# gsc74/DipGenie

Hardware: AMD Instinct MI355X
Metric: dp_state_cells_per_s (higher is better)
Workload: dtype int32

## Files before the change

### dipgenie_amd/capi.py

```python
import contextlib
import ctypes as C
import os
import struct

import numpy as np

_HERE = os.path.dirname(os.path.abspath(__file__))
LIB_PATH = os.environ.get("DG_LIB") or os.path.join(_HERE, "csrc", "libdipgenie_hip.so")

if not os.path.exists(LIB_PATH):
    raise ImportError(
        f"{LIB_PATH} is missing: build it with `make -C dipgenie_amd/csrc` (or __graft_entry__.build()). "
        "dipgenie_amd has no CPU fallback."
    )
try:
    import torch
except ImportError:
    pass
lib = C.CDLL(LIB_PATH)


class DpGraph(C.Structure):
    _fields_ = [
        ("n_vertices", C.c_int32), ("n_levels", C.c_int32), ("R", C.c_int32),
        ("level_off", C.c_void_p), ("out_off", C.c_void_p), ("out_dst", C.c_void_p), ("out_w", C.c_void_p),
        ("hom_off", C.c_void_p), ("het_off", C.c_void_p), ("hom_col", C.c_void_p), ("het_col", C.c_void_p),
    ]


class DpResult(C.Structure):
    _fields_ = [
        ("value", C.c_int32), ("s_het", C.c_int32), ("n_p1", C.c_int32), ("n_p2", C.c_int32),
        ("p1_from", C.c_void_p), ("p1_to", C.c_void_p), ("p2_from", C.c_void_p), ("p2_to", C.c_void_p),
        ("cap", C.c_int32), ("cells", C.c_uint64), ("relaxations", C.c_uint64),
    ]


class DpTiming(C.Structure):
    _fields_ = [
        ("delta_ms", C.c_float), ("forward_ms", C.c_float), ("traceback_ms", C.c_float), ("total_ms", C.c_float),
        ("n_forward_launches", C.c_int64), ("edge_pairs", C.c_uint64), ("colour_entries", C.c_uint64),
        ("state_bytes", C.c_uint64), ("bp_bytes", C.c_uint64), ("delta_bytes", C.c_uint64), ("n_segments", C.c_int32), ("n_chunks", C.c_int32),
    ]


PAIR_SCORE = np.dtype([("value", np.int32), ("s_het", np.int32), ("r1", np.int32), ("r2", np.int32)])

PARTNER = np.dtype([("value", np.int32), ("s_het", np.int32), ("r1", np.int32), ("r2", np.int32)])

LEVEL_MARGIN = np.dtype([("best_vertex", np.int32), ("best_value", np.int32), ("second_vertex", np.int32), ("second_value", np.int32)])

CALL_MARGIN = np.dtype([("vertex", np.int32), ("value", np.int32), ("alt_vertex", np.int32), ("alt_value", np.int32)])

PAIR_OBJECTIVE = np.dtype([("hom_shared", np.int32), ("hom_single", np.int32), ("het_single", np.int32), ("het_both", np.int32)])


class SketchTiming(C.Structure):
    _fields_ = [("kernel_ms", C.c_float), ("sort_ms", C.c_float), ("total_ms", C.c_float), ("n_emitted", C.c_int64)]


SYMBOLS = [
    "dg_create", "dg_destroy", "dg_last_error", "dg_set_stream", "dg_synchronize", "dg_device_info",
    "dg_dp_prealloc", "dg_dp_load_graph", "dg_dp_run", "dg_dp_get_timing", "dg_dp_solve_diploid", "dg_dp_get_level_digest",
    "dg_dp_set_option", "dg_dp_get_launch_profile", "dg_sketch_reads", "dg_sketch_haplotype", "dg_hash_kmers", "dg_free",
    "dg_sketch_get_timing", "dg_sketch_reads_dev", "dg_sketch_count_dictionary_dev", "dg_sketch_merge_runs_dev",
    "dg_sketch_partition_dev", "dg_sketch_rank_dictionary_dev", "dg_sketch_histogram_dev",
    "dg_anchor_begin", "dg_anchor_add_haplotype", "dg_anchor_finish", "dg_dp_solve_haploid", "dg_dp_get_table_digest", "dg_hip_versions", "dg_anchor_add_haplotype_sketched",
    "dg_sketch_set_option", "dg_sketch_get_stat", "dg_sketch_count_rank_dictionary_dev",
    "dg_shard_create", "dg_shard_destroy", "dg_shard_n_ranks", "dg_shard_ctx", "dg_shard_score_reads",
    "dg_dp_run_budgets", "dg_dp_get_budget_values", "dg_dp_score_paths", "dg_dp_best_partners", "dg_dp_partner_marginals",
    "dg_dp_get_option", "dg_sketch_get_option", "dg_dp_list_sweep_variants", "dg_dp_get_answer_paths", "dg_dp_call_margins",
    "dg_dp_objective_paths", "dg_dp_answer_objectives", "dg_dp_get_partner_route",
]

lib.dg_create.restype = C.c_void_p
lib.dg_create.argtypes = [C.c_int]
lib.dg_destroy.argtypes = [C.c_void_p]
lib.dg_destroy.restype = None
lib.dg_last_error.restype = C.c_char_p
lib.dg_set_stream.argtypes = [C.c_void_p, C.c_void_p]
lib.dg_synchronize.argtypes = [C.c_void_p]
lib.dg_device_info.argtypes = [C.c_void_p, C.c_char_p, C.c_int, C.POINTER(C.c_int), C.POINTER(C.c_int64)]
lib.dg_dp_prealloc.argtypes = [C.c_void_p, C.c_int64]
lib.dg_dp_load_graph.argtypes = [C.c_void_p, C.POINTER(DpGraph)]
lib.dg_dp_run.argtypes = [C.c_void_p, C.POINTER(DpResult)]
lib.dg_dp_run_budgets.argtypes = [C.c_void_p, C.c_void_p, C.c_int32, C.POINTER(DpResult)]
lib.dg_dp_get_budget_values.argtypes = [C.c_void_p, C.c_void_p, C.c_int32]
lib.dg_dp_score_paths.argtypes = [C.c_void_p, C.c_void_p, C.c_int64, C.c_void_p]
lib.dg_dp_best_partners.argtypes = [C.c_void_p, C.c_void_p, C.c_int64, C.c_void_p, C.c_void_p, C.c_void_p]
lib.dg_dp_partner_marginals.argtypes = [C.c_void_p, C.c_void_p, C.c_int64, C.c_void_p, C.c_void_p, C.c_void_p]
lib.dg_dp_get_answer_paths.argtypes = [C.c_void_p, C.c_int32, C.c_void_p]
lib.dg_dp_call_margins.argtypes = [C.c_void_p, C.c_int32, C.c_void_p, C.c_void_p, C.c_void_p]
lib.dg_dp_get_partner_route.argtypes = [C.c_void_p, C.POINTER(C.c_int32), C.POINTER(C.c_int64)]
lib.dg_dp_objective_paths.argtypes = [C.c_void_p, C.c_void_p, C.c_int64, C.c_void_p]
lib.dg_dp_answer_objectives.argtypes = [C.c_void_p, C.c_void_p, C.c_int32, C.c_void_p]
lib.dg_dp_get_timing.argtypes = [C.c_void_p, C.POINTER(DpTiming)]
lib.dg_dp_solve_diploid.argtypes = [C.c_void_p, C.POINTER(DpGraph), C.POINTER(DpResult)]
lib.dg_dp_get_level_digest.argtypes = [C.c_void_p, C.c_void_p, C.c_int64]
lib.dg_dp_set_option.argtypes = [C.c_void_p, C.c_char_p, C.c_int64]
lib.dg_dp_get_option.argtypes = [C.c_void_p, C.c_char_p, C.POINTER(C.c_int64)]
lib.dg_dp_get_launch_profile.argtypes = [C.c_void_p, C.c_char_p, C.c_int]
lib.dg_dp_list_sweep_variants.argtypes = [C.c_char_p, C.c_int]
lib.dg_dp_get_table_digest.argtypes = [C.c_void_p, C.c_void_p, C.c_int]
lib.dg_sketch_reads.argtypes = [C.c_void_p, C.c_char_p, C.c_void_p, C.c_int64, C.c_int, C.c_int,
                                C.POINTER(C.c_void_p), C.POINTER(C.c_void_p), C.POINTER(C.c_int64)]
lib.dg_sketch_haplotype.argtypes = [C.c_void_p, C.c_char_p, C.c_int64, C.c_int, C.c_int,
                                    C.POINTER(C.c_void_p), C.POINTER(C.c_void_p), C.POINTER(C.c_int64)]
lib.dg_hash_kmers.argtypes = [C.c_void_p, C.c_char_p, C.c_int64, C.c_int, C.c_void_p]
lib.dg_free.argtypes = [C.c_void_p]
lib.dg_free.restype = None
lib.dg_sketch_get_timing.argtypes = [C.c_void_p, C.POINTER(SketchTiming)]
lib.dg_sketch_reads_dev.argtypes = [C.c_void_p, C.c_void_p, C.c_void_p, C.c_int64, C.c_int64, C.c_int, C.c_int,
                                    C.c_void_p, C.c_void_p, C.c_int64, C.POINTER(C.c_int64)]
lib.dg_sketch_count_dictionary_dev.argtypes = [C.c_void_p, C.c_void_p, C.c_int64, C.c_void_p, C.c_void_p, C.c_int64, C.c_void_p]
lib.dg_sketch_merge_runs_dev.argtypes = [C.c_void_p, C.c_void_p, C.c_void_p, C.c_int64, C.c_void_p, C.c_void_p,
                                         C.c_int64, C.POINTER(C.c_int64)]
lib.dg_sketch_partition_dev.argtypes = [C.c_void_p, C.c_void_p, C.c_int64, C.c_int, C.c_void_p]
lib.dg_sketch_rank_dictionary_dev.argtypes = [C.c_void_p, C.c_void_p, C.c_int64, C.c_void_p, C.c_int64, C.c_int64, C.c_void_p]
lib.dg_sketch_histogram_dev.argtypes = [C.c_void_p, C.c_void_p, C.c_int64, C.c_int, C.c_void_p]
lib.dg_sketch_count_rank_dictionary_dev.argtypes = [C.c_void_p, C.c_void_p, C.c_int64, C.c_void_p, C.c_void_p, C.c_int64, C.c_int64, C.c_void_p, C.c_void_p]
lib.dg_sketch_set_option.argtypes = [C.c_void_p, C.c_char_p, C.c_int64]
lib.dg_sketch_get_option.argtypes = [C.c_void_p, C.c_char_p, C.POINTER(C.c_int64)]
lib.dg_sketch_get_stat.argtypes = [C.c_void_p, C.c_char_p, C.POINTER(C.c_int64)]


class HapGraph(C.Structure):
    _fields_ = [("n_vertices", C.c_int32), ("R", C.c_int32), ("out_off", C.c_void_p), ("out_dst", C.c_void_p), ("out_w", C.c_void_p), ("n_colours", C.c_void_p)]


lib.dg_dp_solve_haploid.argtypes = [C.c_void_p, C.POINTER(HapGraph), C.c_void_p, C.c_void_p, C.c_void_p]


class AnchorResult(C.Structure):
    _fields_ = [("n_occ", C.c_int64), ("n_vtx", C.c_int64), ("occ_id", C.c_void_p), ("occ_hap", C.c_void_p), ("occ_off", C.c_void_p),
                ("occ_len", C.c_void_p), ("vpool", C.c_void_p), ("n_candidates", C.c_int64), ("n_unstable_groups", C.c_int64)]


lib.dg_anchor_begin.argtypes = [C.c_void_p, C.c_int32, C.c_int32, C.c_void_p, C.c_int, C.c_int]
lib.dg_anchor_add_haplotype.argtypes = [C.c_void_p, C.c_int32, C.c_char_p, C.c_int64, C.c_void_p, C.c_void_p, C.c_int64, C.POINTER(C.c_int64)]
lib.dg_anchor_add_haplotype_sketched.argtypes = [C.c_void_p, C.c_int32, C.c_int64, C.c_void_p, C.c_void_p, C.c_int64, C.c_void_p, C.c_void_p, C.c_int64]
lib.dg_anchor_finish.argtypes = [C.c_void_p, C.c_void_p, C.c_int64, C.c_float, C.POINTER(AnchorResult)]


lib.dg_hip_versions.argtypes = [C.POINTER(C.c_int), C.POINTER(C.c_int)]


def hip_versions():
    a, b = C.c_int(), C.c_int()
    if lib.dg_hip_versions(C.byref(a), C.byref(b)) != 0:
        raise DgError(lib.dg_last_error().decode())
    fmt = lambda v: f"{v // 10000000}.{v // 100000 % 100}.{v % 100000}"
    return fmt(a.value), fmt(b.value)


class DgError(RuntimeError):
    pass


def _check(rc, what):
    if rc != 0:
        raise DgError(f"{what} failed (rc={rc}): {lib.dg_last_error().decode()}")


class DpGraphArrays:

    NAMES = ["level_off", "out_off", "out_dst", "out_w", "hom_off", "hom_col", "het_off", "het_col"]
    DTYPES = [np.int32, np.int64, np.int32, np.uint8, np.int64, np.int32, np.int64, np.int32]

    def __init__(self, R, **arrays):
        self.R = int(R)
        for n, dt in zip(self.NAMES, self.DTYPES):
            setattr(self, n, np.ascontiguousarray(arrays[n], dtype=dt))

    @classmethod
    def load(cls, path):
        with open(path, "rb") as f:
            if f.read(8) != b"DGDP0001":
                raise ValueError("not a .dpg file")
            (R,) = struct.unpack("<i", f.read(4))
            arrs = {}
            for n, dt in zip(cls.NAMES, cls.DTYPES):
                (cnt,) = struct.unpack("<Q", f.read(8))
                arrs[n] = np.frombuffer(f.read(cnt * np.dtype(dt).itemsize), dtype=dt).copy()
        return cls(R, **arrs)

    def save(self, path):
        with open(path, "wb") as f:
            f.write(b"DGDP0001")
            f.write(struct.pack("<i", self.R))
            for n in self.NAMES:
                a = getattr(self, n)
                f.write(struct.pack("<Q", a.size))
                f.write(a.tobytes())

    @property
    def n_vertices(self):
        return self.out_off.size - 1

    @property
    def n_levels(self):
        return self.level_off.size - 1

    def as_struct(self, struct_cls=DpGraph):
        g = struct_cls()
        g.n_vertices, g.n_levels, g.R = self.n_vertices, self.n_levels, self.R
        for n in self.NAMES:
            a = getattr(self, n)
            setattr(g, n, a.ctypes.data if a.size else np.zeros(1, a.dtype).ctypes.data)
        return g


class DpOutcome:
    def __init__(self, res, p1, p2):
        self.value, self.s_het = res.value, res.s_het
        self.cells, self.relaxations = res.cells, res.relaxations
        self.p1, self.p2 = p1, p2

    def key(self):
        return (self.value, self.s_het, tuple(self.p1), tuple(self.p2))


def make_result(cap):
    bufs = [np.zeros(cap, np.int32) for _ in range(4)]
    res = DpResult()
    res.p1_from, res.p1_to, res.p2_from, res.p2_to = (b.ctypes.data for b in bufs)
    res.cap = cap
    return res, bufs


def outcome_from(res, bufs):
    p1 = [(int(bufs[0][i]), int(bufs[1][i])) for i in range(res.n_p1)]
    p2 = [(int(bufs[2][i]), int(bufs[3][i])) for i in range(res.n_p2)]
    return DpOutcome(res, p1, p2)


@contextlib.contextmanager
def _options(get, set_, kv):
    saved = []
    try:
        for key, value in kv.items():
            old = get(key)
            set_(key, value)
            saved.append((key, old))
        yield
    finally:
        for key, old in reversed(saved):
            set_(key, old)


class Context:

    def __init__(self, device=0):
        self.h = lib.dg_create(device)
        if not self.h:
            raise DgError(f"dg_create({device}) failed: {lib.dg_last_error().decode()}")

    def close(self):
        if self.h:
            lib.dg_destroy(self.h)
            self.h = None

    def __del__(self):
        try:
            self.close()
        except Exception:
            pass

    def set_stream(self, stream_ptr):
        _check(lib.dg_set_stream(self.h, C.c_void_p(stream_ptr)), "dg_set_stream")

    def device_info(self):
        name = C.create_string_buffer(256)
        ncu, hbm = C.c_int(), C.c_int64()
        _check(lib.dg_device_info(self.h, name, 256, C.byref(ncu), C.byref(hbm)), "dg_device_info")
        return name.value.decode(), ncu.value, hbm.value

    def dp_set_option(self, key, value):
        _check(lib.dg_dp_set_option(self.h, key.encode(), int(value)), "dg_dp_set_option")

    def dp_get_option(self, key):
        v = C.c_int64(0)
        _check(lib.dg_dp_get_option(self.h, key.encode(), C.byref(v)), "dg_dp_get_option")
        return v.value

    def dp_options(self, **kv):
        return _options(self.dp_get_option, self.dp_set_option, kv)

    def dp_prealloc(self, nbytes=0):
        _check(lib.dg_dp_prealloc(self.h, int(nbytes)), "dg_dp_prealloc")

    def dp_load_graph(self, g):
        self._g = g
        st = g.as_struct()
        _check(lib.dg_dp_load_graph(self.h, C.byref(st)), "dg_dp_load_graph")

    def dp_run(self):
        res, bufs = make_result(self._g.R + 8)
        _check(lib.dg_dp_run(self.h, C.byref(res)), "dg_dp_run")
        return outcome_from(res, bufs)

    def dp_run_budgets(self, budgets):
        budgets = [int(b) for b in budgets]
        arr = (DpResult * max(len(budgets), 1))()
        keep = []
        for q, b in enumerate(budgets):
            res, bufs = make_result(max(b, 0) + 8)
            arr[q] = res
            keep.append(bufs)
        want = np.asarray(budgets, np.int32)
        _check(lib.dg_dp_run_budgets(self.h, want.ctypes.data if want.size else None, len(budgets), arr), "dg_dp_run_budgets")
        return [outcome_from(arr[q], keep[q]) for q in range(len(budgets))]

    def dp_budget_values(self):
        out = np.zeros(self._g.R + 1, np.int32)
        _check(lib.dg_dp_get_budget_values(self.h, out.ctypes.data, out.size), "dg_dp_get_budget_values")
        return out

    def dp_score_paths(self, paths):
        p = np.ascontiguousarray(paths, np.int32)
        g = getattr(self, "_g", None)
        if p.ndim != 3 or p.shape[1] != 2 or (g is not None and p.shape[2] != g.n_levels):
            raise ValueError(f"paths must have shape [n, 2, n_levels], got {p.shape}")
        out = np.zeros(p.shape[0], PAIR_SCORE)
        _check(lib.dg_dp_score_paths(self.h, p.ctypes.data if p.size else None, p.shape[0], out.ctypes.data if out.size else None), "dg_dp_score_paths")
        return out

    def dp_best_partners(self, given, budgets, want_paths=True):
        p = np.ascontiguousarray(given, np.int32)
        b = np.ascontiguousarray(budgets, np.int32)
        g = getattr(self, "_g", None)
        if p.ndim != 2 or (g is not None and p.shape[1] != g.n_levels):
            raise ValueError(f"given must have shape [n, n_levels], got {p.shape}")
        if b.shape != (p.shape[0],):
            raise ValueError(f"budgets must have shape [{p.shape[0]}], got {b.shape}")
        out = np.zeros(p.shape[0], PARTNER)
        partners = np.zeros(p.shape, np.int32) if want_paths else None
        _check(lib.dg_dp_best_partners(self.h, p.ctypes.data if p.size else None, p.shape[0], b.ctypes.data if b.size else None,
                                       partners.ctypes.data if want_paths and partners.size else None, out.ctypes.data if out.size else None), "dg_dp_best_partners")
        return out, partners

    def dp_partner_marginals(self, given, budgets, want_vertices=False):
        p = np.ascontiguousarray(given, np.int32)
        b = np.ascontiguousarray(budgets, np.int32)
        g = getattr(self, "_g", None)
        if p.ndim != 2 or (g is not None and p.shape[1] != g.n_levels):
            raise ValueError(f"given must have shape [n, n_levels], got {p.shape}")
        if b.shape != (p.shape[0],):
            raise ValueError(f"budgets must have shape [{p.shape[0]}], got {b.shape}")
        levels = np.zeros(p.shape, LEVEL_MARGIN)
        values = np.zeros((p.shape[0], g.n_vertices if g is not None else 0), np.int32) if want_vertices else None
        _check(lib.dg_dp_partner_marginals(self.h, p.ctypes.data if p.size else None, p.shape[0], b.ctypes.data if b.size else None,
                                           levels.ctypes.data if levels.size else None, values.ctypes.data if want_vertices and values.size else None),
               "dg_dp_partner_marginals")
        return levels, values

    def dp_answer_paths(self, budget):
        g = getattr(self, "_g", None)
        paths = np.zeros((2, g.n_levels if g is not None else 1), np.int32)
        _check(lib.dg_dp_get_answer_paths(self.h, int(budget), paths.ctypes.data), "dg_dp_get_answer_paths")
        return paths

    def dp_call_margins(self, budget, vertex_class=None, want_paths=False):
        g = getattr(self, "_g", None)
        n_levels = g.n_levels if g is not None else 1
        cls = None
        if vertex_class is not None:
            cls = np.ascontiguousarray(vertex_class, np.int32)
            if g is not None and cls.shape != (g.n_vertices,):
                raise ValueError(f"vertex_class must have shape [{g.n_vertices}], got {cls.shape}")
        levels = np.zeros((2, n_levels), CALL_MARGIN)
        paths = np.zeros((2, n_levels), np.int32) if want_paths else None
        _check(lib.dg_dp_call_margins(self.h, int(budget), cls.ctypes.data if cls is not None else None, levels.ctypes.data,
                                      paths.ctypes.data if want_paths else None), "dg_dp_call_margins")
        return levels, paths

    def dp_partner_route(self):
        route, cells = C.c_int32(0), C.c_int64(0)
        _check(lib.dg_dp_get_partner_route(self.h, C.byref(route), C.byref(cells)), "dg_dp_get_partner_route")
        return route.value, cells.value

    def dp_objective_paths(self, paths):
        p = np.ascontiguousarray(paths, np.int32)
        g = getattr(self, "_g", None)
        if p.ndim != 3 or p.shape[1] != 2 or (g is not None and p.shape[2] != g.n_levels):
            raise ValueError(f"paths must have shape [n, 2, n_levels], got {p.shape}")
        out = np.zeros(p.shape[0], PAIR_OBJECTIVE)
        _check(lib.dg_dp_objective_paths(self.h, p.ctypes.data if p.size else None, p.shape[0], out.ctypes.data if out.size else None), "dg_dp_objective_paths")
        return out

    def dp_answer_objectives(self, budgets):
        b = np.ascontiguousarray(budgets, np.int32).reshape(-1)
        out = np.zeros(b.size, PAIR_OBJECTIVE)
        _check(lib.dg_dp_answer_objectives(self.h, b.ctypes.data if b.size else None, b.size, out.ctypes.data if out.size else None), "dg_dp_answer_objectives")
        return out

    def dp_solve(self, g):
        self.dp_load_graph(g)
        return self.dp_run()

    def dp_solve_haploid(self, R, out_off, out_dst, out_w, n_colours):
        out_off = np.ascontiguousarray(out_off, np.int64); out_dst = np.ascontiguousarray(out_dst, np.int32)
        out_w = np.ascontiguousarray(out_w, np.uint8); n_colours = np.ascontiguousarray(n_colours, np.int32)
        n = out_off.size - 1
        g = HapGraph(n, R, out_off.ctypes.data, out_dst.ctypes.data if out_dst.size else 0, out_w.ctypes.data if out_w.size else 0, n_colours.ctypes.data)
        arrs = [np.zeros((n, R + 1), np.int32) for _ in range(3)]
        _check(lib.dg_dp_solve_haploid(self.h, C.byref(g), *(a.ctypes.data for a in arrs)), "dg_dp_solve_haploid")
        return arrs

    def dp_timing(self):
        t = DpTiming()
        _check(lib.dg_dp_get_timing(self.h, C.byref(t)), "dg_dp_get_timing")
        return t

    def dp_launch_profile(self):
        buf = C.create_string_buffer(8192)
        _check(lib.dg_dp_get_launch_profile(self.h, buf, 8192), "dg_dp_get_launch_profile")
        return {k: int(v) for k, v in (item.rsplit(":", 1) for item in buf.value.decode().split())}

    @staticmethod
    def dp_sweep_variants():
        buf = C.create_string_buffer(8192)
        _check(lib.dg_dp_list_sweep_variants(buf, 8192), "dg_dp_list_sweep_variants")
        return buf.value.decode().split()

    TABLES = ["descs", "in_off", "in_edge", "in_dst", "dtrans", "dblk_first", "grp_begin", "dead_cols", "heavy_rows", "rowrec", "rowx", "slots"]

    def dp_table_digest(self):
        out = np.zeros(12, np.uint64)
        _check(lib.dg_dp_get_table_digest(self.h, out.ctypes.data, 12), "dg_dp_get_table_digest")
        return dict(zip(self.TABLES, (int(x) for x in out)))

    def dp_level_digest(self, n_levels):
        out = np.zeros(n_levels, np.uint64)
        _check(lib.dg_dp_get_level_digest(self.h, out.ctypes.data, n_levels), "dg_dp_get_level_digest")
        return out

    def sketch_reads(self, reads, k, w):
        bases = b"".join(reads)
        off = np.zeros(len(reads) + 1, np.int64)
        np.cumsum([len(r) for r in reads], out=off[1:])
        return self.sketch_reads_flat(bases, off, k, w)

    def sketch_reads_flat(self, bases, off, k, w):
        hp, cp, n = C.c_void_p(), C.c_void_p(), C.c_int64()
        off = np.ascontiguousarray(off, np.int64)
        _check(lib.dg_sketch_reads(self.h, bases, off.ctypes.data, off.size - 1, k, w, C.byref(hp), C.byref(cp), C.byref(n)),
               "dg_sketch_reads")
        h = np.ctypeslib.as_array(C.cast(hp, C.POINTER(C.c_uint64)), (n.value,)).copy() if n.value else np.zeros(0, np.uint64)
        c = np.ctypeslib.as_array(C.cast(cp, C.POINTER(C.c_int32)), (n.value,)).copy() if n.value else np.zeros(0, np.int32)
        lib.dg_free(hp)
        lib.dg_free(cp)
        return h, c

    def sketch_haplotype(self, seq, k, w):
        hp, pp, n = C.c_void_p(), C.c_void_p(), C.c_int64()
        _check(lib.dg_sketch_haplotype(self.h, seq, len(seq), k, w, C.byref(hp), C.byref(pp), C.byref(n)), "dg_sketch_haplotype")
        h = np.ctypeslib.as_array(C.cast(hp, C.POINTER(C.c_uint64)), (n.value,)).copy() if n.value else np.zeros(0, np.uint64)
        p = np.ctypeslib.as_array(C.cast(pp, C.POINTER(C.c_int64)), (n.value,)).copy() if n.value else np.zeros(0, np.int64)
        lib.dg_free(hp)
        lib.dg_free(pp)
        return h, p

    def hash_kmers(self, kmers, k):
        n = len(kmers) // k if k > 0 else 0
        out = np.zeros(n, np.uint64)
        _check(lib.dg_hash_kmers(self.h, kmers, n, k, out.ctypes.data), "dg_hash_kmers")
        return out

    def anchor_begin(self, n_haps, n_vertices, top_order_map, k, w):
        top = np.ascontiguousarray(top_order_map, np.int32)
        _check(lib.dg_anchor_begin(self.h, n_haps, n_vertices, top.ctypes.data if top.size else None, k, w), "dg_anchor_begin")

    @staticmethod
    def _steps(step_vtx, step_start):
        sv = np.ascontiguousarray(step_vtx, np.int32)
        ss = np.ascontiguousarray(step_start, np.int64)
        if ss.size != sv.size + 1:
            raise ValueError("step_start needs one entry more than step_vtx")
        return sv if sv.size else np.zeros(1, np.int32), ss, sv.size

    def anchor_add_haplotype(self, h, seq, step_vtx, step_start):
        sv, ss, n_steps = self._steps(step_vtx, step_start)
        n = C.c_int64()
        _check(lib.dg_anchor_add_haplotype(self.h, h, seq, len(seq), sv.ctypes.data, ss.ctypes.data, n_steps, C.byref(n)), "dg_anchor_add_haplotype")
        return n.value

    def anchor_add_haplotype_sketched(self, h, length, hash, pos, step_vtx, step_start):
        sv, ss, n_steps = self._steps(step_vtx, step_start)
        hs = np.ascontiguousarray(hash, np.uint64)
        ps = np.ascontiguousarray(pos, np.int64)
        if hs.size != ps.size:
            raise ValueError("hash and pos differ in length")
        _check(lib.dg_anchor_add_haplotype_sketched(self.h, h, length, hs.ctypes.data if hs.size else None, ps.ctypes.data if ps.size else None, hs.size,
                                                    sv.ctypes.data, ss.ctypes.data, n_steps), "dg_anchor_add_haplotype_sketched")

    def anchor_finish(self, sp_hash, min_shared):
        sp = np.ascontiguousarray(sp_hash, np.uint64)
        res = AnchorResult()
        try:
            _check(lib.dg_anchor_finish(self.h, sp.ctypes.data if sp.size else None, sp.size, float(min_shared), C.byref(res)), "dg_anchor_finish")
            def arr(p, ct, dt, n):
                return np.ctypeslib.as_array(C.cast(p, C.POINTER(ct)), (n,)).astype(dt, copy=True) if n and p else np.zeros(0, dt)
            return dict(occ_id=arr(res.occ_id, C.c_int32, np.int32, res.n_occ), occ_hap=arr(res.occ_hap, C.c_int32, np.int32, res.n_occ),
                        occ_off=arr(res.occ_off, C.c_uint32, np.uint32, res.n_occ), occ_len=arr(res.occ_len, C.c_uint32, np.uint32, res.n_occ),
                        vpool=arr(res.vpool, C.c_int32, np.int32, res.n_vtx), n_candidates=res.n_candidates, n_unstable_groups=res.n_unstable_groups)
        finally:
            for p in (res.occ_id, res.occ_hap, res.occ_off, res.occ_len, res.vpool):
                if p:
                    lib.dg_free(p)

    def sketch_set_option(self, name, value):
        _check(lib.dg_sketch_set_option(self.h, name.encode(), int(value)), "dg_sketch_set_option")

    def sketch_get_option(self, name):
        v = C.c_int64(0)
        _check(lib.dg_sketch_get_option(self.h, name.encode(), C.byref(v)), "dg_sketch_get_option")
        return v.value

    def sketch_options(self, **kv):
        return _options(self.sketch_get_option, self.sketch_set_option, kv)

    def sketch_stat(self, name):
        v = C.c_int64(0)
        _check(lib.dg_sketch_get_stat(self.h, name.encode(), C.byref(v)), "dg_sketch_get_stat")
        return v.value

    def sketch_timing(self):
        t = SketchTiming()
        _check(lib.dg_sketch_get_timing(self.h, C.byref(t)), "dg_sketch_get_timing")
        return t
```

### dipgenie_amd/csrc/dg_dp.hpp

```cpp
#pragma once
#include <condition_variable>
#include <atomic>
#include <map>
#include <mutex>
#include <thread>
#include <tuple>

#include "dg_internal.hpp"

namespace dgi {

constexpr int32_t NEG_INF = INT32_MIN / 4;
constexpr uint32_t BP_NONE = 0xFFFFFFFFu;
constexpr int MAX_K = 1 << 15;
constexpr int BP_MAX_RANK = 255;
constexpr int COOP_MIN = 8;
constexpr int HEAVY_INLINE = 8;
constexpr int ROWX_MAX = 64;
constexpr int DELTA_PER_BLOCK = 256 * 16;
constexpr int DELTA_PAD = 8;
constexpr int32_t CHAIN_CORRUPT = INT32_MIN;
constexpr int64_t DELTA_MAX = 65535, COLOUR_LIST_MAX = 16383;
inline bool colour_lists_fit_delta(int64_t max_hom, int64_t max_het) {
    return max_hom <= COLOUR_LIST_MAX && max_het <= COLOUR_LIST_MAX && 2 * max_hom + 4 * max_het <= DELTA_MAX;
}

struct LevelDesc {
    int32_t a0, k;
    int32_t b0, k2;
    uint32_t in_base;
    int32_t T;
    int64_t delta_off;
    int64_t bp_off;
    int32_t grp_first, ngroups;
    int32_t dead_first, ndead;
    int64_t slot_first;
    int32_t fast_ok, nblocks;
    int32_t heavy_first, n_heavy;
    int32_t bp_wide, bp_nt;
    int64_t rowx_off;
    int32_t rowx_stride;
    int16_t heavy_in[HEAVY_INLINE];
    int32_t dmax;
};

struct TraceOut { int32_t value, s_het, n_e, overflow, corrupt, path_score; };
struct ChainState { int32_t i, j, r, value; };
struct BudgetSlot { int32_t chain, budget, planes, pad_; };
constexpr int BUDGET_SYNC_STRIDE = 128;
constexpr int BUDGET_HELPER_BLOCKS = 80;
struct ColourCsr { const int64_t *hom_off, *het_off; const int32_t *hom_col, *het_col; };

struct SweepArgs {
    const LevelDesc *descs;
    const uint32_t *in_off, *in_edge, *grp_begin;
    const int32_t *in_dst, *dead_cols;
    const uint16_t *delta, *delta_zero;
    char *ring;
    size_t slot_bytes, pad_bytes;
    uint16_t *bp;
    unsigned long long *digest;
    int RP;
    int *progress;
};

struct FastArgs {
    const uint4 *rowrec;
    const uint2 *slots;
    const uint32_t *in_edge, *rowx;
    const int32_t *dead_cols;
    const uint16_t *delta, *delta_zero;
    char *ring;
    uint16_t *bp;
    unsigned long long *digest;
    int RP, pad_bytes;
    uint32_t buf_bytes;
    uint32_t slot_bytes;
    int *progress;
#ifdef DG_SWEEP_PROBE
    unsigned long long *probe;
#endif
};

inline std::atomic<int> &dp_states_on_device(int device) { static std::atomic<int> n[64]; return n[device & 63]; }

struct SweepVariant {
    int rc;
    bool general, coop;
    int index() const;
    std::string name() const;
    bool exists() const;
    static int count();
    static SweepVariant at(int index);
};
struct SweepHist {
    std::vector<int64_t> n = std::vector<int64_t>((size_t)SweepVariant::count(), 0);
    void add(const SweepHist &o, int64_t sign = 1) { for (size_t q = 0; q < n.size(); ++q) n[q] += sign * o.n[q]; }
};

struct DpOptions {
    int64_t side_stream = -1;
    int64_t plane_limit = 1;
    int64_t want_digest = 0;
    int64_t use_fast = 1;
    int64_t adaptive_rc = 1;
    int64_t use_coop = 1;
    int64_t max_blocks = 1024;
    int64_t segment_cells = 0;
    int64_t host_threads = 16;
    int64_t test_poison_level = 0, test_poison_byte = 0xFF;
    int64_t test_force_rc = 0;
    int64_t host_tables = 0;
    int64_t bp_nt_min_cells = 262144;
    int64_t graph_batch = -1;
    int64_t warm_ahead = 128;
    int64_t sync_every = 0;
    int64_t l2_prefetch = 6;
    int64_t use_lean_chain = 1;
    int64_t delta_overlap = 1;
    int64_t pf_far = 128;
    int64_t use_rowx = 1;
    int64_t delta_cap_entries = (int64_t)4 << 30;
    int64_t rc_cap = 65536, rc_t0_ns = 3000, rc_tg_ps = 20000, rc_tw_ps = 50;
    int64_t chunk_units_cfg = (int64_t)4 << 30;
    int64_t score_slab_bytes = (int64_t)256 << 20;
    int64_t partner_slab_bytes = (int64_t)4 << 30;
    int64_t partner_wide = 0;
    int64_t objective_lds_bytes = 131072;
};

struct DpState {
    explicit DpState(int dev) : device(dev) { ++dp_states_on_device(device); }
    ~DpState() { --dp_states_on_device(device); }
    const int device;
    DpOptions opt;
    bool side_stream_ok() const { return opt.side_stream < 0 ? dp_states_on_device(device).load() <= 1 : opt.side_stream != 0; }
    DpState(const DpState &) = delete;
    DpState &operator=(const DpState &) = delete;
    int32_t nV = 0, L = 0, R = 0, RP = 0, cap = 0;
    bool loaded = false;
    bool lean_chain = false;
    std::vector<hipEvent_t> delta_piece_ev;
    std::vector<int32_t> delta_piece_level;
    int delta_piece_next = 0;
    hipStream_t pf_stream = nullptr;
    hipEvent_t pf_ev = nullptr;
    int pf_seq = 0;
    bool pf_active = false;
    int pf_tested = 0;
    std::vector<int> seg_begin;
    std::vector<int64_t> ckpt_off;
    bool graph_failed = false;
    typedef std::tuple<int, int, const void *, int> GraphKey;
    struct Batch { hipGraphExec_t exec = nullptr; SweepHist hist; };
    std::map<GraphKey, Batch> graphs;
    bool all_fast = false;
    size_t state_alloc_bytes = 0;
    std::vector<LevelDesc> descs;
    uint64_t cells = 0, relaxations = 0, edge_pairs = 0, colour_entries = 0;
    int64_t total_units = 0, max_level_units = 0;
    int64_t max_level_cells = 0, delta_entries = 0, n_delta_blocks = 0, pad_front = 0;
    std::vector<int64_t> level_units;
    std::vector<int32_t> dwin_t, level_win;
    int cur_win = -1;
    std::vector<int32_t> dtrans_host;
    std::vector<int64_t> dblk_first_host;
    int64_t delta_buf_entries = 0;
    std::vector<int32_t> level_dmax;
    int64_t n_grp = 0, n_dead = 0, n_heavy_rows = 0, n_slot_records = 0, n_rowx_words = 0, n_dtrans = 0, n_edges = 0;
    DevBuf d_descs, d_in_off, d_in_edge, d_in_dst, d_hom_off, d_het_off, d_hom_col, d_het_col, d_eflag, d_eself;
    DevBuf d_delta, d_bp, d_ring, d_digest, d_dblk_first, d_dtrans, d_grp, d_dead, d_heavy, d_rowrec, d_rowx, d_slots, d_ckpt, d_pfctl;
#ifdef DG_SWEEP_PROBE
    DevBuf d_probe;
#endif
    std::vector<uint64_t> digest_host;
    SweepHist launch_hist;
    dg_dp_timing timing;
    hipEvent_t ev[4] = {nullptr, nullptr, nullptr, nullptr};
    struct Pool {
        std::mutex mu;
        std::condition_variable cv;
        std::vector<void *> chunks;
        size_t chunk_units = (size_t)DpOptions().chunk_units_cfg;
        size_t target = 0;
        size_t cap_chunks = 0;
        bool running = false, failed = false, paused = false;
        std::thread th;
    } pool;
    std::vector<int> chunk_begin;
    int seg_chunks = 1;
    DevBuf d_sink, d_ch_path, d_ch_state, d_ch_sync, d_ch_trace, d_ch_edges, d_ch_tab;
    std::vector<int32_t> sink_host;
    std::vector<BudgetSlot> tab_host;
    int n_groups = 0;
    mutable int walk_seq = 0;
    DevBuf d_sc_paths, d_sc_out, d_sc_err;
    DevBuf d_pt_pairs, d_pt_bud, d_pt_val, d_pt_out, d_pt_err, d_pt_bp, d_pt_scores;
    DevBuf d_pt_state;
    int32_t pt_route = 0;
    int64_t pt_route_cells = 0;
    DevBuf d_mg_levels, d_mg_vertex;
    bool run_ok = false;
    DevBuf d_ans_paths, d_ans_cnt;
    DevBuf d_cm_class, d_cm_out;
    bool ob_dict = false;
    int64_t ob_ch = 0, ob_ct = 0;
    DevBuf d_ob_hom_rank, d_ob_het_rank, d_ob_paths, d_ob_out, d_ob_err, d_ob_bits;
};

inline ColourCsr colour_csr(const DpState &S) {
    return ColourCsr{S.d_hom_off.as<int64_t>(), S.d_het_off.as<int64_t>(), S.d_hom_col.as<int32_t>(), S.d_het_col.as<int32_t>()};
}

void pool_request(DpState &S, int device, size_t target);
void pool_trim(DpState &S, size_t keep);
inline void pool_clear(DpState &S) { pool_trim(S, 0); }
void *pool_wait(DpState &S, size_t c);
struct PoolPause {
    DpState &S;
    explicit PoolPause(DpState &s);
    ~PoolPause();
};
void graphs_clear(DpState &S);
double wall_s();

int dp_load(dg_ctx *c, const dg_dp_graph *g);
int dp_build_tables_device(dg_ctx *c, const dg_dp_graph *g, DpState &S, std::vector<int32_t> &dtrans, std::vector<int64_t> &dblk_first, int &max_k);
int dp_table_digest(dg_ctx *c, uint64_t *out, int n);

void delta_launch_edge_flags(const DpState &S, hipStream_t s);
const uint16_t *delta_launch_window(DpState &S, int w, hipStream_t s);
const uint16_t *delta_launch_overlapped(DpState &S, hipStream_t s);
void delta_overlap_free(DpState &S);

struct SweepLaunch {
    SweepArgs A;
    FastArgs F;
    bool small_state = true;
    int rc_sel = 0;
    bool digest = false;
    int rp_active = 0;
    SweepHist hist;
};
void sweep_prepare(const DpState &S, SweepLaunch &X);
void sweep_init_state(const DpState &S, hipStream_t s);
int sweep_launch_level(const DpState &S, SweepLaunch &X, int l, hipStream_t s);
void sweep_warm_tables(const DpState &S, const SweepLaunch &X, int q0, int q1, hipStream_t s);
int sweep_prefetch_begin(DpState &S, const SweepLaunch &X, int lb, int le, bool delta_resident, hipStream_t s);
void sweep_prefetch_end(DpState &S, int le, hipStream_t s);
void sweep_prefetch_free(DpState &S);

void trace_launch_warm_rows(const DpState &S, int lb, int le, hipStream_t s);
void trace_launch_chains(const DpState &S, int n, int l_hi, int l_lo, const uint16_t *bp_biased, const int32_t *final_val, hipStream_t s);
void trace_launch_finish_chain(const DpState &S, const uint2 *path, int32_t *edges, const ChainState *st, TraceOut *out, hipStream_t s);
void trace_debug_report(const DpState &S, int n);

void budgets_launch_sink_copy(const DpState &S, const int32_t *sink_state, hipStream_t s);
int budgets_reserve(DpState &S, int n);
int budgets_prepare(DpState &S, const int32_t *budgets, int n, hipStream_t s);
void budgets_launch_finish(const DpState &S, int n, hipStream_t s);
int budgets_find_chain(const char *fn, const DpState *S, int32_t budget, int &chain);
void budgets_launch_expand(const DpState &S, int chain, int swap, int32_t *out, int32_t *cnt, hipStream_t s);
int dp_get_answer_paths(dg_ctx *c, int32_t budget, int32_t *paths);

int dp_score_paths(dg_ctx *c, const int32_t *paths, int64_t n_pairs, dg_dp_pair_score *out);
int score_pair_blocks(const DpState &S);
void score_launch_pairs(const DpState &S, const int32_t *pairs, int64_t n, int32_t *out, unsigned long long *err, hipStream_t s);

int dp_objective_paths(dg_ctx *c, const int32_t *paths, int64_t n_pairs, dg_dp_pair_objective *out);
int dp_answer_objectives(dg_ctx *c, const int32_t *budgets, int32_t n_budgets, dg_dp_pair_objective *out);
int64_t objective_lds_limit(const dg_ctx *c);

int dp_best_partners(dg_ctx *c, const int32_t *given, int64_t n, const int32_t *budgets, int32_t *partners, dg_dp_partner *out);

int dp_partner_marginals(dg_ctx *c, const int32_t *given, int64_t n, const int32_t *budgets, dg_dp_level_margin *levels, int32_t *vertex_values);
int dp_call_margins(dg_ctx *c, int32_t budget, const int32_t *vertex_class, dg_dp_call_margin *levels, int32_t *paths);

}
```

### dipgenie_amd/csrc/dg_dp_run.hip

```cpp
#include <algorithm>
#include <cstdlib>
#include <cstring>
#include <ctime>

#include "dg_dp.hpp"

namespace dgi {

constexpr int DELTA_NO_PIECES = 1 << 30;

double wall_s() { struct timespec ts; clock_gettime(CLOCK_MONOTONIC, &ts); return ts.tv_sec + 1e-9 * ts.tv_nsec; }

void graphs_clear(DpState &S) {
    for (auto &kv : S.graphs) if (kv.second.exec) (void)hipGraphExecDestroy(kv.second.exec);
    S.graphs.clear();
}

void dp_state_free(DpState *s) {
    if (!s) return;
    graphs_clear(*s);
    sweep_prefetch_free(*s);
    delta_overlap_free(*s);
    { std::unique_lock<std::mutex> lk(s->pool.mu); s->pool.target = 0; }
    s->pool.cv.notify_all();
    if (s->pool.th.joinable()) s->pool.th.join();
    const double tf0 = wall_s();
    for (void *q : s->pool.chunks) (void)hipFree(q);
    if (getenv("DG_DEBUG")) fprintf(stderr, "[dipgenie_hip] destroy: %zu lattice chunks freed in %.3f s\n", s->pool.chunks.size(), wall_s() - tf0);
    for (auto &e : s->ev) if (e) (void)hipEventDestroy(e);
    delete s;
}

void pool_request(DpState &S, int device, size_t target) {
    std::unique_lock<std::mutex> lk(S.pool.mu);
    S.pool.target = std::max(target, S.pool.chunks.size());
    if (S.pool.running || S.pool.chunks.size() >= S.pool.target) return;
    if (S.pool.th.joinable()) { lk.unlock(); S.pool.th.join(); lk.lock(); }
    S.pool.running = true;
    S.pool.failed = false;
    DpState *Sp = &S;
    S.pool.th = std::thread([Sp, device]() {
        (void)hipSetDevice(device);
        for (;;) {
            size_t bytes;
            {
                std::unique_lock<std::mutex> lk2(Sp->pool.mu);
                Sp->pool.cv.wait(lk2, [&] { return !Sp->pool.paused || Sp->pool.chunks.size() >= Sp->pool.target; });
                if (Sp->pool.chunks.size() >= Sp->pool.target) { Sp->pool.running = false; Sp->pool.cv.notify_all(); return; }
                bytes = Sp->pool.chunk_units * 2;
            }
            void *q = nullptr;
            const hipError_t e = hipMalloc(&q, bytes);
            std::unique_lock<std::mutex> lk2(Sp->pool.mu);
            if (e != hipSuccess) { (void)hipGetLastError(); Sp->pool.failed = true; Sp->pool.running = false; Sp->pool.cv.notify_all(); return; }
            Sp->pool.chunks.push_back(q);
            Sp->pool.cv.notify_all();
            lk2.unlock();
            std::this_thread::sleep_for(std::chrono::milliseconds(1));
        }
    });
}
PoolPause::PoolPause(DpState &s) : S(s) { std::unique_lock<std::mutex> lk(S.pool.mu); S.pool.paused = true; }
PoolPause::~PoolPause() { { std::unique_lock<std::mutex> lk(S.pool.mu); S.pool.paused = false; } S.pool.cv.notify_all(); }
void pool_trim(DpState &S, size_t keep) {
    { std::unique_lock<std::mutex> lk(S.pool.mu); S.pool.target = std::min(std::min(S.pool.target, keep), S.pool.chunks.size()); }
    S.pool.cv.notify_all();
    if (S.pool.th.joinable()) S.pool.th.join();
    std::unique_lock<std::mutex> lk(S.pool.mu);
    while (S.pool.chunks.size() > keep) { (void)hipFree(S.pool.chunks.back()); S.pool.chunks.pop_back(); }
    S.pool.running = false;
}
void *pool_wait(DpState &S, size_t c) {
    std::unique_lock<std::mutex> lk(S.pool.mu);
    S.pool.cv.wait(lk, [&] { return S.pool.chunks.size() > c || S.pool.failed || !S.pool.running; });
    return S.pool.chunks.size() > c ? S.pool.chunks[c] : nullptr;
}

namespace {

struct Run {
    dg_ctx *c;
    DpState &S;
    hipStream_t s;
    SweepLaunch X;
    int64_t n_launch = 0;
    int next_warm = 0;
    double host_enqueue_s = 0;
    int n_chains = 1;
    std::vector<uint16_t *> pool_base;

    Run(dg_ctx *c_, DpState &S_) : c(c_), S(S_), s(c_->stream) { sweep_prepare(S, X); }
    int n_win() const { return (int)S.dwin_t.size() - 1; }
    int32_t *state_ptr(int level) const { return (int32_t *)(S.d_ring.as<char>() + (size_t)(level & 1) * S.state_alloc_bytes) + S.pad_front; }
    size_t level_cells(int level) const {
        const int64_t k = level == 0 ? 1 : S.descs[level].k2;
        return (size_t)(k * k * S.RP);
    }
    void load_window(int w) { X.A.delta = X.F.delta = delta_launch_window(S, w, s); }

    int issue_levels(int l0, int l1, int lb, int le) {
        for (int l = l0; l < l1; ++l) {
            if (S.level_win[l] >= 0 && S.level_win[l] != S.cur_win) load_window(S.level_win[l]);
            if (S.opt.warm_ahead > 0 && l >= next_warm && (l == lb || !(S.pf_active && S.opt.pf_far > 0))) {
                const int q0 = l == lb ? l : (int)std::min<int64_t>(l + S.opt.warm_ahead, le), q1 = (int)std::min<int64_t>(l + 2 * S.opt.warm_ahead, le);
                if (q1 > q0) sweep_warm_tables(S, X, q0, q1, s);
            }
            if (l >= next_warm) next_warm = l + (int)std::max<int64_t>(S.opt.warm_ahead, 1);
            if (int rc = sweep_launch_level(S, X, l, s)) return rc;
            ++n_launch;
            if (S.opt.sync_every > 0 && n_launch % S.opt.sync_every == 0) DG_HIP(hipStreamSynchronize(s));
        }
        return DG_OK;
    }

    int sweep_range(int lb, int le, uint16_t *bp_biased) {
        X.A.bp = bp_biased; X.F.bp = bp_biased;
        next_warm = lb;
        if (int rc = sweep_prefetch_begin(S, X, lb, le, n_win() == 1, s)) return rc;
        const int64_t gb = S.opt.graph_batch >= 0 ? S.opt.graph_batch : 1000;
        const int pf_key = ((S.pf_active && S.opt.pf_far > 0) ? 1 : 0) | (X.rp_active << 1);
        for (int l0 = lb; l0 < le;) {
            const bool use_graph = gb > 0 && n_win() == 1 && S.opt.sync_every == 0 && !S.graph_failed;
            const int l1 = use_graph ? (int)std::min<int64_t>((int64_t)l0 + gb, le) : le;
            while (S.delta_piece_next < (int)S.delta_piece_level.size() && S.delta_piece_level[S.delta_piece_next] < l1) {
                DG_HIP(hipStreamWaitEvent(s, S.delta_piece_ev[S.delta_piece_next], 0));
                ++S.delta_piece_next;
            }
            const DpState::GraphKey key(l0, l1, (const void *)bp_biased, pf_key);
            DpState::Batch *slot = nullptr;
            bool capturing = false;
            if (use_graph) {
                slot = &S.graphs[key];
                if (slot->exec) {
                    DG_HIP(hipGraphLaunch(slot->exec, s));
                    X.hist.add(slot->hist);
                    n_launch += l1 - l0; l0 = l1;
                    continue;
                }
                if (hipStreamBeginCapture(s, hipStreamCaptureModeThreadLocal) == hipSuccess) capturing = true;
                else { (void)hipGetLastError(); S.graph_failed = true; continue; }
            }
            const int64_t n_launch_before = n_launch;
            const SweepHist hist_before = X.hist;
            if (int rc = issue_levels(l0, l1, lb, le)) {
                if (capturing) {
                    hipGraph_t cg = nullptr;
                    (void)hipStreamEndCapture(s, &cg);
                    if (cg) (void)hipGraphDestroy(cg);
                    (void)hipGetLastError();
                    S.graphs.erase(key);
                }
                return rc;
            }
            if (capturing) {
                hipGraph_t cg = nullptr;
                const bool ok = hipStreamEndCapture(s, &cg) == hipSuccess && cg && hipGraphInstantiate(&slot->exec, cg, nullptr, nullptr, 0) == hipSuccess;
                if (cg) (void)hipGraphDestroy(cg);
                if (!ok) {
                    (void)hipGetLastError();
                    slot->exec = nullptr; S.graph_failed = true; n_launch = n_launch_before; X.hist = hist_before;
                    continue;
                }
                slot->hist = X.hist;
                slot->hist.add(hist_before, -1);
                DG_HIP(hipGraphLaunch(slot->exec, s));
            }
            l0 = l1;
        }
        sweep_prefetch_end(S, le, s);
        return DG_OK;
    }

    int wait_for_chunks() {
        if (S.d_bp.p) return DG_OK;
        const double tw0 = wall_s();
        const size_t need = (size_t)std::min(S.seg_chunks, (int)S.chunk_begin.size() - 1);
        if (!pool_wait(S, need - 1)) { set_error("back-pointer lattice: hipMalloc of a %.1f GB chunk failed", S.pool.chunk_units * 2 / 1e9); return DG_ERR_OOM; }
        std::unique_lock<std::mutex> lk(S.pool.mu);
        for (size_t q = 0; q < need; ++q) pool_base.push_back((uint16_t *)S.pool.chunks[q]);
        if (getenv("DG_DEBUG")) fprintf(stderr, "[dipgenie_hip] run: waited %.3f s for lattice chunks\n", wall_s() - tw0);
        return DG_OK;
    }

    std::tuple<int, int, uint16_t *> chunk(int ch, int c0) const {
        const int lb = S.d_bp.p ? 1 : S.chunk_begin[ch], le = S.d_bp.p ? S.L : S.chunk_begin[ch + 1];
        return {lb, le, (S.d_bp.p ? S.d_bp.as<uint16_t>() : pool_base[ch - c0]) - S.descs[lb].bp_off};
    }

    int sweep_and_walk(int c0, int c1, bool from_sink, bool mark_forward_end) {
        for (int ch = c0; ch < c1; ++ch) {
            const auto [lb, le, bp] = chunk(ch, c0);
            const double th0 = wall_s();
            if (int rc = sweep_range(lb, le, bp)) return rc;
            host_enqueue_s += wall_s() - th0;
        }
        if (mark_forward_end) { DG_HIP(hipEventRecord(S.ev[2], s)); budgets_launch_sink_copy(S, state_ptr(S.L - 1), s); }
        if (S.opt.test_poison_level > 0 && S.opt.test_poison_level < S.L)
            for (int ch = c0; ch < c1; ++ch) {
                const auto [lb, le, bp] = chunk(ch, c0);
                const int lp = (int)S.opt.test_poison_level;
                if (lp >= lb && lp < le) DG_HIP(hipMemsetAsync(bp + S.descs[lp].bp_off, (int)S.opt.test_poison_byte, 2 * (size_t)S.level_units[lp], s));
            }
        for (int ch = c1 - 1; ch >= c0; --ch) {
            const auto [lb, le, bp] = chunk(ch, c0);
            trace_launch_warm_rows(S, lb, le, s);
            const int32_t *final_val = from_sink && ch == c1 - 1 ? state_ptr(S.L - 1) : (const int32_t *)nullptr;
            trace_launch_chains(S, n_chains, le - 1, lb, bp, final_val, s);
        }
        return DG_OK;
    }

    int forward_and_trace() {
        const int n_seg = (int)S.seg_begin.size() - 1, n_chunks_all = (int)S.chunk_begin.size() - 1;
        DG_HIP(hipEventRecord(S.ev[0], s));
        S.cur_win = -1;
        S.delta_piece_next = DELTA_NO_PIECES;
        if (n_win() == 1 && S.n_delta_blocks > 0) X.A.delta = X.F.delta = delta_launch_overlapped(S, s);
        DG_HIP(hipEventRecord(S.ev[1], s));
        if (S.opt.want_digest) DG_HIP(hipMemsetAsync(S.d_digest.p, 0, 8 * (size_t)S.L, s));
#ifdef DG_SWEEP_PROBE
        {
            std::vector<unsigned long long> init((size_t)S.L * 8, 0ULL);
            for (int l = 0; l < S.L; ++l) init[(size_t)l * 8] = ~0ULL;
            DG_HIP(hipMemcpy(S.d_probe.p, init.data(), 8 * init.size(), hipMemcpyHostToDevice));
        }
#endif
        sweep_init_state(S, s);
        if (n_seg == 1) {
            if (int rc = sweep_and_walk(0, S.d_bp.p ? 1 : n_chunks_all, true, true)) return rc;
        } else {
            int64_t planes_swept = 0;
            for (int sg = 0; sg < n_seg; ++sg) {
                if (sg > 0)
                    DG_HIP(hipMemcpyAsync(S.d_ckpt.as<int32_t>() + S.ckpt_off[sg], state_ptr(S.seg_begin[sg] - 1),
                                          4 * level_cells(S.seg_begin[sg] - 1), hipMemcpyDeviceToDevice, s));
                if (int rc = sweep_range(S.seg_begin[sg], S.seg_begin[sg + 1], nullptr)) return rc;
            }
            DG_HIP(hipEventRecord(S.ev[2], s));
            budgets_launch_sink_copy(S, state_ptr(S.L - 1), s);
            X.digest = false;
            for (int sg = n_seg - 1; sg >= 0; --sg) {
                const int lb = S.seg_begin[sg];
                if (sg > 0)
                    DG_HIP(hipMemcpyAsync(state_ptr(lb - 1), S.d_ckpt.as<int32_t>() + S.ckpt_off[sg], 4 * level_cells(lb - 1), hipMemcpyDeviceToDevice, s));
                else
                    sweep_init_state(S, s);
                const int c0 = sg * S.seg_chunks, c1 = std::min(n_chunks_all, c0 + S.seg_chunks);
                if (int rc = sweep_and_walk(c0, c1, sg == n_seg - 1, false)) return rc;
                if (S.opt.plane_limit && sg > 0) {
                    std::vector<ChainState> cs((size_t)n_chains);
                    DG_HIP(hipMemcpyAsync(cs.data(), S.d_ch_state.p, sizeof(ChainState) * cs.size(), hipMemcpyDeviceToHost, s));
                    DG_HIP(hipStreamSynchronize(s));
                    int planes = 1;
                    for (const ChainState &q : cs) {
                        if (q.value == NEG_INF) continue;
                        planes = std::max(planes, (q.value != CHAIN_CORRUPT && q.r >= 0 && q.r < S.RP) ? q.r + 1 : S.RP);
                    }
                    X.rp_active = planes;
                    planes_swept += (int64_t)planes * (S.seg_begin[sg] - S.seg_begin[sg - 1]);
                }
            }
            if (getenv("DG_DEBUG") && S.opt.plane_limit) fprintf(stderr, "[dipgenie_hip] run: second pass swept %.1f %% of the (level, plane) pairs before the last segment\n",
                                                              100.0 * (double)planes_swept / std::max(1.0, (double)S.RP * (S.seg_begin[n_seg - 1] - 1)));
        }
        budgets_launch_finish(S, n_chains, s);
        DG_HIP(hipEventRecord(S.ev[3], s));
        DG_HIP(hipGetLastError());
        return DG_OK;
    }
};

}

static int emit_result(const DpState &S, const TraceOut &to, const int32_t *edges, dg_dp_result *res, int budget) {
    char who[32] = "";
    if (budget >= 0) snprintf(who, sizeof who, " (budget %d)", budget);
    if (to.value == CHAIN_CORRUPT || to.corrupt) { set_error("back-pointer lattice is corrupt: the chain walk left its level (a level was not swept?)%s", who); return DG_ERR_STATE; }
    if (to.value != NEG_INF && to.path_score != to.value) {
        set_error("traceback path scores %d but the DP value is %d: sweep, lattice and walk disagree%s", to.path_score, to.value, who); return DG_ERR_STATE;
    }
    if (to.overflow || to.n_e > S.cap) { set_error("traceback edge list overflow (%d > %d)%s", to.n_e, S.cap, who); return DG_ERR_STATE; }
    res->value = to.value; res->s_het = to.s_het;
    res->cells = S.cells; res->relaxations = S.relaxations;
    std::vector<int> order(to.n_e);
    for (int q = 0; q < to.n_e; ++q) order[q] = q;
    std::stable_sort(order.begin(), order.end(), [&](int a, int b) { return edges[a] < edges[b]; });
    int n1 = 0, n2 = 0;
    for (int q : order) {
        const int from = edges[S.cap + q], tov = edges[2 * S.cap + q];
        if (edges[3 * S.cap + q] == 0) { if (n1 < res->cap && res->p1_from && res->p1_to) { res->p1_from[n1] = from; res->p1_to[n1] = tov; } ++n1; }
        else { if (n2 < res->cap && res->p2_from && res->p2_to) { res->p2_from[n2] = from; res->p2_to[n2] = tov; } ++n2; }
    }
    res->n_p1 = n1; res->n_p2 = n2;
    return DG_OK;
}

static int dp_run(dg_ctx *c, const int32_t *budgets, int n_budgets, dg_dp_result *res, bool name_budget) {
    DpState &S = *c->dp;
    Run run(c, S);
    hipStream_t s = c->stream;
    if (int rc = run.wait_for_chunks()) return rc;
    std::vector<TraceOut> to((size_t)n_budgets);
    std::vector<int32_t> edges(4 * (size_t)S.cap * (size_t)n_budgets);
    S.run_ok = false;
    if (int rc = budgets_prepare(S, budgets, n_budgets, s)) return rc;
    run.n_chains = n_budgets;
    S.sink_host.clear();
    const int rc_run = run.forward_and_trace();
    S.launch_hist = run.X.hist;
    if (rc_run) return rc_run;
    DG_HIP(hipMemcpyAsync(to.data(), S.d_ch_trace.p, sizeof(TraceOut) * to.size(), hipMemcpyDeviceToHost, s));
    DG_HIP(hipMemcpyAsync(edges.data(), S.d_ch_edges.p, 4 * edges.size(), hipMemcpyDeviceToHost, s));
    std::vector<int32_t> sink((size_t)S.RP);
    DG_HIP(hipMemcpyAsync(sink.data(), S.d_sink.p, 4 * sink.size(), hipMemcpyDeviceToHost, s));
    if (S.opt.want_digest) {
        S.digest_host.assign(S.L, 0);
        DG_HIP(hipMemcpyAsync(S.digest_host.data(), S.d_digest.p, 8 * (size_t)S.L, hipMemcpyDeviceToHost, s));
    }
    DG_HIP(hipStreamSynchronize(s));
    S.sink_host.swap(sink);
#ifdef DG_SWEEP_PROBE
    if (const char *po = getenv("DG_PROBE_OUT")) {
        std::vector<unsigned long long> pr((size_t)S.L * 8);
        DG_HIP(hipMemcpy(pr.data(), S.d_probe.p, 8 * pr.size(), hipMemcpyDeviceToHost));
        if (FILE *f = fopen(po, "wb")) { fwrite(pr.data(), 8, pr.size(), f); fclose(f); }
    }
#endif
    if (getenv("DG_DEBUG") && S.lean_chain) trace_debug_report(S, n_budgets);
    if (getenv("DG_DEBUG") && S.pf_stream) {
        int w[4] = {0, 0, 0, 0};
        if (hipStreamSynchronize(S.pf_stream) == hipSuccess && hipMemcpy(w, S.d_pfctl.p, sizeof w, hipMemcpyDeviceToHost) == hipSuccess)
            fprintf(stderr, "[dipgenie_hip] run: L2 table prefetcher covered %d levels (since load)\n", w[2]);
    }
    if (getenv("DG_DEBUG"))
        fprintf(stderr, "[dipgenie_hip] run: host issued %lld sweep launches in %.1f ms (%.2f us each)\n", (long long)run.n_launch, 1e3 * run.host_enqueue_s,
                1e6 * run.host_enqueue_s / (double)std::max<int64_t>(run.n_launch, 1));
    DG_HIP(hipEventElapsedTime(&S.timing.delta_ms, S.ev[0], S.ev[1]));
    DG_HIP(hipEventElapsedTime(&S.timing.forward_ms, S.ev[1], S.ev[2]));
    DG_HIP(hipEventElapsedTime(&S.timing.traceback_ms, S.ev[2], S.ev[3]));
    DG_HIP(hipEventElapsedTime(&S.timing.total_ms, S.ev[0], S.ev[3]));
    S.timing.n_forward_launches = run.n_launch;
    S.timing.n_segments = (int32_t)S.seg_begin.size() - 1;
    S.timing.n_chunks = (int32_t)S.chunk_begin.size() - 1;
    for (int q = 0; q < n_budgets; ++q)
        if (int rc = emit_result(S, to[q], edges.data() + 4 * (size_t)S.cap * (size_t)q, res + q, name_budget ? budgets[q] : -1)) return rc;
    S.run_ok = true;
    return DG_OK;
}

static int dp_run_budgets(dg_ctx *c, const int32_t *budgets, int32_t n, dg_dp_result *results) {
    DpState *Sp = c->dp;
    if (!Sp || !Sp->loaded) { set_error("dg_dp_run_budgets: no graph loaded"); return DG_ERR_STATE; }
    if (!budgets || !results || n <= 0) { set_error("dg_dp_run_budgets: budgets, results and n_budgets > 0 are required"); return DG_ERR_ARG; }
    std::vector<char> seen((size_t)Sp->RP, 0);
    for (int q = 0; q < n; ++q) {
        const int b = budgets[q];
        if (b < 0 || b > Sp->R) { set_error("dg_dp_run_budgets: budget %d (entry %d) outside 0..%d, the R of the loaded graph", b, q, Sp->R); return DG_ERR_ARG; }
        if (seen[b]) { set_error("dg_dp_run_budgets: budget %d listed twice", b); return DG_ERR_ARG; }
        seen[b] = 1;
        if (results[q].cap < b + 2) { set_error("dg_dp_run_budgets: results[%d].cap = %d, budget %d needs %d", q, results[q].cap, b, b + 2); return DG_ERR_ARG; }
    }
    return dp_run(c, budgets, n, results, true);
}

static int dp_run_single(dg_ctx *c, dg_dp_result *res) {
    if (!c->dp || !c->dp->loaded) { set_error("dg_dp_run: no graph loaded"); return DG_ERR_STATE; }
    if (!res) { set_error("dg_dp_run: null result"); return DG_ERR_ARG; }
    const int32_t budget = c->dp->R;
    return dp_run(c, &budget, 1, res, false);
}

}

extern "C" int dg_dp_load_graph(dg_ctx *c, const dg_dp_graph *g) {
    if (int rc = dgi::bind(c)) return rc;
    return dgi::dp_load(c, g);
}
extern "C" int dg_dp_run(dg_ctx *c, dg_dp_result *r) {
    if (int rc = dgi::bind(c)) return rc;
    return dgi::dp_run_single(c, r);
}
extern "C" int dg_dp_run_budgets(dg_ctx *c, const int32_t *budgets, int32_t n_budgets, dg_dp_result *results) {
    if (int rc = dgi::bind(c)) return rc;
    return dgi::dp_run_budgets(c, budgets, n_budgets, results);
}
extern "C" int dg_dp_get_budget_values(dg_ctx *c, int32_t *out, int32_t n) {
    if (!c || !c->dp || !out) { dgi::set_error("dg_dp_get_budget_values: no state"); return DG_ERR_STATE; }
    const std::vector<int32_t> &v = c->dp->sink_host;
    if (v.empty()) { dgi::set_error("dg_dp_get_budget_values: no completed dg_dp_run / dg_dp_run_budgets on the loaded graph"); return DG_ERR_STATE; }
    if (n < (int32_t)v.size()) { dgi::set_error("dg_dp_get_budget_values: out has %d entries, R + 1 = %zu needed", n, v.size()); return DG_ERR_ARG; }
    memcpy(out, v.data(), 4 * v.size());
    return DG_OK;
}
extern "C" int dg_dp_solve_diploid(dg_ctx *c, const dg_dp_graph *g, dg_dp_result *r) {
    if (int rc = dg_dp_load_graph(c, g)) return rc;
    return dg_dp_run(c, r);
}
extern "C" int dg_dp_prealloc(dg_ctx *c, int64_t bytes) {
    if (int rc = dgi::bind(c)) return rc;
    if (!c->dp) c->dp = new dgi::DpState(c->device);
    dgi::DpState &S = *c->dp;
    if (S.pool.chunk_units != (size_t)S.opt.chunk_units_cfg) { dgi::pool_clear(S); S.pool.chunk_units = (size_t)S.opt.chunk_units_cfg; }
    const size_t chunk_bytes = S.pool.chunk_units * 2;
    if (S.pool.cap_chunks == 0) {
        size_t free_b = 0, total_b = 0;
        DG_HIP(hipMemGetInfo(&free_b, &total_b));
        S.pool.cap_chunks = std::max<size_t>(1, (size_t)(0.6 * (double)free_b) / chunk_bytes);
    }
    const size_t want_chunks = bytes > 0 ? std::min(((size_t)bytes + chunk_bytes - 1) / chunk_bytes, S.pool.cap_chunks) : S.pool.cap_chunks;
    dgi::pool_request(S, c->device, want_chunks);
    return DG_OK;
}
extern "C" int dg_dp_get_timing(dg_ctx *c, dg_dp_timing *t) {
    if (!c || !c->dp || !t) { dgi::set_error("dg_dp_get_timing: no state"); return DG_ERR_STATE; }
    *t = c->dp->timing;
    return DG_OK;
}
extern "C" int dg_dp_get_level_digest(dg_ctx *c, uint64_t *out, int64_t n) {
    if (!c || !c->dp || !out) { dgi::set_error("dg_dp_get_level_digest: no state"); return DG_ERR_STATE; }
    if ((int64_t)c->dp->digest_host.size() != n) { dgi::set_error("digest not collected (set option digest=1) or size mismatch"); return DG_ERR_STATE; }
    memcpy(out, c->dp->digest_host.data(), 8 * (size_t)n);
    return DG_OK;
}
extern "C" int dg_dp_get_table_digest(dg_ctx *c, uint64_t *out, int n) {
    if (int rc = dgi::bind(c)) return rc;
    return dgi::dp_table_digest(c, out, n);
}
extern "C" int dg_dp_get_launch_profile(dg_ctx *c, char *buf, int cap) {
    if (!c || !c->dp || !buf || cap < 2) { dgi::set_error("dg_dp_get_launch_profile: no state"); return DG_ERR_STATE; }
    std::string out;
    for (int q = 0; q < dgi::SweepVariant::count(); ++q)
        if (const int64_t n = c->dp->launch_hist.n[(size_t)q]) out += (out.empty() ? "" : " ") + dgi::SweepVariant::at(q).name() + ':' + std::to_string(n);
    if ((int)out.size() + 1 > cap) { dgi::set_error("dg_dp_get_launch_profile: buffer too small (%zu needed)", out.size() + 1); return DG_ERR_ARG; }
    memcpy(buf, out.c_str(), out.size() + 1);
    return DG_OK;
}
extern "C" int dg_dp_list_sweep_variants(char *buf, int cap) {
    std::string out;
    for (int q = 0; q < dgi::SweepVariant::count(); ++q)
        if (dgi::SweepVariant::at(q).exists()) out += (out.empty() ? "" : " ") + dgi::SweepVariant::at(q).name();
    if (!buf || (int)out.size() + 1 > cap) { dgi::set_error("dg_dp_list_sweep_variants: buffer too small (%zu needed)", out.size() + 1); return DG_ERR_ARG; }
    memcpy(buf, out.c_str(), out.size() + 1);
    return DG_OK;
}
typedef dgi::DpOptions DpO;
static const struct DpOptionKey { const char *key; int64_t DpO::*field; int64_t lo; bool nonpos_is_default; } dp_option_keys[] = {
    {"digest", &DpO::want_digest, 0, false}, {"fast", &DpO::use_fast, 0, false}, {"adaptive_rc", &DpO::adaptive_rc, 0, false}, {"coop", &DpO::use_coop, 0, false},
    {"sync_every", &DpO::sync_every, 0, false}, {"rc_t0_ns", &DpO::rc_t0_ns, 0, false}, {"rc_tg_ps", &DpO::rc_tg_ps, 0, false}, {"rc_tw_ps", &DpO::rc_tw_ps, 0, false},
    {"rc_cap", &DpO::rc_cap, 0, true}, {"max_blocks", &DpO::max_blocks, 0, true}, {"bp_nt_min_cells", &DpO::bp_nt_min_cells, 0, false}, {"warm_ahead", &DpO::warm_ahead, 0, false},
    {"graph_batch", &DpO::graph_batch, -1, false}, {"l2_prefetch", &DpO::l2_prefetch, 0, false}, {"delta_overlap", &DpO::delta_overlap, 0, false}, {"pf_far", &DpO::pf_far, 0, false},
    {"side_stream", &DpO::side_stream, -1, false}, {"plane_limit", &DpO::plane_limit, 0, false}, {"test_poison_level", &DpO::test_poison_level, 0, false},
    {"test_poison_byte", &DpO::test_poison_byte, 0, false}, {"test_force_rc", &DpO::test_force_rc, 0, false}, {"score_slab_bytes", &DpO::score_slab_bytes, 0, true}, {"partner_slab_bytes", &DpO::partner_slab_bytes, 0, true},
    {"partner_wide", &DpO::partner_wide, 0, false},
    {"objective_lds_bytes", &DpO::objective_lds_bytes, 0, true},
    {"rowx", &DpO::use_rowx, 0, false}, {"lean_chain", &DpO::use_lean_chain, 0, false}, {"segment_cells", &DpO::segment_cells, 0, false},
    {"host_threads", &DpO::host_threads, 1, false}, {"host_tables", &DpO::host_tables, 0, false}, {"delta_cap_entries", &DpO::delta_cap_entries, 0, true},
    {"lattice_chunk_cells", &DpO::chunk_units_cfg, 1, false},
};
static int dp_option(dg_ctx *c, const char *what, const char *key, const int64_t *set, int64_t *get) {
    if (!c || !key || (!set && !get)) { dgi::set_error("%s: null", what); return DG_ERR_ARG; }
    if (!c->dp) c->dp = new dgi::DpState(c->device);
    dgi::DpState &S = *c->dp;
    if (set) dgi::graphs_clear(S);
    for (const DpOptionKey &o : dp_option_keys) {
        if (strcmp(key, o.key)) continue;
        if (!set) { *get = S.opt.*o.field; return DG_OK; }
        int64_t v = *set;
        if (o.field == &DpO::chunk_units_cfg) {
            if (v < o.lo) { dgi::set_error("lattice_chunk_cells must be positive"); return DG_ERR_ARG; }
            dgi::pool_clear(S);
            v = (int64_t)(S.pool.chunk_units = ((size_t)v + 1) & ~(size_t)1);
        }
        if (o.field == &DpO::objective_lds_bytes) v = std::min(v, dgi::objective_lds_limit(c));
        if (o.field == &DpO::partner_wide) v = std::min<int64_t>(v, 2);
        S.opt.*o.field = o.nonpos_is_default && v <= 0 ? DpO().*o.field : v < o.lo ? o.lo : v;
        return DG_OK;
    }
    dgi::set_error("unknown option %s", key);
    return DG_ERR_ARG;
}
extern "C" int dg_dp_set_option(dg_ctx *c, const char *key, int64_t v) { return dp_option(c, "dg_dp_set_option", key, &v, nullptr); }
extern "C" int dg_dp_get_option(dg_ctx *c, const char *key, int64_t *value) { return dp_option(c, "dg_dp_get_option", key, nullptr, value); }
```

### dipgenie_amd/csrc/dg_dp_sweep.hip

```cpp
#include <algorithm>
#include <cmath>
#include <type_traits>

#include "dg_dp.hpp"

namespace dgi {

#define DG_SLOT(LEVEL) ((LEVEL) & 1)

constexpr unsigned long long DIGEST_PRED_MUL = 0x9E3779B97F4A7C15ULL;

__device__ __forceinline__ void store_bp_nt(uint16_t *p, uint32_t v) { asm volatile("global_store_short %0, %1, off nt" ::"v"(p), "v"(v) : "memory"); }
__device__ __forceinline__ uint32_t ord_rank(int eu, int ev) { return ((uint32_t)(BP_MAX_RANK - eu) << 8) | (uint32_t)(BP_MAX_RANK - ev); }

__device__ __forceinline__ unsigned long long digest_term(int value, unsigned long long o, uint32_t pred_i, uint32_t pred_j) {
    return (unsigned long long)(uint32_t)(value + 1) * (o + 1) +
           DIGEST_PRED_MUL * ((((unsigned long long)pred_i << 15) | pred_j) + 1ULL) * (o + 1);
}

__device__ __forceinline__ int lane_down1(int x) { return __builtin_amdgcn_update_dpp(x, x, 0x130 , 0xF, 0xF, false); }
__device__ __forceinline__ int lane_up1(int x) { return __builtin_amdgcn_update_dpp(x, x, 0x138 , 0xF, 0xF, false); }

struct LevelHead {
    const uint4 *rowrec_l;
    const uint2 *slots_l;
    const uint32_t *rowx_l;
    const int32_t *cur;
    const uint16_t *dm;
    int rowx_stride, RP, k, pad_bytes, dT;
    uint32_t buf_bytes;
};

__device__ __forceinline__ __amdgpu_buffer_rsrc_t state_rsrc(const int32_t *padded_base, uint32_t bytes) {
    return __builtin_amdgcn_make_buffer_rsrc((void *)padded_base, 0, bytes, 0x00020000);
}

__device__ __forceinline__ void publish_level(int *progress, int lvl) {
    if ((blockIdx.x | blockIdx.y | blockIdx.z) == 0 && threadIdx.x == 0) __hip_atomic_store(progress, lvl, __ATOMIC_RELAXED, __HIP_MEMORY_SCOPE_AGENT);
}

__device__ __forceinline__ uint32_t ord_word(int i, int j, int wu, int wv) {
    return ((uint32_t)(0x7FFF - i) << 17) | ((uint32_t)(0x7FFF - j) << 2) | ((uint32_t)wu << 1) | (uint32_t)wv;
}
__device__ __forceinline__ uint32_t bp_from_ord(uint32_t o) {
    const uint32_t i = 0x7FFFu - (o >> 17), j = 0x7FFFu - ((o >> 2) & 0x7FFFu);
    return i | (j << 15) | (((o >> 1) & 1u) << 30) | ((o & 1u) << 31);
}
template <int RC, bool DIGEST>
__device__ __forceinline__ void sweep_level_pairs(const SweepArgs &A, int lvl, int wave_id, int n_waves) {
    const LevelDesc d = A.descs[lvl];
    const int RP = A.RP;
    const int32_t *__restrict__ cur = (const int32_t *)(A.ring + (size_t)DG_SLOT(lvl - 1) * A.slot_bytes + A.pad_bytes);
    int32_t *__restrict__ nxt = (int32_t *)(A.ring + (size_t)DG_SLOT(lvl) * A.slot_bytes + A.pad_bytes);
    const int lane = threadIdx.x & 63;
    const int nchunk = (RP + RC - 1) / RC;
    const int64_t ntask = (int64_t)d.k2 * d.ngroups * nchunk;
    const bool has_delta = d.delta_off >= 0;
    const uint16_t *dm = has_delta ? A.delta + d.delta_off : A.delta_zero;
    const int dT = has_delta ? d.T : 0, dmask = has_delta ? -1 : 0;
    const uint32_t *gb = A.grp_begin + d.grp_first;
    unsigned long long dsum = 0;
    for (int64_t task = wave_id; task < ntask; task += n_waves) {
        const int g = (int)(task % d.ngroups);
        const int64_t rest = task / d.ngroups;
        const int rc = (int)(rest % nchunk), i2 = (int)(rest / nchunk);
        const int r0 = rc * RC;
        const uint32_t gbeg = gb[g], gend = gb[g + 1];
        const uint32_t eu0 = A.in_off[d.b0 + i2], eu1 = A.in_off[d.b0 + i2 + 1];
        int bval[RC];
        uint32_t bord[RC];
#pragma unroll
        for (int q = 0; q < RC; ++q) { bval[q] = NEG_INF; bord[q] = 0; }
        int j2 = -1 - lane;
        for (uint32_t cb = gbeg; cb < gend; cb += 64) {
            const uint32_t ev = cb + lane;
            const bool act = ev < gend;
            int j = 0, wv = 0, evr = 0;
            if (act) {
                const uint32_t pv = A.in_edge[ev];
                j = (int)(pv & 0x7FFFFFFFu); wv = (int)(pv >> 31);
                const int cv = A.in_dst[ev];
                j2 = cv - d.b0;
                if (!d.bp_wide) evr = (int)(ev - A.in_off[cv]);
            }
            const int dcol = (int)(ev - d.in_base) & dmask;
            for (uint32_t eu = eu0; eu < eu1; ++eu) {
                const uint32_t pu = A.in_edge[eu];
                const int i = (int)(pu & 0x7FFFFFFFu), wu = (int)(pu >> 31);
                if (act) {
                    const int w = wu + wv;
                    const int dl = (int)dm[(int64_t)(eu - d.in_base) * dT + dcol];
                    const uint32_t ord = d.bp_wide ? ord_word(i, j, wu, wv) : ord_rank((int)(eu - eu0), evr);
                    const int32_t *base = cur + ((int64_t)i * RP + (r0 - w)) * d.k + j;
                    int vals[RC];
#pragma unroll
                    for (int q = 0; q < RC; ++q) vals[q] = base[q * d.k];
#pragma unroll
                    for (int q = 0; q < RC; ++q) {
                        const int cand = vals[q] + dl;
                        const bool ok = (r0 + q < RP) & (r0 + q - w >= 0) & (vals[q] != NEG_INF);
                        const bool take = ok & ((cand > bval[q]) | ((cand == bval[q]) & (ord > bord[q])));
                        bval[q] = take ? cand : bval[q];
                        bord[q] = take ? ord : bord[q];
                    }
                }
            }
        }
        const int span = (int)min(gend - gbeg, 64u);
        for (int s = 1; s < span; s <<= 1) {
            const int oj2 = __shfl_down(j2, s);
            const bool same = (lane + s < 64) & (oj2 == j2);
#pragma unroll
            for (int q = 0; q < RC; ++q) {
                const int ov = __shfl_down(bval[q], s);
                const uint32_t oo = (uint32_t)__shfl_down((int)bord[q], s);
                const bool take = same & ((ov > bval[q]) | ((ov == bval[q]) & (oo > bord[q])));
                bval[q] = take ? ov : bval[q];
                bord[q] = take ? oo : bord[q];
            }
        }
        const int pj2 = __shfl_up(j2, 1);
        const bool head = (j2 >= 0) & ((lane == 0) | (pj2 != j2));
        if (head) {
#pragma unroll
            for (int q = 0; q < RC; ++q) {
                const int r2 = r0 + q;
                if (r2 < RP) {
                    const int64_t idx = ((int64_t)i2 * RP + r2) * d.k2 + j2;
                    nxt[idx] = bval[q];
                    if (A.bp) {
                        if (d.bp_wide) __builtin_nontemporal_store((uint32_t)(bval[q] == NEG_INF ? BP_NONE : bp_from_ord(bord[q])), (uint32_t *)(A.bp + d.bp_off + 2 * idx));
                        else __builtin_nontemporal_store((uint16_t)~bord[q], &A.bp[d.bp_off + idx]);
                    }
                    if (DIGEST && bval[q] != NEG_INF) {
                        const unsigned long long o = ((unsigned long long)r2 * d.k2 + i2) * d.k2 + j2;
                        uint32_t pi, pj;
                        if (d.bp_wide) { const uint32_t h = bp_from_ord(bord[q]); pi = h & 0x7FFFu; pj = (h >> 15) & 0x7FFFu; }
                        else {
                            const uint32_t ru = BP_MAX_RANK - (bord[q] >> 8), rv = BP_MAX_RANK - (bord[q] & 0xFFu);
                            pi = A.in_edge[eu0 + ru] & 0x7FFFFFFFu;
                            pj = A.in_edge[A.in_off[d.b0 + j2] + rv] & 0x7FFFFFFFu;
                        }
                        dsum += digest_term(bval[q], o, pi, pj);
                    }
                }
            }
        }
        if (g == 0 && d.ndead > 0) {
            for (int t = lane; t < d.ndead * RC; t += 64) {
                const int q = t % RC, c = A.dead_cols[d.dead_first + t / RC];
                if (r0 + q < RP) {
                    const int64_t idx = ((int64_t)i2 * RP + r0 + q) * d.k2 + c;
                    nxt[idx] = NEG_INF;
                    if (A.bp) {
                        if (d.bp_wide) __builtin_nontemporal_store((uint32_t)(BP_NONE), (uint32_t *)(A.bp + d.bp_off + 2 * idx));
                        else __builtin_nontemporal_store((uint16_t)0xFFFFu, &A.bp[d.bp_off + idx]);
                    }
                }
            }
        }
    }
    if (DIGEST && dsum) atomicAdd(&A.digest[lvl], dsum);
}

template <int RC, bool DIGEST>
__global__ __launch_bounds__(256) void dp_sweep_kernel(SweepArgs A, int lvl) {
    sweep_level_pairs<RC, DIGEST>(A, lvl, (int)(blockIdx.x * 4 + (threadIdx.x >> 6)), (int)(gridDim.x * 4));
}

__global__ void dp_init_kernel(int32_t *cur, int RP) {
    const int r = (int)(blockIdx.x * blockDim.x + threadIdx.x);
    if (r < RP) cur[r] = 0;
}


template <int RC>
__device__ __forceinline__ void relax_select(const int (&vals)[RC], int dl, uint32_t ord, int r0, int w, int RP,
                                             int (&bval)[RC], uint32_t (&bord)[RC]) {
#pragma unroll
    for (int q = 0; q < RC; ++q) {
        const int cand = vals[q] + dl;
        const bool ok = (r0 + q < RP) & (r0 + q - w >= 0) & (vals[q] != NEG_INF);
        const bool take = ok & ((cand > bval[q]) | ((cand == bval[q]) & (ord > bord[q])));
        bval[q] = take ? cand : bval[q];
        bord[q] = take ? ord : bord[q];
    }
}

__device__ __forceinline__ void merge_best(int ov, uint32_t oo, bool same, int &bv, uint32_t &bo) {
    const bool take = same & ((ov > bv) | ((ov == bv) & (oo > bo)));
    bv = take ? ov : bv;
    bo = take ? oo : bo;
}

#ifdef DG_SWEEP_PROBE
#define DG_PROBE_BEGIN unsigned long long pq[6] = {0, 0, 0, 0, 0, 0}; \
    const bool probe_on = A.probe != nullptr && blockIdx.x == 0 && blockIdx.y == 0 && (threadIdx.x >> 6) == 0 && (int)blockIdx.z < d.k2;
#define DG_PROBE(q) do { if (probe_on) { asm volatile("s_waitcnt vmcnt(0) lgkmcnt(0)" ::: "memory"); pq[q] = __builtin_amdgcn_s_memrealtime(); } } while (0)
#define DG_PROBE_END do { if (probe_on && (threadIdx.x & 63) == 0) { \
        atomicMin(&A.probe[(size_t)lvl * 8 + 0], pq[0]); atomicMax(&A.probe[(size_t)lvl * 8 + 1], pq[5]); \
        if ((int)blockIdx.z == d.k2 / 2) for (int q = 0; q < 6; ++q) A.probe[(size_t)lvl * 8 + 2 + q] = pq[q]; } } while (0)
#else
#define DG_PROBE_BEGIN
#define DG_PROBE(q) do { } while (0)
#define DG_PROBE_END do { } while (0)
#endif

template <int RC, bool DIGEST, bool GENERAL, int COOP>
__device__ __forceinline__ void sweep_task(const LevelHead &H, const FastArgs &A, const LevelDesc &d, __amdgpu_buffer_rsrc_t cur_rsrc,
                                           int32_t *__restrict__ nxt, int i2, int g, int r0, int lvl, int part = 0, uint2 *ex = nullptr) {
    const int lane = threadIdx.x & 63;
    const int RP = H.RP;
    DG_PROBE_BEGIN
    DG_PROBE(0);
    const uint4 rr = H.rowrec_l[i2];
    uint2 sl = H.slots_l[g * 64 + lane];
    const bool rowx = !GENERAL && H.rowx_stride > 0;
    uint32_t mypu = 0;
    if (rowx && lane < H.rowx_stride) mypu = H.rowx_l[i2 * H.rowx_stride + lane];
    int steps = __builtin_amdgcn_readfirstlane((int)(sl.y >> 28));
    const int j2 = (sl.x != 0xFFFFFFFFu) ? (int)((sl.x >> 16) & 0x7FFFu) : -1 - lane;
    int nblk = 1;
    if (GENERAL) {
        if (steps == 14) return;
        if (steps == 15) {
            const int col = __builtin_amdgcn_readfirstlane(j2);
            nblk = ((int)H.rowrec_l[col].y + 63) >> 6;
            steps = 6;
        }
    }
    const uint16_t *dm = H.dm;
    const int dT = H.dT;
    const bool has_delta = dT != 0;
    const int du = (int)rr.y;
    if (COOP == 1 && du > COOP_MIN) return;
    DG_PROBE(1);
    const int t_lo = COOP == 2 ? (du * part) >> 2 : 0, t_hi = COOP == 2 ? (du * (part + 1)) >> 2 : du;
    int bval[RC];
    uint32_t bord[RC];
#pragma unroll
    for (int q = 0; q < RC; ++q) { bval[q] = NEG_INF; bord[q] = 0; }
    const int64_t erow0 = (int64_t)rr.x * dT;
    const int rowbytes = H.k * 4;
    bool act = false;
    for (int blk = 0; blk < (GENERAL ? nblk : 1); ++blk) {
        if (GENERAL && blk > 0) sl = H.slots_l[(g + blk) * 64 + lane];
        const bool actb = sl.x != 0xFFFFFFFFu;
        act |= actb;
        const int j = (int)(sl.x & 0x7FFFu), wv = (int)((sl.x >> 15) & 1u);
        const int dcol = has_delta ? (int)(sl.y & 0x000FFFFFu) : 0;
        const int evr = (int)((sl.y >> 20) & 0xFFu);
        if (du <= 2) {
            if (actb && du > 0) {
                const int ia = (int)(rr.z & 0x7FFFu), wa = (int)(rr.z >> 31) + wv;
                const int ib = (int)(rr.w & 0x7FFFu), wb = (int)(rr.w >> 31) + wv;
                const int offa = ((ia * RP + (r0 - wa)) * H.k + j) * 4 + H.pad_bytes;
                const int offb = ((ib * RP + (r0 - wb)) * H.k + j) * 4 + H.pad_bytes;
                int va[RC], vb[RC];
                const int dla = (int)dm[erow0 + dcol];
                int dlb = 0;
#pragma unroll
                for (int q = 0; q < RC; ++q)
                    va[q] = __builtin_amdgcn_raw_buffer_load_b32(cur_rsrc, offa + q * rowbytes, 0, 0);
                if (du == 2) {
                    dlb = (int)dm[erow0 + dT + dcol];
#pragma unroll
                    for (int q = 0; q < RC; ++q)
                        vb[q] = __builtin_amdgcn_raw_buffer_load_b32(cur_rsrc, offb + q * rowbytes, 0, 0);
                }
                relax_select<RC>(va, dla, ord_rank(0, evr), r0, wa, RP, bval, bord);
                if (du == 2) relax_select<RC>(vb, dlb, ord_rank(1, evr), r0, wb, RP, bval, bord);
            }
        } else {
            constexpr int U = GENERAL ? (RC >= 4 ? 2 : 4) : (RC >= 8 ? 2 : (RC >= 4 ? 4 : 8));
            for (int c0 = GENERAL ? t_lo : 0; c0 < t_hi; c0 += GENERAL ? 64 : (1 << 30)) {
                const int tb = GENERAL ? c0 : t_lo, te = GENERAL ? min(c0 + 64, t_hi) : t_hi;
                if (!rowx) { mypu = 0; if (c0 + lane < te) mypu = A.in_edge[rr.x + c0 + lane]; }
                for (int t = tb; t < te; t += U) {
                    uint32_t wmask = 0;
                    if (actb) {
                        int vals[U][RC], dl[U];
#pragma unroll
                        for (int u = 0; u < U; ++u) {
                            if (t + u < te) {
                                const uint32_t p = (uint32_t)__builtin_amdgcn_readlane((int)mypu, t + u - c0);
                                wmask |= (p >> 31) << u;
                                const int iu = (int)(p & 0x7FFFFFFFu), w = (int)(p >> 31) + wv;
                                const int off = ((iu * RP + (r0 - w)) * H.k + j) * 4 + H.pad_bytes;
                                dl[u] = (int)dm[erow0 + (int64_t)(t + u) * dT + dcol];
#pragma unroll
                                for (int q = 0; q < RC; ++q)
                                    vals[u][q] = __builtin_amdgcn_raw_buffer_load_b32(cur_rsrc, off + q * rowbytes, 0, 0);
                            }
                        }
#pragma unroll
                        for (int u = 0; u < U; ++u) {
                            if (t + u < te) {
                                const int wu = (int)((wmask >> u) & 1u);
                                relax_select<RC>(vals[u], dl[u], ord_rank(t + u, evr), r0, wu + wv, RP, bval, bord);
                            }
                        }
                    }
                }
            }
        }
    }
    DG_PROBE(2);
    if (COOP == 2) {
        if (part > 0) {
#pragma unroll
            for (int q = 0; q < RC; ++q) ex[((part - 1) * RC + q) * 64 + lane] = make_uint2((uint32_t)bval[q], bord[q]);
        }
        __syncthreads();
        if (part > 0) return;
#pragma unroll
        for (int p = 0; p < 3; ++p) {
#pragma unroll
            for (int q = 0; q < RC; ++q) {
                const uint2 o = ex[(p * RC + q) * 64 + lane];
                merge_best((int)o.x, o.y, true, bval[q], bord[q]);
            }
        }
    }
    if (steps > 0) {
        const int oj2 = lane_down1(j2);
        const bool same = (lane + 1 < 64) & (oj2 == j2);
#pragma unroll
        for (int q = 0; q < RC; ++q) merge_best(lane_down1(bval[q]), (uint32_t)lane_down1((int)bord[q]), same, bval[q], bord[q]);
    }
    for (int st = 1, sh = 2; st < steps; ++st, sh <<= 1) {
        const int oj2 = __shfl_down(j2, sh);
        const bool same = (lane + sh < 64) & (oj2 == j2);
#pragma unroll
        for (int q = 0; q < RC; ++q) merge_best(__shfl_down(bval[q], sh), (uint32_t)__shfl_down((int)bord[q], sh), same, bval[q], bord[q]);
    }
    const int pj2 = lane_up1(j2);
    const bool head = act & ((lane == 0) | (pj2 != j2));
    unsigned long long dsum = 0;
    DG_PROBE(3);
    if (head) {
#pragma unroll
        for (int q = 0; q < RC; ++q) {
            const int r2 = r0 + q;
            if (r2 < RP) {
                const int idx = (i2 * RP + r2) * d.k2 + j2;
                nxt[idx] = bval[q];
                if (A.bp) { if (d.bp_nt) store_bp_nt(&A.bp[d.bp_off + idx], ~bord[q]); else A.bp[d.bp_off + idx] = (uint16_t)~bord[q]; }
                if (DIGEST && bval[q] != NEG_INF) {
                    const unsigned long long o = ((unsigned long long)r2 * d.k2 + i2) * d.k2 + j2;
                    const uint32_t ru = BP_MAX_RANK - (bord[q] >> 8), rv = BP_MAX_RANK - (bord[q] & 0xFFu);
                    const uint32_t pi = A.in_edge[rr.x + ru] & 0x7FFFFFFFu;
                    const uint32_t pj = A.in_edge[H.rowrec_l[j2].x + rv] & 0x7FFFFFFFu;
                    dsum += digest_term(bval[q], o, pi, pj);
                }
            }
        }
    }
    if (g == 0 && d.ndead > 0) {
        for (int t = lane; t < d.ndead * RC; t += 64) {
            const int q = t % RC, c = A.dead_cols[d.dead_first + t / RC];
            if (r0 + q < RP) {
                const int64_t idx = ((int64_t)i2 * RP + r0 + q) * d.k2 + c;
                nxt[idx] = NEG_INF;
                if (A.bp) { if (d.bp_nt) store_bp_nt(&A.bp[d.bp_off + idx], 0xFFFFu); else A.bp[d.bp_off + idx] = (uint16_t)0xFFFFu; }
            }
        }
    }
    if (DIGEST && dsum) atomicAdd(&A.digest[lvl], dsum);
#ifdef DG_SWEEP_PROBE
    if (probe_on) pq[4] = __builtin_amdgcn_s_memrealtime();
    DG_PROBE(5);
    DG_PROBE_END;
#endif
}

#ifndef DG_PLAIN_WG
#define DG_PLAIN_WG 256
#endif
#define DG_PLAIN_GW ((DG_PLAIN_WG / 64) < 4 ? (DG_PLAIN_WG / 64) : 4)
#define DG_PLAIN_CH ((DG_PLAIN_WG / 64) / DG_PLAIN_GW)
template <int RC, bool DIGEST, bool GENERAL>
__global__ __launch_bounds__(DG_PLAIN_WG) void dp_sweep_fast_kernel(const uint4 *rowrec_l, const uint2 *slots_l, const uint32_t *rowx_l, const int32_t *cur, const uint16_t *dm,
                                                            int rowx_stride, int nblocks, int rp_k, int pad_bytes, int dT, uint32_t buf_bytes,
                                                            FastArgs A, LevelDesc d, int lvl) {
    const LevelHead H{rowrec_l, slots_l, rowx_l, cur, dm, rowx_stride, rp_k & 0x1FFF, rp_k >> 13, pad_bytes, dT, buf_bytes};
    publish_level(A.progress, lvl);
    const int wv = (int)(threadIdx.x >> 6);
    const int g = (int)blockIdx.x * DG_PLAIN_GW + (wv % DG_PLAIN_GW);
    const int r0 = ((int)blockIdx.y * DG_PLAIN_CH + wv / DG_PLAIN_GW) * RC;
    if (g >= nblocks || r0 >= (rp_k & 0x1FFF)) return;
    int32_t *nxt = (int32_t *)(A.ring + (size_t)DG_SLOT(lvl) * A.slot_bytes + A.pad_bytes);
    sweep_task<RC, DIGEST, GENERAL, 0>(H, A, d, state_rsrc(cur, buf_bytes), nxt, (int)blockIdx.z, g, r0, lvl);
}

template <int RC, bool DIGEST, bool GENERAL>
__global__ __launch_bounds__(256) void dp_sweep_coop_kernel(const uint4 *rowrec_l, const uint2 *slots_l, const uint32_t *rowx_l, const int32_t *cur,
                                                            int rowx_stride, int nblocks, int n_heavy, int rp_k, unsigned long long heavy_lo,
                                                            unsigned long long heavy_hi,
                                                            FastArgs A, LevelDesc d, int lvl, const uint16_t *dm, int dT, const int32_t *__restrict__ heavy_rows) {
    const LevelHead H{rowrec_l, slots_l, rowx_l, cur, dm, rowx_stride, rp_k & 0x1FFF, rp_k >> 13, A.pad_bytes, dT, A.buf_bytes};
    publish_level(A.progress, lvl);
    int32_t *nxt = (int32_t *)(A.ring + (size_t)DG_SLOT(lvl) * A.slot_bytes + A.pad_bytes);
    const int r0 = (int)blockIdx.y * RC;
    const int zc = 4 * n_heavy;
    if ((int)blockIdx.z < zc) {
        __shared__ uint2 ex[3 * RC * 64];
        const int hz = (int)blockIdx.z;
        const int g = (int)blockIdx.x * 4 + (hz & 3);
        if (g >= nblocks) return;
        const int h = hz >> 2;
        int i2;
        if (h < 4) i2 = (int)((heavy_lo >> (16 * h)) & 0xFFFFu);
        else if (h < HEAVY_INLINE) i2 = (int)((heavy_hi >> (16 * (h - 4))) & 0xFFFFu);
        else i2 = heavy_rows[d.heavy_first + h];
        sweep_task<RC, DIGEST, GENERAL, 2>(H, A, d, state_rsrc(cur, A.buf_bytes), nxt, i2, g, r0, lvl, (int)(threadIdx.x >> 6), ex);
        return;
    }
    const int g = (int)blockIdx.x * 4 + (int)(threadIdx.x >> 6);
    if (g >= nblocks) return;
    sweep_task<RC, DIGEST, GENERAL, 1>(H, A, d, state_rsrc(cur, A.buf_bytes), nxt, (int)blockIdx.z - zc, g, r0, lvl);
}

constexpr int WARM_RANGES = 5;
struct WarmRanges { const char *p[WARM_RANGES]; long long n16[WARM_RANGES]; };
__global__ __launch_bounds__(256) void dp_warm_tables_kernel(WarmRanges W) {
    const long long tid = (long long)blockIdx.x * blockDim.x + threadIdx.x, nth = (long long)gridDim.x * blockDim.x;
#pragma unroll
    for (int q = 0; q < WARM_RANGES; ++q) {
        const uint4 *p = (const uint4 *)W.p[q];
        for (long long i = tid; i < W.n16[q]; i += nth) { uint4 v = p[i]; asm volatile("" ::"v"(v.x), "v"(v.y), "v"(v.z), "v"(v.w)); }
    }
}

constexpr int PF_WORKGROUPS = 16, PF_FAR_WORKGROUPS = 16;
constexpr unsigned long long PF_IDLE_TICKS = 30000;
struct PfCtl { int seq, stop, levels_done, probe, probe_ok, pad_[27]; int level; int pad2_[31]; };

__global__ void dp_pf_ctl_kernel(PfCtl *c, int seq, int level, int stop) {
    __hip_atomic_store(&c->level, level, __ATOMIC_RELAXED, __HIP_MEMORY_SCOPE_AGENT);
    __hip_atomic_store(&c->stop, stop, __ATOMIC_RELAXED, __HIP_MEMORY_SCOPE_AGENT);
    __hip_atomic_store(&c->seq, seq, __ATOMIC_RELEASE, __HIP_MEMORY_SCOPE_AGENT);
}

__global__ void dp_pf_probe_wait_kernel(PfCtl *c, int token) {
    const unsigned long long t0 = __builtin_amdgcn_s_memrealtime();
    int ok = 0;
    while (__builtin_amdgcn_s_memrealtime() - t0 < 200000ULL) {
        if (__hip_atomic_load(&c->probe, __ATOMIC_RELAXED, __HIP_MEMORY_SCOPE_AGENT) == token) { ok = 1; break; }
        __builtin_amdgcn_s_sleep(16);
    }
    c->probe_ok = ok;
}
__global__ void dp_pf_probe_set_kernel(PfCtl *c, int token) { __hip_atomic_store(&c->probe, token, __ATOMIC_RELAXED, __HIP_MEMORY_SCOPE_AGENT); }

__global__ __launch_bounds__(64) void dp_l2_prefetch_kernel(const LevelDesc *__restrict__ descs, FastArgs F, PfCtl *ctl, int seq, int lb, int le, int ahead_near, int delta_resident, int far) {
    __shared__ int dump[64];
#define DG_DROP_LOAD(PTR) __builtin_amdgcn_global_load_lds((const __attribute__((address_space(1))) void *)(PTR), (__attribute__((address_space(3))) void *)dump, 4, 0, 0)
    const bool far_role = (int)blockIdx.x >= PF_WORKGROUPS;
    const int lane = (int)threadIdx.x;
    const int slot = far_role ? (int)blockIdx.x - PF_WORKGROUPS : (int)(blockIdx.x >> 3), nslot = far_role ? (int)gridDim.x - PF_WORKGROUPS : PF_WORKGROUPS >> 3;
    const int ahead = far_role ? far : ahead_near, behind = far_role ? far - 64 : 0;
    int last = INT32_MIN, done = 0;
    unsigned long long t_last = __builtin_amdgcn_s_memrealtime();
    int *level_word = &ctl->level;
    auto lines = [&](const char *base, long long bytes) {
        if (bytes <= 0) return;
        const uintptr_t a = (uintptr_t)base & ~(uintptr_t)127;
        const int n = (int)(((uintptr_t)base + (uintptr_t)bytes - a + 127) >> 7);
        for (int t = slot * 64 + lane; t < n; t += nslot * 64) DG_DROP_LOAD((const char *)a + ((size_t)t << 7));
    };
    int polls = 0;
    for (int lp = lb; lp < le;) {
        if ((polls++ & 31) == 0 &&
            (__hip_atomic_load(&ctl->seq, __ATOMIC_ACQUIRE, __HIP_MEMORY_SCOPE_AGENT) != seq || __hip_atomic_load(&ctl->stop, __ATOMIC_RELAXED, __HIP_MEMORY_SCOPE_AGENT))) break;
        const int lv = __builtin_amdgcn_readfirstlane(__hip_atomic_load(level_word, __ATOMIC_RELAXED, __HIP_MEMORY_SCOPE_AGENT));
        const unsigned long long now = __builtin_amdgcn_s_memrealtime();
        if (lv != last) { last = lv; t_last = now; } else if (now - t_last > PF_IDLE_TICKS) break;
        if (lp <= lv + behind) lp = lv + behind + 1;
        if (lp >= le) break;
        if (lp - lv > ahead) { __builtin_amdgcn_s_sleep(48); continue; }
        const LevelDesc &d = descs[lp];
        const int k2 = __builtin_amdgcn_readfirstlane(d.k2), T = __builtin_amdgcn_readfirstlane(d.T);
        lines((const char *)(F.rowrec + d.b0), 16LL * k2);
        lines((const char *)(F.slots + d.slot_first), 512LL * d.nblocks);
        lines((const char *)(F.in_edge + d.in_base), 4LL * T);
        if (d.rowx_stride > 0) lines((const char *)(F.rowx + d.rowx_off), 4LL * k2 * d.rowx_stride);
        if (delta_resident && d.delta_off >= 0 && (long long)T * T <= (128 << 10)) lines((const char *)(F.delta + d.delta_off), 2LL * T * T);
        ++lp; ++done;
    }
    if (lane == 0 && blockIdx.x == 0) atomicAdd(&ctl->levels_done, done);
#undef DG_DROP_LOAD
}

enum : unsigned { RC_COOP = 1, RC_PART = 2, RC_ALL = 4, RC_ANY = 7 };
constexpr struct SweepRc { int rc; unsigned is; } SWEEP_RCS[] = {
    {1, RC_COOP | RC_PART}, {2, RC_COOP | RC_PART}, {3, RC_COOP | RC_PART}, {4, RC_COOP | RC_PART}, {5, RC_PART}, {6, RC_PART},
    {8, RC_PART | RC_ALL}, {10, RC_PART}, {11, RC_PART}, {16, RC_PART}, {19, RC_ALL}, {33, RC_ALL}};
constexpr int N_SWEEP_RCS = (int)(sizeof SWEEP_RCS / sizeof SWEEP_RCS[0]);
constexpr bool sweep_rcs_ascend(int q = 1) { return q >= N_SWEEP_RCS || (SWEEP_RCS[q - 1].rc < SWEEP_RCS[q].rc && sweep_rcs_ascend(q + 1)); }
static_assert(SWEEP_RCS[0].rc >= 1 && sweep_rcs_ascend() && (SWEEP_RCS[N_SWEEP_RCS - 1].is & RC_ALL), "ascending (choose_rc's ties go to the larger RC), and the largest chunk is an all-planes one");

int SweepVariant::count() { return 1 + 4 * N_SWEEP_RCS; }
SweepVariant SweepVariant::at(int index) { return index == 0 ? SweepVariant{0, false, false} : SweepVariant{SWEEP_RCS[(index - 1) / 4].rc, ((index - 1) & 2) != 0, ((index - 1) & 1) != 0}; }
int SweepVariant::index() const {
    for (int q = 0; q < N_SWEEP_RCS; ++q) if (SWEEP_RCS[q].rc == rc) return 1 + 4 * q + (general ? 2 : 0) + (coop ? 1 : 0);
    return 0;
}
bool SweepVariant::exists() const {
    if (rc == 0) return !general && !coop;
    for (const SweepRc &e : SWEEP_RCS) if (e.rc == rc) return !coop || (e.is & RC_COOP);
    return false;
}
std::string SweepVariant::name() const {
    return rc == 0 ? "dp_sweep_kernel" : std::string("dp_sweep_") + (coop ? "coop" : "fast") + "_kernel<" + std::to_string(rc) + (general ? ",general>" : ",lean>");
}

template <unsigned WANT, int Q = 0, class F>
static bool launch_variant(int rc, bool digest, bool general, F &f) {
    if constexpr (Q < N_SWEEP_RCS) {
        if constexpr ((SWEEP_RCS[Q].is & WANT) != 0) if (rc == SWEEP_RCS[Q].rc) {
            constexpr std::integral_constant<int, SWEEP_RCS[Q].rc> RC{};
            if (digest) { if (general) f(RC, std::true_type{}, std::true_type{}); else f(RC, std::true_type{}, std::false_type{}); }
            else { if (general) f(RC, std::false_type{}, std::true_type{}); else f(RC, std::false_type{}, std::false_type{}); }
            return true;
        }
        return launch_variant<WANT, Q + 1>(rc, digest, general, f);
    }
    return false;
}

void sweep_prepare(const DpState &S, SweepLaunch &X) {
    for (const SweepRc &e : SWEEP_RCS) if ((e.is & RC_ALL) && (X.rc_sel = e.rc) >= S.RP) break;
    X.digest = S.opt.want_digest != 0; X.rp_active = S.RP;
    X.small_state = S.state_alloc_bytes < ((size_t)1 << 31);
    SweepArgs &A = X.A;
    A.descs = S.d_descs.as<LevelDesc>(); A.in_off = S.d_in_off.as<uint32_t>(); A.in_edge = S.d_in_edge.as<uint32_t>();
    A.grp_begin = S.d_grp.as<uint32_t>(); A.in_dst = S.d_in_dst.as<int32_t>(); A.dead_cols = S.d_dead.as<int32_t>();
    A.delta = A.delta_zero = S.d_delta.as<uint16_t>();
    A.ring = S.d_ring.as<char>(); A.slot_bytes = S.state_alloc_bytes; A.pad_bytes = 4 * (size_t)S.pad_front;
    A.bp = nullptr; A.digest = S.d_digest.as<unsigned long long>(); A.RP = S.RP;
    FastArgs &F = X.F;
    F.rowrec = S.d_rowrec.as<uint4>(); F.slots = S.d_slots.as<uint2>(); F.in_edge = A.in_edge; F.rowx = S.d_rowx.as<uint32_t>(); F.dead_cols = A.dead_cols;
    F.delta = F.delta_zero = A.delta; F.bp = nullptr; F.digest = A.digest; F.RP = S.RP;
    F.ring = S.d_ring.as<char>(); F.slot_bytes = (uint32_t)S.state_alloc_bytes;
#ifdef DG_SWEEP_PROBE
    F.probe = S.d_probe.as<unsigned long long>();
#endif
    F.progress = A.progress = &S.d_pfctl.as<PfCtl>()->level;
    F.pad_bytes = (int)(4 * S.pad_front);
    F.buf_bytes = (uint32_t)std::min<size_t>(S.state_alloc_bytes, 0x7FFFFFFFu);
}

void sweep_init_state(const DpState &S, hipStream_t s) {
    hipLaunchKernelGGL(dp_init_kernel, dim3((unsigned)((S.RP + 255) / 256)), dim3(256), 0, s, S.d_ring.as<int32_t>() + S.pad_front, S.RP);
}

static void choose_rc(const DpState &S, const SweepLaunch &X, const LevelDesc &d, int l, int &rc, bool &coop) {
    const int rc_sel = rc = X.rc_sel;
    coop = false;
    if (S.opt.adaptive_rc == 0) return;
    const bool coop_ok = S.opt.use_coop && d.n_heavy > 0 && d.k2 + 4 * d.n_heavy <= 65535;
    const double dmax = (double)std::max(1, S.level_dmax[l]);
    double best = 1e300;
    for (int pass = (coop_ok && S.opt.use_coop == 2) ? 1 : 0; pass < (coop_ok ? 2 : 1); ++pass) {
        for (const SweepRc &e : SWEEP_RCS) {
            if (e.rc != rc_sel && !((e.is & RC_PART) && e.rc < rc_sel)) continue;
            if (pass == 1 && !(e.is & RC_COOP)) continue;
            if (S.opt.test_force_rc && e.rc != S.opt.test_force_rc) continue;
            const double rows = pass ? (double)d.k2 + 4.0 * d.n_heavy : (double)d.k2;
            const double chain = pass ? std::max((double)COOP_MIN, std::ceil(dmax / 4.0)) + 1.0 : dmax;
            const double W = rows * d.nblocks * ((X.rp_active + e.rc - 1) / e.rc);
            const double T = std::max(1.0, W / (double)S.opt.rc_cap) * ((double)S.opt.rc_t0_ns + chain * e.rc * (double)S.opt.rc_tg_ps * 1e-3) + W * (double)S.opt.rc_tw_ps * 1e-3;
            if (T <= best) { best = T; rc = e.rc; coop = pass == 1; }
        }
    }
}

int sweep_launch_level(const DpState &S, SweepLaunch &X, int l, hipStream_t s) {
    LevelDesc d = S.descs[l];
    d.bp_nt = (int64_t)d.k2 * d.k2 * S.RP >= S.opt.bp_nt_min_cells ? 1 : 0;
    SweepVariant v{0, false, false};
    bool launched;
    if (d.fast_ok && X.small_state && S.RP <= 65535 && S.opt.use_fast) {
        choose_rc(S, X, d, l, v.rc, v.coop);
        v.general = d.fast_ok == 2;
        const int nch = (X.rp_active + v.rc - 1) / v.rc;
        const dim3 grid((unsigned)((d.nblocks + 3) / 4), (unsigned)nch, (unsigned)(d.k2 + (v.coop ? 4 * d.n_heavy : 0)));
        const dim3 pgrid((unsigned)((d.nblocks + DG_PLAIN_GW - 1) / DG_PLAIN_GW), (unsigned)((nch + DG_PLAIN_CH - 1) / DG_PLAIN_CH), grid.z);
        const int32_t *hv = S.d_heavy.as<int32_t>();
        const FastArgs &F = X.F;
        const uint4 *rowrec_l = F.rowrec + d.b0;
        const uint2 *slots_l = F.slots + d.slot_first;
        const uint32_t *rowx_l = F.rowx + d.rowx_off;
        const int32_t *cur = (const int32_t *)(F.ring + (size_t)DG_SLOT(l - 1) * F.slot_bytes);
        const int dT = d.delta_off >= 0 ? d.T : 0;
        const uint16_t *dm = dT ? F.delta + d.delta_off - (int64_t)d.in_base * dT : F.delta_zero;
        const int rp_k = S.RP | (d.k << 13);
        unsigned long long hlo = 0, hhi = 0;
        for (int q = 0; q < 4; ++q) { hlo |= (unsigned long long)(uint16_t)d.heavy_in[q] << (16 * q); hhi |= (unsigned long long)(uint16_t)d.heavy_in[4 + q] << (16 * q); }
        auto fast = [&](auto RC, auto DG, auto GEN) { hipLaunchKernelGGL((dp_sweep_fast_kernel<RC.value, DG.value, GEN.value>), pgrid, dim3(DG_PLAIN_WG), 0, s, rowrec_l, slots_l, rowx_l, cur, dm, d.rowx_stride, d.nblocks, rp_k, F.pad_bytes, dT, F.buf_bytes, F, d, l); };
        auto cooperative = [&](auto RC, auto DG, auto GEN) { hipLaunchKernelGGL((dp_sweep_coop_kernel<RC.value, DG.value, GEN.value>), grid, dim3(256), 0, s, rowrec_l, slots_l, rowx_l, cur, d.rowx_stride, d.nblocks, d.n_heavy, rp_k, hlo, hhi, F, d, l, dm, dT, hv); };
        launched = v.coop ? launch_variant<RC_COOP>(v.rc, X.digest, v.general, cooperative) : launch_variant<RC_ANY>(v.rc, X.digest, v.general, fast);
    } else {
        const int nchunk = (S.RP + X.rc_sel - 1) / X.rc_sel;
        const int64_t ntask = (int64_t)d.k2 * d.ngroups * nchunk;
        const unsigned grid = (unsigned)std::min<int64_t>((ntask + 3) / 4, S.opt.max_blocks);
        const SweepArgs &A = X.A;
        auto generic = [&](auto RC, auto DG, auto) { hipLaunchKernelGGL((dp_sweep_kernel<RC.value, DG.value>), dim3(grid), dim3(256), 0, s, A, l); };
        launched = launch_variant<RC_ALL>(X.rc_sel, X.digest, false, generic);
    }
    if (!launched) { set_error("sweep of level %d: no %s kernel is instantiated for chunks of %d recombination counts", l, v.coop ? "cooperative" : v.rc ? "fast" : "generic", v.rc ? v.rc : X.rc_sel); return DG_ERR_STATE; }
    X.hist.n[(size_t)v.index()]++;
    return DG_OK;
}

void sweep_warm_tables(const DpState &S, const SweepLaunch &X, int q0, int q1, hipStream_t s) {
    const LevelDesc &da = S.descs[q0], &db = S.descs[q1 - 1];
    const FastArgs &F = X.F;
    WarmRanges W{};
    auto put = [&](int q, const void *base, int64_t b0, int64_t b1) {
        const uintptr_t a = ((uintptr_t)base + (uintptr_t)b0) & ~(uintptr_t)15, e = ((uintptr_t)base + (uintptr_t)b1) & ~(uintptr_t)15;
        W.p[q] = (const char *)a; W.n16[q] = e > a ? (long long)((e - a) >> 4) : 0;
    };
    put(0, F.rowrec, 16 * (int64_t)da.b0, 16 * ((int64_t)db.b0 + db.k2));
    put(1, F.slots, 8 * da.slot_first, 8 * (db.slot_first + (int64_t)db.nblocks * 64));
    put(2, F.in_edge, 4 * (int64_t)da.in_base, 4 * ((int64_t)db.in_base + db.T));
    int64_t d0 = -1, d1 = -1, x0 = -1, x1 = -1;
    for (int q = q0; q < q1; ++q) {
        const LevelDesc &dq = S.descs[q];
        if (dq.rowx_stride > 0) {
            if (x0 < 0) x0 = dq.rowx_off;
            x1 = dq.rowx_off + (int64_t)dq.k2 * dq.rowx_stride;
        }
        if (dq.delta_off < 0 || S.level_win[q] != S.cur_win) continue;
        const int64_t e = dq.delta_off + (int64_t)dq.T * dq.T;
        d0 = d0 < 0 ? dq.delta_off : std::min(d0, dq.delta_off);
        d1 = std::max(d1, e);
    }
    if (d0 >= 0) put(3, F.delta, 2 * d0, 2 * d1);
    if (x0 >= 0) put(4, F.rowx, 4 * x0, 4 * x1);
    long long tot = 0;
    for (int q = 0; q < WARM_RANGES; ++q) tot += W.n16[q];
    if (tot <= 0) return;
    const unsigned grid = (unsigned)std::min<long long>((tot + 255) / 256, 2048);
    hipLaunchKernelGGL(dp_warm_tables_kernel, dim3(grid), dim3(256), 0, s, W);
}

int sweep_prefetch_begin(DpState &S, const SweepLaunch &X, int lb, int le, bool delta_resident, hipStream_t s) {
    S.pf_active = false;
    if (S.opt.l2_prefetch <= 0 || !X.small_state || !S.opt.use_fast || le - lb < 64) return DG_OK;
    if (!S.pf_stream && hipStreamCreateWithFlags(&S.pf_stream, hipStreamNonBlocking) != hipSuccess) { (void)hipGetLastError(); S.pf_stream = nullptr; S.opt.l2_prefetch = 0; return DG_OK; }
    if (!S.pf_ev && hipEventCreateWithFlags(&S.pf_ev, hipEventDisableTiming) != hipSuccess) { (void)hipGetLastError(); S.pf_ev = nullptr; S.opt.l2_prefetch = 0; return DG_OK; }
    if (!S.side_stream_ok()) return DG_OK;
    if (!S.pf_tested) {
        S.pf_tested = 1;
        DG_HIP(hipStreamSynchronize(s));
        hipLaunchKernelGGL(dp_pf_probe_wait_kernel, dim3(1), dim3(1), 0, S.pf_stream, S.d_pfctl.as<PfCtl>(), 0x5EED);
        hipLaunchKernelGGL(dp_pf_probe_set_kernel, dim3(1), dim3(1), 0, s, S.d_pfctl.as<PfCtl>(), 0x5EED);
        PfCtl h;
        if (hipStreamSynchronize(S.pf_stream) != hipSuccess || hipStreamSynchronize(s) != hipSuccess ||
            hipMemcpy(&h, S.d_pfctl.p, sizeof h, hipMemcpyDeviceToHost) != hipSuccess || !h.probe_ok) {
            (void)hipGetLastError();
            if (getenv("DG_DEBUG")) fprintf(stderr, "[dipgenie_hip] L2 prefetcher off: its stream does not run beside the sweep's\n");
            S.opt.l2_prefetch = 0;
            return DG_OK;
        }
    }
    const int seq = ++S.pf_seq;
    hipLaunchKernelGGL(dp_pf_ctl_kernel, dim3(1), dim3(1), 0, s, S.d_pfctl.as<PfCtl>(), seq, lb - 1, 0);
    DG_HIP(hipEventRecord(S.pf_ev, s));
    DG_HIP(hipStreamWaitEvent(S.pf_stream, S.pf_ev, 0));
    const int far = (int)S.opt.pf_far;
    hipLaunchKernelGGL(dp_l2_prefetch_kernel, dim3(PF_WORKGROUPS + (far > 0 ? PF_FAR_WORKGROUPS : 0)), dim3(64), 0, S.pf_stream, S.d_descs.as<LevelDesc>(), X.F,
                       S.d_pfctl.as<PfCtl>(), seq, lb, le, (int)S.opt.l2_prefetch, delta_resident ? 1 : 0, far);
    S.pf_active = true;
    return DG_OK;
}
void sweep_prefetch_end(DpState &S, int le, hipStream_t s) {
    if (S.pf_stream && S.opt.l2_prefetch > 0) hipLaunchKernelGGL(dp_pf_ctl_kernel, dim3(1), dim3(1), 0, s, S.d_pfctl.as<PfCtl>(), S.pf_seq, le, 1);
}
void sweep_prefetch_free(DpState &S) {
    if (S.pf_stream) { (void)hipStreamSynchronize(S.pf_stream); (void)hipStreamDestroy(S.pf_stream); S.pf_stream = nullptr; }
    if (S.pf_ev) { (void)hipEventDestroy(S.pf_ev); S.pf_ev = nullptr; }
}

}
```

### dipgenie_amd/csrc/dg_dp_tables.hip

```cpp
#include <algorithm>
#include <cstdlib>
#include <cstring>

#include "dg_dp.hpp"

namespace dgi {

namespace {

constexpr int64_t ROWX_MAX_LEVEL_CELLS = (int64_t)1 << 21;
constexpr int64_t ROWX_BUDGET_WORDS = (int64_t)1 << 30;

struct Part {
    std::vector<int32_t> dtrans, dead_cols, heavy;
    std::vector<uint32_t> grp_begin, slots, rowx;
    std::vector<int64_t> dblk_first;
    int64_t cells = 0, units = 0, max_level_cells = 0, max_level_units = 0, delta_entries = 0, nblk = 0;
    uint64_t edge_pairs = 0, colour_entries = 0;
};

struct Builder {
    const dg_dp_graph *g;
    DpState &S;
    int nV, L, NT;
    int64_t E = 0;
    int max_k = 0;
    std::vector<int> lcut;
    std::vector<std::string> terr;
    std::vector<int> trc;
    std::vector<int32_t> level_of;
    std::vector<uint32_t> in_off, in_edge;
    std::vector<int32_t> in_dst;
    std::vector<uint8_t> has_col;
    std::vector<uint32_t> rowrec;
    std::vector<int32_t> dtrans, dead_cols, heavy_rows;
    std::vector<uint32_t> grp_begin, slots, rowx;
    std::vector<int64_t> dblk_first;

    Builder(const dg_dp_graph *g_, DpState &S_) : g(g_), S(S_), nV(g_->n_vertices), L(g_->n_levels) {
        NT = (int)std::max<int64_t>(1, std::min<int64_t>({(int64_t)S.opt.host_threads, (int64_t)std::thread::hardware_concurrency(), (int64_t)L / 64 + 1}));
        lcut.assign(NT + 1, L);
        lcut[0] = 0;
        for (int t = 1; t < NT; ++t) {
            const int32_t want = (int32_t)((int64_t)nV * t / NT);
            lcut[t] = (int)(std::upper_bound(g->level_off, g->level_off + L + 1, want) - g->level_off) - 1;
            lcut[t] = std::min(std::max(lcut[t], lcut[t - 1]), L);
        }
        terr.resize(NT);
        trc.assign(NT, DG_OK);
    }
    template <class F> void run_threads(F &&fn) {
        std::vector<std::thread> th;
        for (int t = 1; t < NT; ++t) th.emplace_back([&fn, t] { fn(t); });
        fn(0);
        for (auto &x : th) x.join();
    }
    template <class... A> void tfail(int t, int rc, const char *fmt, A... a) {
        if (trc[t] != DG_OK) return;
        char buf[256];
        snprintf(buf, sizeof buf, fmt, a...);
        terr[t] = buf; trc[t] = rc;
    }
    int first_error() {
        for (int t = 0; t < NT; ++t) if (trc[t] != DG_OK) { set_error("%s", terr[t].c_str()); return trc[t]; }
        return DG_OK;
    }
    int range_v0(int t) const { return g->level_off[lcut[t]]; }
    int range_v1(int t) const { return lcut[t + 1] < L ? g->level_off[lcut[t + 1]] : nV; }

    int validate_and_index();
    int build_in_csr();
    int check_colours();
    int build_level_tables();
};

int Builder::validate_and_index() {
    for (int l = 0; l < L; ++l)
        if (g->level_off[l + 1] <= g->level_off[l]) { set_error("level %d is empty", l); return DG_ERR_ARG; }
    level_of.resize(nV);
    std::vector<int> tmax_k(NT, 0);
    run_threads([&](int t) {
        for (int l = lcut[t]; l < lcut[t + 1]; ++l) {
            tmax_k[t] = std::max(tmax_k[t], g->level_off[l + 1] - g->level_off[l]);
            for (int v = g->level_off[l]; v < g->level_off[l + 1]; ++v) level_of[v] = l;
        }
    });
    for (int t = 0; t < NT; ++t) max_k = std::max(max_k, tmax_k[t]);
    if (max_k > MAX_K) { set_error("level width %d exceeds the supported %d", max_k, MAX_K); return DG_ERR_UNSUPPORTED; }
    if (g->out_off[0] != 0) { set_error("out_off must start at 0"); return DG_ERR_ARG; }
    for (int t = 1; t <= NT; ++t) {
        const int v = lcut[t] < L ? g->level_off[lcut[t]] : nV;
        if (g->out_off[v] < 0) { set_error("out_off negative at %d", v); return DG_ERR_ARG; }
    }
    E = g->out_off[nV];
    if (E < 0 || E >= (int64_t)1 << 31) { set_error("unsupported number of edges (%lld)", (long long)E); return DG_ERR_UNSUPPORTED; }
    return DG_OK;
}

int Builder::build_in_csr() {
    in_off.assign((size_t)nV + 1, 0);
    in_edge.resize((size_t)E);
    in_dst.resize((size_t)E);
    run_threads([&](int t) {
        for (int u = range_v0(t); u < range_v1(t); ++u) {
            if (g->out_off[u + 1] < g->out_off[u] || g->out_off[u + 1] > E) { tfail(t, DG_ERR_ARG, "out_off not monotone at %d", u); return; }
            for (int64_t e = g->out_off[u]; e < g->out_off[u + 1]; ++e) {
                const int v = g->out_dst[e];
                if (v < 0 || v >= nV || level_of[v] != level_of[u] + 1) { tfail(t, DG_ERR_ARG, "edge %d->%d does not go to the next level", u, v); return; }
                if (g->out_w[e] > 1) { tfail(t, DG_ERR_ARG, "edge weight %d > 1", (int)g->out_w[e]); return; }
                in_off[v + 1]++;
            }
        }
    });
    if (int rc = first_error()) return rc;
    for (int v = 0; v < nV; ++v) in_off[v + 1] += in_off[v];
    run_threads([&](int t) {
        const int da = g->level_off[std::min(lcut[t] + 1, L)], db = g->level_off[std::min(lcut[t + 1] + 1, L)];
        std::vector<uint32_t> fill(in_off.begin() + da, in_off.begin() + db);
        for (int u = range_v0(t); u < range_v1(t); ++u) {
            const uint32_t pos = (uint32_t)(u - g->level_off[level_of[u]]);
            for (int64_t e = g->out_off[u]; e < g->out_off[u + 1]; ++e) {
                const int v = g->out_dst[e];
                const uint32_t slot = fill[v - da]++;
                in_edge[slot] = pos | ((uint32_t)g->out_w[e] << 31);
                in_dst[slot] = v;
            }
        }
        for (int v = da; v < db; ++v)
            for (uint32_t e = in_off[v] + 1; e < in_off[v + 1]; ++e)
                if ((in_edge[e] & 0x7FFFFFFFu) == (in_edge[e - 1] & 0x7FFFFFFFu) && in_edge[e] != in_edge[e - 1]) {
                    tfail(t, DG_ERR_UNSUPPORTED, "parallel edges with different weights into vertex %d: tie order would be schedule dependent", v);
                    return;
                }
    });
    return first_error();
}

int Builder::check_colours() {
    if (g->hom_off[0] != 0 || g->het_off[0] != 0) { set_error("colour offsets must start at 0"); return DG_ERR_ARG; }
    std::vector<int64_t> tmax_list(2 * (size_t)NT, 0);
    has_col.assign(L, 0);
    run_threads([&](int t) {
        for (int v = range_v0(t); v < range_v1(t); ++v) {
            for (int pass = 0; pass < 2; ++pass) {
                const int64_t *off = pass ? g->het_off : g->hom_off;
                const int32_t *colv = pass ? g->het_col : g->hom_col;
                if (off[v + 1] < off[v]) { tfail(t, DG_ERR_ARG, "colour offsets not monotone at %d", v); return; }
                tmax_list[2 * t + pass] = std::max(tmax_list[2 * t + pass], off[v + 1] - off[v]);
                if (off[v + 1] > off[v]) has_col[level_of[v]] = 1;
                for (int64_t q = off[v] + 1; q < off[v + 1]; ++q)
                    if (colv[q] <= colv[q - 1]) { tfail(t, DG_ERR_ARG, "colour list of vertex %d is not sorted-unique", v); return; }
            }
        }
    });
    if (int rc = first_error()) return rc;
    int64_t max_hom = 0, max_het = 0;
    for (int t = 0; t < NT; ++t) { max_hom = std::max(max_hom, tmax_list[2 * t]); max_het = std::max(max_het, tmax_list[2 * t + 1]); }
    if (!colour_lists_fit_delta(max_hom, max_het)) {
        set_error("colour lists too long for uint16 score deltas (longest hom list %lld, longest het list %lld: 2 hom + 4 het must not exceed 65535)", (long long)max_hom, (long long)max_het);
        return DG_ERR_UNSUPPORTED;
    }
    return DG_OK;
}

int Builder::build_level_tables() {
    S.descs.assign(L, LevelDesc{});
    S.cells = S.relaxations = S.edge_pairs = S.colour_entries = 0;
    S.total_units = 0; S.max_level_units = 0; S.max_level_cells = S.RP; S.delta_entries = DELTA_PAD;
    S.level_units.assign(L, 0);
    S.level_dmax.assign(L, 0);
    rowrec.assign((size_t)nV * 4, 0);
    std::vector<Part> part(NT);
    run_threads([&](int t) {
        Part &P = part[t];
        for (int v = range_v0(t); v < range_v1(t); ++v) {
            const uint32_t e0 = in_off[v], dv = in_off[v + 1] - e0;
            rowrec[4 * (size_t)v] = e0; rowrec[4 * (size_t)v + 1] = dv;
            const int a0v = g->level_off[std::max(0, level_of[v] - 1)];
            for (uint32_t q = 0; q < 2; ++q) {
                uint32_t word = 0;
                if (dv > q) {
                    word = in_edge[e0 + q];
                    const int src = a0v + (int)(word & 0x7FFFu);
                    if (in_off[src + 1] - in_off[src] == 1) word |= 1u << 16;
                }
                rowrec[4 * (size_t)v + 2 + q] = word;
            }
        }
        auto &gb = P.grp_begin; auto &dead = P.dead_cols; auto &slots_p = P.slots;
        for (int l = std::max(1, lcut[t]); l < lcut[t + 1]; ++l) {
            LevelDesc &d = S.descs[l];
            d.a0 = g->level_off[l - 1]; d.k = g->level_off[l] - d.a0;
            d.b0 = g->level_off[l]; d.k2 = g->level_off[l + 1] - d.b0;
            d.in_base = in_off[d.b0];
            d.T = (int32_t)(in_off[d.b0 + d.k2] - d.in_base);
            auto indeg = [&](int c) { return in_off[d.b0 + c + 1] - in_off[d.b0 + c]; };
            d.grp_first = (int32_t)gb.size();
            d.dead_first = (int32_t)dead.size();
            d.heavy_first = (int32_t)P.heavy.size();
            uint32_t max_indeg = 0;
            for (int c = 0; c < d.k2; ++c) {
                max_indeg = std::max(max_indeg, indeg(c));
                if (indeg(c) > (uint32_t)COOP_MIN) P.heavy.push_back(c);
            }
            d.n_heavy = (int32_t)P.heavy.size() - d.heavy_first;
            for (int q = 0; q < HEAVY_INLINE; ++q) d.heavy_in[q] = q < d.n_heavy ? (int16_t)P.heavy[(size_t)d.heavy_first + q] : (int16_t)-1;
            S.level_dmax[l] = (int32_t)max_indeg;
            d.dmax = (int32_t)max_indeg;
            {
                uint32_t cur_size = 0;
                for (int c = 0; c < d.k2; ++c) {
                    const uint32_t e0 = in_off[d.b0 + c], dv = indeg(c);
                    if (dv == 0) { dead.push_back(c); continue; }
                    if (cur_size == 0 || cur_size + dv > 64 || dv > 64) { gb.push_back(e0); cur_size = 0; }
                    cur_size += dv;
                    if (dv > 64) cur_size = 65;
                }
            }
            d.ngroups = (int32_t)gb.size() - d.grp_first;
            gb.push_back(d.in_base + (uint32_t)d.T);
            d.slot_first = (int64_t)(slots_p.size() / 2);
            d.fast_ok = (d.T < (1 << 20)) ? 1 : 0;
            d.bp_wide = max_indeg > (uint32_t)BP_MAX_RANK ? 1 : 0;
            if (d.bp_wide) d.fast_ok = 0;
            int32_t n_blocks = 0;
            for (int gi = 0; gi < d.ngroups; ++gi) {
                const uint32_t gb0 = gb[d.grp_first + gi], ge0 = gb[d.grp_first + gi + 1];
                const bool giant = ge0 - gb0 > 64;
                if (giant && d.fast_ok) d.fast_ok = 2;
                uint32_t maxdv = 1;
                if (!giant)
                    for (uint32_t e = gb0; e < ge0;) {
                        const uint32_t dv = indeg(in_dst[e] - d.b0);
                        maxdv = std::max(maxdv, dv);
                        e += dv;
                    }
                uint32_t steps = 0;
                while ((1u << steps) < std::min(maxdv, 64u)) ++steps;
                const uint32_t nb = giant ? (ge0 - gb0 + 63) / 64 : 1;
                const size_t s0 = slots_p.size();
                slots_p.resize(s0 + (size_t)nb * 128);
                uint32_t *sp = slots_p.data() + s0;
                for (uint32_t bq = 0; bq < nb; ++bq) {
                    const uint32_t tag = giant ? (bq == 0 ? 15u : 14u) : steps;
                    for (uint32_t q = 0; q < 64; ++q, sp += 2) {
                        const uint32_t e = gb0 + bq * 64 + q;
                        if (e < ge0) {
                            const uint32_t pv = in_edge[e];
                            sp[0] = (pv & 0x7FFFu) | ((pv >> 31) << 15) | ((uint32_t)(in_dst[e] - d.b0) << 16);
                            sp[1] = (e - d.in_base) | ((e - in_off[in_dst[e]]) << 20) | (tag << 28);
                        } else {
                            sp[0] = 0xFFFFFFFFu;
                            sp[1] = tag << 28;
                        }
                    }
                }
                n_blocks += (int32_t)nb;
            }
            if (n_blocks == 0) {
                for (int q = 0; q < 64; ++q) { slots_p.push_back(0xFFFFFFFFu); slots_p.push_back(0); }
                n_blocks = 1;
            }
            d.nblocks = n_blocks;
            d.ndead = (int32_t)dead.size() - d.dead_first;
            if (d.ngroups == 0) { d.ngroups = 1; gb.push_back(d.in_base + (uint32_t)d.T); }
            const int64_t ncell = (int64_t)d.k2 * d.k2 * S.RP;
            d.rowx_off = (int64_t)P.rowx.size();
            d.rowx_stride = 0;
            if (S.opt.use_rowx && d.fast_ok == 1 && max_indeg > 2 && max_indeg <= (uint32_t)ROWX_MAX && ncell <= ROWX_MAX_LEVEL_CELLS) {
                d.rowx_stride = (int32_t)max_indeg;
                P.rowx.resize(P.rowx.size() + (size_t)d.k2 * max_indeg, 0u);
                uint32_t *rx = P.rowx.data() + d.rowx_off;
                for (int c = 0; c < d.k2; ++c)
                    for (uint32_t q = 0; q < indeg(c); ++q) rx[(size_t)c * max_indeg + q] = in_edge[in_off[d.b0 + c] + q];
            }
            const int64_t units = ((d.bp_wide ? 2 * ncell : ncell) + 1) & ~(int64_t)1;
            S.level_units[l] = units;
            d.bp_off = P.units;
            P.units += units;
            P.cells += ncell;
            P.max_level_cells = std::max(P.max_level_cells, ncell);
            P.max_level_units = std::max(P.max_level_units, units);
            P.edge_pairs += (uint64_t)d.T * (uint64_t)d.T;
            if (has_col[l - 1] || has_col[l]) {
                d.delta_off = P.delta_entries;
                P.delta_entries += (int64_t)d.T * d.T;
                P.dtrans.push_back(l);
                P.dblk_first.push_back(P.nblk);
                P.nblk += ((int64_t)d.T * d.T + DELTA_PER_BLOCK - 1) / DELTA_PER_BLOCK;
                int64_t f = 0;
                for (uint32_t e = d.in_base; e < d.in_base + (uint32_t)d.T; ++e) {
                    const int sv = d.a0 + (int)(in_edge[e] & 0x7FFFFFFFu), tv = in_dst[e];
                    f += (g->hom_off[sv + 1] - g->hom_off[sv]) + (g->het_off[sv + 1] - g->het_off[sv]) +
                         (g->hom_off[tv + 1] - g->hom_off[tv]) + (g->het_off[tv + 1] - g->het_off[tv]);
                }
                P.colour_entries += (uint64_t)(2 * (int64_t)d.T * f);
            } else {
                d.delta_off = -1;
            }
        }
    });
    std::vector<int64_t> b_grp(NT + 1, 0), b_dead(NT + 1, 0), b_slot(NT + 1, 0), b_cells(NT + 1, 0), b_units(NT + 1, 0), b_delta(NT + 1, DELTA_PAD),
        b_blk(NT + 1, 0), b_dt(NT + 1, 0), b_heavy(NT + 1, 0), b_rowx(NT + 1, 0);
    for (int t = 0; t < NT; ++t) {
        const Part &P = part[t];
        b_grp[t + 1] = b_grp[t] + (int64_t)P.grp_begin.size();
        b_dead[t + 1] = b_dead[t] + (int64_t)P.dead_cols.size();
        b_slot[t + 1] = b_slot[t] + (int64_t)P.slots.size() / 2;
        b_cells[t + 1] = b_cells[t] + P.cells;
        b_units[t + 1] = b_units[t] + P.units;
        b_delta[t + 1] = b_delta[t] + P.delta_entries;
        b_blk[t + 1] = b_blk[t] + P.nblk;
        b_dt[t + 1] = b_dt[t] + (int64_t)P.dtrans.size();
        b_heavy[t + 1] = b_heavy[t] + (int64_t)P.heavy.size();
        b_rowx[t + 1] = b_rowx[t] + (int64_t)P.rowx.size();
        S.max_level_cells = std::max(S.max_level_cells, P.max_level_cells);
        S.max_level_units = std::max(S.max_level_units, P.max_level_units);
        S.edge_pairs += P.edge_pairs;
        S.colour_entries += P.colour_entries;
    }
    S.total_units = b_units[NT];
    {
        int kmax = 1;
        bool wide = false;
        for (int l = 1; l < L; ++l) { kmax = std::max(kmax, S.descs[l].k2); wide |= S.descs[l].bp_wide != 0; }
        S.lean_chain = S.opt.use_lean_chain && !wide && S.max_level_cells < ((int64_t)1 << 30) && (int64_t)S.RP * kmax < ((int64_t)1 << 24) && nV < (1 << 27);
    }
    S.cells = (uint64_t)b_cells[NT];
    S.delta_entries = b_delta[NT];
    S.n_delta_blocks = b_blk[NT];
    S.relaxations = S.edge_pairs * (uint64_t)S.RP;
    if (b_grp[NT] >= (int64_t)1 << 31 || b_dead[NT] >= (int64_t)1 << 31) { set_error("group tables too large"); return DG_ERR_UNSUPPORTED; }
    if (S.n_delta_blocks >= (int64_t)1 << 31) { set_error("delta grid too large"); return DG_ERR_UNSUPPORTED; }
    const int64_t rowx_words = std::min(b_rowx[NT], ROWX_BUDGET_WORDS);
    dtrans.resize((size_t)b_dt[NT]); dead_cols.resize((size_t)b_dead[NT]); heavy_rows.resize((size_t)b_heavy[NT] + 1);
    grp_begin.resize((size_t)b_grp[NT]);
    slots.resize((size_t)b_slot[NT] * 2);
    rowx.assign((size_t)rowx_words + 4, 0u);
    dblk_first.resize((size_t)b_dt[NT]);
    run_threads([&](int t) {
        Part &P = part[t];
        for (int l = std::max(1, lcut[t]); l < lcut[t + 1]; ++l) {
            LevelDesc &d = S.descs[l];
            d.grp_first += (int32_t)b_grp[t];
            d.dead_first += (int32_t)b_dead[t];
            d.heavy_first += (int32_t)b_heavy[t];
            d.slot_first += b_slot[t];
            d.bp_off += b_units[t];
            if (d.delta_off >= 0) d.delta_off += b_delta[t];
            d.rowx_off += b_rowx[t];
            if (d.rowx_stride > 0 && d.rowx_off + (int64_t)d.k2 * d.rowx_stride > rowx_words) d.rowx_stride = 0;
        }
        std::copy(P.grp_begin.begin(), P.grp_begin.end(), grp_begin.begin() + b_grp[t]);
        std::copy(P.dead_cols.begin(), P.dead_cols.end(), dead_cols.begin() + b_dead[t]);
        std::copy(P.heavy.begin(), P.heavy.end(), heavy_rows.begin() + b_heavy[t]);
        std::copy(P.slots.begin(), P.slots.end(), slots.begin() + 2 * b_slot[t]);
        std::copy(P.dtrans.begin(), P.dtrans.end(), dtrans.begin() + b_dt[t]);
        if (b_rowx[t] < rowx_words)
            std::copy(P.rowx.begin(), P.rowx.begin() + std::min<int64_t>((int64_t)P.rowx.size(), rowx_words - b_rowx[t]), rowx.begin() + b_rowx[t]);
        for (size_t q = 0; q < P.dblk_first.size(); ++q) dblk_first[(size_t)b_dt[t] + q] = P.dblk_first[q] + b_blk[t];
        std::vector<uint32_t>().swap(P.slots); std::vector<uint32_t>().swap(P.rowx);
    });
    return DG_OK;
}

void plan_delta_windows(DpState &S, const std::vector<int32_t> &dtrans, const std::vector<int64_t> &dblk_first) {
    S.dtrans_host = dtrans;
    S.dblk_first_host = dblk_first;
    S.dblk_first_host.push_back(S.n_delta_blocks);
    S.dwin_t.assign(1, 0);
    S.level_win.assign(S.L, -1);
    int64_t acc = 0, max_win = 0;
    for (size_t t = 0; t < dtrans.size(); ++t) {
        const int64_t n = (int64_t)S.descs[dtrans[t]].T * S.descs[dtrans[t]].T;
        if (acc > 0 && acc + n > S.opt.delta_cap_entries) { S.dwin_t.push_back((int32_t)t); max_win = std::max(max_win, acc); acc = 0; }
        acc += n;
        S.level_win[dtrans[t]] = (int32_t)S.dwin_t.size() - 1;
    }
    max_win = std::max(max_win, acc);
    S.dwin_t.push_back((int32_t)dtrans.size());
    S.delta_buf_entries = DELTA_PAD + max_win;
}

int plan_lattice(dg_ctx *c, DpState &S, size_t st_bytes, size_t dl_bytes, size_t table_bytes, size_t &bp_bytes, size_t &ck_bytes, bool dbg) {
    const int L = S.L;
    size_t free_b = 0, total_b = 0;
    DG_HIP(hipMemGetInfo(&free_b, &total_b));
    size_t pool_bytes;
    { std::unique_lock<std::mutex> lk(S.pool.mu); pool_bytes = S.pool.chunks.size() * S.pool.chunk_units * 2; }
    const size_t have = free_b + pool_bytes + S.d_bp.bytes + S.d_delta.bytes + S.d_ring.bytes + S.d_ckpt.bytes;
    const size_t fixed = st_bytes + dl_bytes + table_bytes + ((size_t)2 << 30);
    if (fixed > have) {
        set_error("graph needs %.1f GB of HBM for state/delta/tables but only %.1f GB is free", fixed / 1e9, have / 1e9);
        return DG_ERR_OOM;
    }
    size_t chunk_units = (size_t)S.opt.chunk_units_cfg;
    if (S.opt.segment_cells > 0) chunk_units = std::min(chunk_units, ((size_t)S.opt.segment_cells + 1) & ~(size_t)1);
    if ((size_t)S.max_level_units > chunk_units) chunk_units = (size_t)S.max_level_units;
    S.chunk_begin.assign(1, 1);
    {
        size_t acc = 0;
        for (int l = 1; l < L; ++l) {
            const size_t nu = (size_t)S.level_units[l];
            if (acc > 0 && acc + nu > chunk_units) { S.chunk_begin.push_back(l); acc = 0; }
            acc += nu;
        }
        S.chunk_begin.push_back(L);
    }
    const size_t n_chunks = S.chunk_begin.size() - 1;
    const bool tiny = n_chunks == 1 && S.total_units < S.opt.chunk_units_cfg / 8 && S.opt.segment_cells == 0;
    const size_t chunk_bytes = chunk_units * 2;
    const size_t resident_bytes = tiny ? (size_t)S.total_units * 2 : n_chunks * chunk_bytes;
    const bool segmented = (resident_bytes + fixed > have || S.opt.segment_cells > 0) && n_chunks > 1;
    if (!segmented && resident_bytes + fixed > have) {
        set_error("back-pointer lattice of %.1f GB (one level alone needs %.1f GB) does not fit the %.1f GB of free HBM", resident_bytes / 1e9,
                  S.max_level_units * 2 / 1e9, (have - fixed) / 1e9);
        return DG_ERR_OOM;
    }
    size_t group = n_chunks;
    S.seg_begin.assign(1, 1);
    S.ckpt_off.assign(1, 0);
    int64_t ckpt_cells = 0;
    if (segmented) {
        group = S.opt.segment_cells > 0 ? 1 : std::max<size_t>(1, std::min(n_chunks - 1, (have - fixed) / chunk_bytes));
        if (S.opt.segment_cells == 0) group = std::min(group, std::max<size_t>(8, pool_bytes / chunk_bytes + 2));
        for (;; --group) {
            S.seg_begin.assign(1, 1);
            S.ckpt_off.assign(1, 0);
            ckpt_cells = 0;
            for (size_t cb = group; cb < n_chunks; cb += group) {
                const int l = S.chunk_begin[cb];
                S.seg_begin.push_back(l);
                S.ckpt_off.push_back(ckpt_cells);
                ckpt_cells += (int64_t)S.descs[l].k * S.descs[l].k * S.RP;
            }
            if (group * chunk_bytes + (size_t)ckpt_cells * 4 + fixed <= have || group == 1) break;
        }
        if (group * chunk_bytes + (size_t)ckpt_cells * 4 + fixed > have) {
            set_error("segmented lattice needs %.1f GB (+%.1f GB checkpoints) but only %.1f GB of HBM is free", group * chunk_bytes / 1e9,
                      ckpt_cells * 4 / 1e9, (have - fixed) / 1e9);
            return DG_ERR_OOM;
        }
        if (dbg)
            fprintf(stderr, "[dipgenie_hip] lattice %.1f GB does not fit: %zu segments of <= %zu chunks of %.1f GB, checkpoints %.2f GB\n",
                    S.total_units * 2 / 1e9, S.seg_begin.size(), group, chunk_bytes / 1e9, ckpt_cells * 4 / 1e9);
    }
    S.seg_begin.push_back(L);
    S.seg_chunks = (int)group;
    bp_bytes = tiny ? resident_bytes : group * chunk_bytes;
    ck_bytes = (size_t)ckpt_cells * 4;
    S.d_bp.release();
    if (tiny) {
        pool_clear(S);
        if (int rc = S.d_bp.ensure((size_t)S.total_units * 2)) return rc;
    } else {
        if (chunk_units != S.pool.chunk_units) { pool_clear(S); S.pool.chunk_units = chunk_units; pool_bytes = 0; }
        const size_t mapped = pool_bytes / chunk_bytes;
        if (mapped > group && free_b < fixed + ck_bytes) pool_trim(S, group);
        pool_request(S, c->device, group);
        if (dbg) fprintf(stderr, "[dipgenie_hip] lattice: %zu chunks of %.1f GB (%zu resident at a time), %zu mapped so far\n", n_chunks, chunk_bytes / 1e9, group, mapped);
    }
    return DG_OK;
}

int upload(DevBuf &b, const void *src, size_t bytes, hipStream_t s) {
    if (int rc = b.ensure(bytes)) return rc;
    if (bytes) DG_HIP(hipMemcpyAsync(b.p, src, bytes, hipMemcpyHostToDevice, s));
    return DG_OK;
}

}

int dp_load(dg_ctx *c, const dg_dp_graph *g) {
    const bool dbg = getenv("DG_DEBUG") != nullptr;
    double tl0 = wall_s();
    auto lap = [&](const char *what) { if (dbg) { double t = wall_s(); fprintf(stderr, "[dipgenie_hip] load: %-22s %.3f s\n", what, t - tl0); tl0 = t; } };
    if (!g || !g->level_off || !g->out_off || !g->out_dst || !g->out_w || !g->hom_off || !g->het_off) {
        set_error("dg_dp_load_graph: null array"); return DG_ERR_ARG;
    }
    const int nV = g->n_vertices, L = g->n_levels, R = g->R;
    if (nV < 2 || L < 2 || R < 0 || R > 4096) { set_error("dg_dp_load_graph: bad sizes (V=%d L=%d R=%d)", nV, L, R); return DG_ERR_ARG; }
    if (g->level_off[0] != 0 || g->level_off[L] != nV) { set_error("level_off must span [0, n_vertices]"); return DG_ERR_ARG; }
    if (g->level_off[1] != 1) { set_error("level 0 must hold exactly the source vertex"); return DG_ERR_ARG; }
    if (!c->dp) c->dp = new DpState(c->device);
    DpState &S = *c->dp;
    graphs_clear(S);
    S.loaded = false;
    S.ob_dict = false;
    S.nV = nV; S.L = L; S.R = R; S.RP = R + 1;
    hipStream_t s = c->stream;
    PoolPause pause(S);
    std::vector<int32_t> dtrans;
    std::vector<int64_t> dblk_first;
    int max_k = 1;
    if (!S.opt.host_tables) {
        if (int rc = dp_build_tables_device(c, g, S, dtrans, dblk_first, max_k)) return rc;
    } else {
        Builder B(g, S);
        if (int rc = B.validate_and_index()) return rc;
        if (int rc = B.build_in_csr()) return rc;
        lap("validate + in-CSR");
        if (int rc = B.check_colours()) return rc;
        lap("colour checks");
        if (int rc = B.build_level_tables()) return rc;
        lap("descs + groups + slots");
        if (int rc = upload(S.d_descs, S.descs.data(), sizeof(LevelDesc) * L, s)) return rc;
        if (int rc = upload(S.d_in_off, B.in_off.data(), 4 * B.in_off.size(), s)) return rc;
        if (int rc = upload(S.d_in_edge, B.in_edge.data(), 4 * B.in_edge.size(), s)) return rc;
        if (int rc = upload(S.d_in_dst, B.in_dst.data(), 4 * B.in_dst.size(), s)) return rc;
        if (int rc = upload(S.d_hom_off, g->hom_off, 8 * ((size_t)nV + 1), s)) return rc;
        if (int rc = upload(S.d_het_off, g->het_off, 8 * ((size_t)nV + 1), s)) return rc;
        if (int rc = upload(S.d_hom_col, g->hom_col, 4 * (size_t)g->hom_off[nV], s)) return rc;
        if (int rc = upload(S.d_het_col, g->het_col, 4 * (size_t)g->het_off[nV], s)) return rc;
        if (int rc = upload(S.d_dtrans, B.dtrans.data(), 4 * B.dtrans.size(), s)) return rc;
        if (int rc = upload(S.d_dblk_first, B.dblk_first.data(), 8 * B.dblk_first.size(), s)) return rc;
        if (int rc = upload(S.d_grp, B.grp_begin.data(), 4 * B.grp_begin.size(), s)) return rc;
        if (int rc = upload(S.d_dead, B.dead_cols.data(), 4 * B.dead_cols.size(), s)) return rc;
        if (int rc = upload(S.d_heavy, B.heavy_rows.data(), 4 * B.heavy_rows.size(), s)) return rc;
        if (int rc = upload(S.d_rowrec, B.rowrec.data(), 4 * B.rowrec.size(), s)) return rc;
        if (int rc = upload(S.d_rowx, B.rowx.data(), 4 * B.rowx.size(), s)) return rc;
        if (int rc = upload(S.d_slots, B.slots.data(), 4 * B.slots.size(), s)) return rc;
        DG_HIP(hipStreamSynchronize(s));
        S.n_grp = (int64_t)B.grp_begin.size(); S.n_dead = (int64_t)B.dead_cols.size(); S.n_heavy_rows = (int64_t)B.heavy_rows.size() - 1;
        S.n_slot_records = (int64_t)B.slots.size() / 2; S.n_rowx_words = (int64_t)B.rowx.size() - 4;
        dtrans.swap(B.dtrans); dblk_first.swap(B.dblk_first);
        max_k = B.max_k;
        lap("table uploads");
    }
    S.n_dtrans = (int64_t)dtrans.size();
    S.n_edges = g->out_off[nV];
    plan_delta_windows(S, dtrans, dblk_first);
    const size_t n_edges = (size_t)g->out_off[nV];
    const size_t st_bytes = (size_t)S.max_level_cells * 4 * 2, dl_bytes = (size_t)S.delta_buf_entries * 2;
    size_t bp_bytes = 0, ck_bytes = 0;
    if (int rc = plan_lattice(c, S, st_bytes, dl_bytes, 3 * n_edges + 16 * (size_t)L + (1 << 20), bp_bytes, ck_bytes, dbg)) return rc;
    lap("plan lattice");
    if (int rc = S.d_eflag.ensure(n_edges + 16)) return rc;
    if (int rc = S.d_eself.ensure(2 * n_edges + 16)) return rc;
    delta_launch_edge_flags(S, s);
    if (int rc = S.d_delta.ensure(dl_bytes)) return rc;
    DG_HIP(hipMemsetAsync(S.d_delta.p, 0, 2 * DELTA_PAD, s));
    if (int rc = S.d_ckpt.ensure(ck_bytes)) return rc;
    if (int rc = S.d_pfctl.ensure(256)) return rc;
    DG_HIP(hipMemsetAsync(S.d_pfctl.p, 0, 256, s));
    S.pad_front = 2 * (int64_t)max_k;
    const size_t pad_bytes = 4 * (size_t)(S.pad_front + 33 * (int64_t)max_k);
    S.state_alloc_bytes = (((size_t)S.max_level_cells * 4 + pad_bytes) + 255) & ~(size_t)255;
    if (int rc = S.d_ring.ensure(S.state_alloc_bytes * 2)) return rc;
    DG_HIP(hipMemsetAsync(S.d_ring.p, 0, S.state_alloc_bytes * 2, s));
    if (int rc = S.d_digest.ensure(8 * (size_t)L)) return rc;
#ifdef DG_SWEEP_PROBE
    if (int rc = S.d_probe.ensure(64 * (size_t)L)) return rc;
#endif
    if (int rc = S.d_sink.ensure(4 * (size_t)S.RP)) return rc;
    S.sink_host.clear();
    S.cap = 2 * (R + 8);
    if (int rc = budgets_reserve(S, 1)) return rc;
    lap("allocs");
    for (auto &e : S.ev) if (!e) DG_HIP(hipEventCreate(&e));
    memset(&S.timing, 0, sizeof S.timing);
    S.timing.edge_pairs = S.edge_pairs;
    S.timing.colour_entries = S.colour_entries;
    S.timing.state_bytes = st_bytes; S.timing.bp_bytes = bp_bytes; S.timing.delta_bytes = dl_bytes;
    S.loaded = true;
    return DG_OK;
}

int dp_table_digest(dg_ctx *c, uint64_t *out, int n) {
    DpState *Sp = c->dp;
    if (!Sp || !Sp->loaded) { set_error("dg_dp_get_table_digest: no graph loaded"); return DG_ERR_STATE; }
    if (!out || n < 12) { set_error("dg_dp_get_table_digest: need 12 words"); return DG_ERR_ARG; }
    DpState &S = *Sp;
    DG_HIP(hipStreamSynchronize(c->stream));
    std::vector<unsigned char> h;
    auto fnv = [&](const DevBuf &b, size_t bytes, uint64_t &dst) -> int {
        h.resize(bytes);
        if (bytes) DG_HIP(hipMemcpy(h.data(), b.p, bytes, hipMemcpyDeviceToHost));
        uint64_t x = 1469598103934665603ULL;
        for (size_t i = 0; i < bytes; ++i) { x ^= h[i]; x *= 1099511628211ULL; }
        dst = x;
        return DG_OK;
    };
    if (int rc = fnv(S.d_descs, sizeof(LevelDesc) * (size_t)S.L, out[0])) return rc;
    if (int rc = fnv(S.d_in_off, 4 * ((size_t)S.nV + 1), out[1])) return rc;
    if (int rc = fnv(S.d_in_edge, 4 * (size_t)S.n_edges, out[2])) return rc;
    if (int rc = fnv(S.d_in_dst, 4 * (size_t)S.n_edges, out[3])) return rc;
    if (int rc = fnv(S.d_dtrans, 4 * (size_t)S.n_dtrans, out[4])) return rc;
    if (int rc = fnv(S.d_dblk_first, 8 * (size_t)S.n_dtrans, out[5])) return rc;
    if (int rc = fnv(S.d_grp, 4 * (size_t)S.n_grp, out[6])) return rc;
    if (int rc = fnv(S.d_dead, 4 * (size_t)S.n_dead, out[7])) return rc;
    if (int rc = fnv(S.d_heavy, 4 * (size_t)S.n_heavy_rows, out[8])) return rc;
    if (int rc = fnv(S.d_rowrec, 16 * (size_t)S.nV, out[9])) return rc;
    if (int rc = fnv(S.d_rowx, 4 * (size_t)S.n_rowx_words, out[10])) return rc;
    if (int rc = fnv(S.d_slots, 8 * (size_t)S.n_slot_records, out[11])) return rc;
    return DG_OK;
}

}
```

### include/dipgenie_hip.h

```cpp
#ifndef DIPGENIE_HIP_H
#define DIPGENIE_HIP_H
#include <stdint.h>
#ifdef __cplusplus
extern "C" {
#endif

#define DG_OK              0
#define DG_ERR_ARG        -1
#define DG_ERR_NO_DEVICE  -2
#define DG_ERR_HIP        -3
#define DG_ERR_OOM        -4
#define DG_ERR_UNSUPPORTED -5
#define DG_ERR_STATE      -6

typedef struct dg_ctx dg_ctx;

dg_ctx     *dg_create(int device);
void        dg_destroy(dg_ctx *);
const char *dg_last_error(void);
int         dg_set_stream(dg_ctx *, void *hip_stream);
int         dg_synchronize(dg_ctx *);
int         dg_device_info(dg_ctx *, char *name, int name_cap, int *n_cu, int64_t *hbm_bytes);
int         dg_hip_versions(int *compiled, int *runtime);

typedef struct dg_dp_graph {
    int32_t n_vertices, n_levels, R;
    const int32_t *level_off;
    const int64_t *out_off;
    const int32_t *out_dst;
    const uint8_t *out_w;
    const int64_t *hom_off, *het_off;
    const int32_t *hom_col, *het_col;
} dg_dp_graph;

typedef struct dg_dp_result {
    int32_t value, s_het, n_p1, n_p2;
    int32_t *p1_from, *p1_to, *p2_from, *p2_to;
    int32_t cap;
    uint64_t cells, relaxations;
} dg_dp_result;

typedef struct dg_dp_timing {
    float delta_ms;
    float forward_ms;
    float traceback_ms;
    float total_ms;
    int64_t n_forward_launches;
    uint64_t edge_pairs;
    uint64_t colour_entries;
    uint64_t state_bytes, bp_bytes, delta_bytes;
    int32_t n_segments;
    int32_t n_chunks;
} dg_dp_timing;

int dg_dp_prealloc(dg_ctx *, int64_t bytes);
int dg_dp_load_graph(dg_ctx *, const dg_dp_graph *);
int dg_dp_run(dg_ctx *, dg_dp_result *);
int dg_dp_get_timing(dg_ctx *, dg_dp_timing *);
int dg_dp_solve_diploid(dg_ctx *, const dg_dp_graph *, dg_dp_result *);
int dg_dp_run_budgets(dg_ctx *, const int32_t *budgets, int32_t n_budgets, dg_dp_result *results);
int dg_dp_get_budget_values(dg_ctx *, int32_t *out, int32_t n);
typedef struct dg_dp_pair_score {
    int32_t value;
    int32_t s_het;
    int32_t r1, r2;
} dg_dp_pair_score;
int dg_dp_score_paths(dg_ctx *, const int32_t *paths, int64_t n_pairs, dg_dp_pair_score *out);
typedef struct dg_dp_partner {
    int32_t value;
    int32_t s_het;
    int32_t r1, r2;
} dg_dp_partner;
int dg_dp_best_partners(dg_ctx *, const int32_t *given, int64_t n, const int32_t *budgets, int32_t *partners, dg_dp_partner *out);
typedef struct dg_dp_level_margin {
    int32_t best_vertex, best_value;
    int32_t second_vertex, second_value;
} dg_dp_level_margin;
int dg_dp_partner_marginals(dg_ctx *, const int32_t *given, int64_t n, const int32_t *budgets, dg_dp_level_margin *levels, int32_t *vertex_values);
int dg_dp_get_answer_paths(dg_ctx *, int32_t budget, int32_t *paths);
typedef struct dg_dp_call_margin {
    int32_t vertex, value;
    int32_t alt_vertex, alt_value;
} dg_dp_call_margin;
int dg_dp_call_margins(dg_ctx *, int32_t budget, const int32_t *vertex_class, dg_dp_call_margin *levels, int32_t *paths);
int dg_dp_get_partner_route(dg_ctx *, int32_t *route, int64_t *cells);
typedef struct dg_dp_pair_objective {
    int32_t hom_shared, hom_single;
    int32_t het_single, het_both;
} dg_dp_pair_objective;
int dg_dp_objective_paths(dg_ctx *, const int32_t *paths, int64_t n_pairs, dg_dp_pair_objective *out);
int dg_dp_answer_objectives(dg_ctx *, const int32_t *budgets, int32_t n_budgets, dg_dp_pair_objective *out);
int dg_dp_get_level_digest(dg_ctx *, uint64_t *out, int64_t n);
int dg_dp_set_option(dg_ctx *, const char *key, int64_t value);
int dg_dp_get_option(dg_ctx *, const char *key, int64_t *value);
int dg_dp_get_table_digest(dg_ctx *, uint64_t *out, int n);
int dg_dp_get_launch_profile(dg_ctx *, char *buf, int cap);
int dg_dp_list_sweep_variants(char *buf, int cap);

typedef struct dg_hap_graph {
    int32_t n_vertices, R;
    const int64_t *out_off;
    const int32_t *out_dst;
    const uint8_t *out_w;
    const int32_t *n_colours;
} dg_hap_graph;
int dg_dp_solve_haploid(dg_ctx *, const dg_hap_graph *, int32_t *dp, int32_t *back_vtx, int32_t *back_r);

int dg_sketch_reads(dg_ctx *, const char *bases, const int64_t *read_off, int64_t n_reads, int k, int w,
                    uint64_t **hash, int32_t **n_reads_with_hash, int64_t *n_distinct);
int dg_sketch_haplotype(dg_ctx *, const char *seq, int64_t len, int k, int w,
                        uint64_t **hash, int64_t **pos, int64_t *n);
int dg_hash_kmers(dg_ctx *, const char *kmers, int64_t n, int k, uint64_t *out);
void dg_free(void *);

typedef struct dg_sketch_timing { float kernel_ms, sort_ms, total_ms; int64_t n_emitted; } dg_sketch_timing;
int dg_sketch_get_timing(dg_ctx *, dg_sketch_timing *);
int dg_sketch_set_option(dg_ctx *, const char *name, int64_t value);
int dg_sketch_get_option(dg_ctx *, const char *name, int64_t *value);
int dg_sketch_get_stat(dg_ctx *, const char *name, int64_t *value);

int dg_sketch_reads_dev(dg_ctx *, const char *bases_dev, const int64_t *read_off_dev, int64_t n_reads,
                        int64_t n_bases, int k, int w, uint64_t *hash_dev, int32_t *count_dev, int64_t cap,
                        int64_t *n_distinct);
int dg_sketch_count_dictionary_dev(dg_ctx *, const uint64_t *dict_dev, int64_t n_dict,
                                   const uint64_t *hash_dev, const int32_t *count_dev, int64_t n,
                                   int32_t *counts_dev);
int dg_sketch_merge_runs_dev(dg_ctx *, const uint64_t *hash_dev, const int32_t *count_dev, int64_t n_total,
                             uint64_t *out_hash_dev, int32_t *out_count_dev, int64_t cap, int64_t *n_out);

int dg_sketch_partition_dev(dg_ctx *, const uint64_t *hash_dev, int64_t n, int world, int64_t *split_dev);
int dg_sketch_rank_dictionary_dev(dg_ctx *, const uint64_t *dict_dev, int64_t n_dict, const uint64_t *hash_dev, int64_t n,
                                  int64_t base, int64_t *rank1_dev);
int dg_sketch_count_rank_dictionary_dev(dg_ctx *, const uint64_t *dict_dev, int64_t n_dict, const uint64_t *hash_dev,
                                        const int32_t *count_dev, int64_t n, int64_t base, int32_t *counts_dev, int64_t *rank1_dev);
int dg_sketch_histogram_dev(dg_ctx *, const int32_t *count_dev, int64_t n, int n_bins, uint64_t *hist_dev);

typedef struct dg_shard dg_shard;
dg_shard *dg_shard_create(int n_ranks, const int *devices, int transport);
void      dg_shard_destroy(dg_shard *);
int       dg_shard_n_ranks(dg_shard *);
dg_ctx   *dg_shard_ctx(dg_shard *, int rank);
int       dg_shard_score_reads(dg_shard *, const char *bases, const int64_t *read_off, int64_t n_reads, int k, int w,
                               const uint64_t *hap_hash, int64_t n_hap_hash, uint64_t **sp_hash, int32_t **sp_count, int64_t *n_sp,
                               int64_t *hist, int n_bins, int64_t *n_dict, int64_t *dict_hits, double *ms_sketch_max, double *ms_exchange_max);

int dg_anchor_begin(dg_ctx *, int32_t n_haps, int32_t n_vertices, const int32_t *top_order_map ,
                    int k, int w);
int dg_anchor_add_haplotype(dg_ctx *, int32_t h, const char *seq, int64_t len, const int32_t *step_vtx, const int64_t *step_start,
                            int64_t n_steps, int64_t *n_minimizers);
int dg_anchor_add_haplotype_sketched(dg_ctx *, int32_t h, int64_t len, const uint64_t *hash, const int64_t *pos, int64_t n,
                                     const int32_t *step_vtx, const int64_t *step_start, int64_t n_steps);
typedef struct dg_anchor_result {
    int64_t n_occ, n_vtx;
    int32_t *occ_id, *occ_hap;
    uint32_t *occ_off, *occ_len;
    int32_t *vpool;
    int64_t n_candidates;
    int64_t n_unstable_groups;
} dg_anchor_result;
int dg_anchor_finish(dg_ctx *, const uint64_t *sp_hash, int64_t n_sp, float min_shared, dg_anchor_result *out);

#ifdef __cplusplus
}
#endif
#endif
```

Measured before the change: 59.64 billion.

## Fuse adjacent DP levels into paired sweep kernel with composed transition tables

Adds a pair-level path that processes two consecutive DP levels in one kernel launch. It uses precomputed composed in-edge tables (prow/pslots) for levels whose composed in-degree, width and transition size stay within small bounds. Ring-buffer parity is tracked with a flip bit, and graph capture records flips and launch counts so replay stays consistent. The aim is to cut the launch count and the write and read of intermediate states between the two levels. In exchange it adds host-side table building, a larger front pad, and extra prefetch logic, and it may redo work when composed in-degree grows.

```diff
diff --git a/dipgenie_amd/capi.py b/dipgenie_amd/capi.py
--- a/dipgenie_amd/capi.py
+++ b/dipgenie_amd/capi.py
@@ -70,7 +70,7 @@
     "dg_shard_create", "dg_shard_destroy", "dg_shard_n_ranks", "dg_shard_ctx", "dg_shard_score_reads",
     "dg_dp_run_budgets", "dg_dp_get_budget_values", "dg_dp_score_paths", "dg_dp_best_partners", "dg_dp_partner_marginals",
     "dg_dp_get_option", "dg_sketch_get_option", "dg_dp_list_sweep_variants", "dg_dp_get_answer_paths", "dg_dp_call_margins",
-    "dg_dp_objective_paths", "dg_dp_answer_objectives", "dg_dp_get_partner_route",
+    "dg_dp_objective_paths", "dg_dp_answer_objectives", "dg_dp_get_partner_route", "dg_dp_get_pair_profile", "dg_dp_list_pair_variants",
 ]
 
 lib.dg_create.restype = C.c_void_p
@@ -101,6 +101,8 @@
 lib.dg_dp_get_option.argtypes = [C.c_void_p, C.c_char_p, C.POINTER(C.c_int64)]
 lib.dg_dp_get_launch_profile.argtypes = [C.c_void_p, C.c_char_p, C.c_int]
 lib.dg_dp_list_sweep_variants.argtypes = [C.c_char_p, C.c_int]
+lib.dg_dp_get_pair_profile.argtypes = [C.c_void_p, C.c_char_p, C.c_int]
+lib.dg_dp_list_pair_variants.argtypes = [C.c_char_p, C.c_int]
 lib.dg_dp_get_table_digest.argtypes = [C.c_void_p, C.c_void_p, C.c_int]
 lib.dg_sketch_reads.argtypes = [C.c_void_p, C.c_char_p, C.c_void_p, C.c_int64, C.c_int, C.c_int,
                                 C.POINTER(C.c_void_p), C.POINTER(C.c_void_p), C.POINTER(C.c_int64)]
@@ -417,6 +419,17 @@
         _check(lib.dg_dp_get_launch_profile(self.h, buf, 8192), "dg_dp_get_launch_profile")
         return {k: int(v) for k, v in (item.rsplit(":", 1) for item in buf.value.decode().split())}
 
+    def dp_pair_profile(self):
+        buf = C.create_string_buffer(1024)
+        _check(lib.dg_dp_get_pair_profile(self.h, buf, 1024), "dg_dp_get_pair_profile")
+        return {k: int(v) for k, v in (item.rsplit(":", 1) for item in buf.value.decode().split())}
+
+    @staticmethod
+    def dp_pair_variants():
+        buf = C.create_string_buffer(1024)
+        _check(lib.dg_dp_list_pair_variants(buf, 1024), "dg_dp_list_pair_variants")
+        return buf.value.decode().split()
+
     @staticmethod
     def dp_sweep_variants():
         buf = C.create_string_buffer(8192)
diff --git a/dipgenie_amd/csrc/dg_dp.hpp b/dipgenie_amd/csrc/dg_dp.hpp
--- a/dipgenie_amd/csrc/dg_dp.hpp
+++ b/dipgenie_amd/csrc/dg_dp.hpp
@@ -62,6 +62,7 @@
     unsigned long long *digest;
     int RP;
     int *progress;
+    int flip;
 };
 
 struct FastArgs {
@@ -77,6 +78,7 @@
     uint32_t buf_bytes;
     uint32_t slot_bytes;
     int *progress;
+    int flip;
 #ifdef DG_SWEEP_PROBE
     unsigned long long *probe;
 #endif
@@ -93,6 +95,23 @@
     static int count();
     static SweepVariant at(int index);
 };
+constexpr int PAIR_MAX_INDEG = 8;
+constexpr int PAIR_MAX_WIDTH = 255;
+constexpr int PAIR_MAX_T = 2047;
+constexpr int PAIR_RCS[] = {1, 2, 4};
+constexpr int N_PAIR_RCS = (int)(sizeof PAIR_RCS / sizeof PAIR_RCS[0]);
+struct PairDesc {
+    int32_t l, nblocks;
+    int32_t k0, k1, k2;
+    int32_t dmax;
+    int64_t row_first;
+    int64_t slot_first;
+};
+struct PairHist {
+    int64_t n[N_PAIR_RCS] = {};
+    void add(const PairHist &o, int64_t sign = 1) { for (int q = 0; q < N_PAIR_RCS; ++q) n[q] += sign * o.n[q]; }
+};
+
 struct SweepHist {
     std::vector<int64_t> n = std::vector<int64_t>((size_t)SweepVariant::count(), 0);
     void add(const SweepHist &o, int64_t sign = 1) { for (size_t q = 0; q < n.size(); ++q) n[q] += sign * o.n[q]; }
@@ -126,6 +145,8 @@
     int64_t score_slab_bytes = (int64_t)256 << 20;
     int64_t partner_slab_bytes = (int64_t)4 << 30;
     int64_t partner_wide = 0;
+    int64_t pair_levels = 1;
+    int64_t pair_min = 4096;
     int64_t objective_lds_bytes = 131072;
 };
 
@@ -152,7 +173,7 @@
     std::vector<int64_t> ckpt_off;
     bool graph_failed = false;
     typedef std::tuple<int, int, const void *, int> GraphKey;
-    struct Batch { hipGraphExec_t exec = nullptr; SweepHist hist; };
+    struct Batch { hipGraphExec_t exec = nullptr; SweepHist hist; PairHist pair_hist; int64_t n_launch = 0; int flips = 0; };
     std::map<GraphKey, Batch> graphs;
     bool all_fast = false;
     size_t state_alloc_bytes = 0;
@@ -169,6 +190,10 @@
     std::vector<int32_t> level_dmax;
     int64_t n_grp = 0, n_dead = 0, n_heavy_rows = 0, n_slot_records = 0, n_rowx_words = 0, n_dtrans = 0, n_edges = 0;
     DevBuf d_descs, d_in_off, d_in_edge, d_in_dst, d_hom_off, d_het_off, d_hom_col, d_het_col, d_eflag, d_eself;
+    std::vector<PairDesc> pairs;
+    std::vector<int32_t> pair_at;
+    DevBuf d_pairs, d_pair_at, d_prow, d_pslots;
+    PairHist pair_hist;
     DevBuf d_delta, d_bp, d_ring, d_digest, d_dblk_first, d_dtrans, d_grp, d_dead, d_heavy, d_rowrec, d_rowx, d_slots, d_ckpt, d_pfctl;
 #ifdef DG_SWEEP_PROBE
     DevBuf d_probe;
@@ -227,6 +252,7 @@
 int dp_load(dg_ctx *c, const dg_dp_graph *g);
 int dp_build_tables_device(dg_ctx *c, const dg_dp_graph *g, DpState &S, std::vector<int32_t> &dtrans, std::vector<int64_t> &dblk_first, int &max_k);
 int dp_table_digest(dg_ctx *c, uint64_t *out, int n);
+int dp_build_pairs(dg_ctx *c, const dg_dp_graph *g, DpState &S);
 
 void delta_launch_edge_flags(const DpState &S, hipStream_t s);
 const uint16_t *delta_launch_window(DpState &S, int w, hipStream_t s);
@@ -241,10 +267,15 @@
     bool digest = false;
     int rp_active = 0;
     SweepHist hist;
+    PairHist pair_hist;
+    bool pairs_ok = false;
+    int flip = 0;
 };
 void sweep_prepare(const DpState &S, SweepLaunch &X);
 void sweep_init_state(const DpState &S, hipStream_t s);
 int sweep_launch_level(const DpState &S, SweepLaunch &X, int l, hipStream_t s);
+int sweep_launch_pair(const DpState &S, SweepLaunch &X, int l, hipStream_t s);
+std::string pair_variant_name(int q);
 void sweep_warm_tables(const DpState &S, const SweepLaunch &X, int q0, int q1, hipStream_t s);
 int sweep_prefetch_begin(DpState &S, const SweepLaunch &X, int lb, int le, bool delta_resident, hipStream_t s);
 void sweep_prefetch_end(DpState &S, int le, hipStream_t s);
diff --git a/dipgenie_amd/csrc/dg_dp_pairs.hip b/dipgenie_amd/csrc/dg_dp_pairs.hip
--- /dev/null
+++ b/dipgenie_amd/csrc/dg_dp_pairs.hip
@@ -0,0 +1,104 @@
+#include <algorithm>
+#include <cstdlib>
+
+#include "dg_dp.hpp"
+
+namespace dgi {
+
+int dp_build_pairs(dg_ctx *c, const dg_dp_graph *g, DpState &S) {
+    S.pairs.clear(); S.pair_at.clear();
+    S.d_pairs.release(); S.d_pair_at.release(); S.d_prow.release(); S.d_pslots.release();
+    const int L = S.L, nV = S.nV;
+    if (!S.opt.pair_levels || (int64_t)(L - 1) / 2 < std::max<int64_t>(S.opt.pair_min, 1) || (int)S.dwin_t.size() != 2 || S.RP > 0x1FFF) return DG_OK;
+    const double t0 = wall_s();
+    std::vector<uint32_t> in_off((size_t)nV + 1, 0), in_edge((size_t)g->out_off[nV]);
+    DG_HIP(hipMemcpyAsync(in_off.data(), S.d_in_off.p, 4 * in_off.size(), hipMemcpyDeviceToHost, c->stream));
+    if (!in_edge.empty()) DG_HIP(hipMemcpyAsync(in_edge.data(), S.d_in_edge.p, 4 * in_edge.size(), hipMemcpyDeviceToHost, c->stream));
+    DG_HIP(hipStreamSynchronize(c->stream));
+    auto indeg = [&](int v) { return (int)(in_off[v + 1] - in_off[v]); };
+    auto level_ok = [&](int l) {
+        const LevelDesc &d = S.descs[l];
+        return d.fast_ok == 1 && d.ndead == 0 && d.k2 <= PAIR_MAX_WIDTH && d.T <= PAIR_MAX_T && !d.bp_wide;
+    };
+    auto composed = [&](int v, int a0m) {
+        int n = 0;
+        for (uint32_t e = in_off[v]; e < in_off[v + 1]; ++e) n += indeg(a0m + (int)(in_edge[e] & 0x7FFFu));
+        return n;
+    };
+    std::vector<int32_t> at((size_t)L, -1);
+    std::vector<PairDesc> pairs;
+    for (int l = 2; l < L; ++l) {
+        if (!level_ok(l - 1) || !level_ok(l)) continue;
+        const LevelDesc &d = S.descs[l];
+        bool ok = true;
+        int dmax = 0;
+        for (int v = d.b0; v < d.b0 + d.k2 && ok; ++v) { const int n = composed(v, d.a0); dmax = std::max(dmax, n); ok = n >= 1 && n <= PAIR_MAX_INDEG; }
+        if (!ok) continue;
+        PairDesc p{};
+        p.l = l; p.k0 = S.descs[l - 1].k; p.k1 = d.k; p.k2 = d.k2; p.dmax = dmax;
+        at[l] = (int32_t)pairs.size(); at[l - 1] = -2;
+        pairs.push_back(p);
+        ++l;
+    }
+    if ((int64_t)pairs.size() < std::max<int64_t>(S.opt.pair_min, 1)) return DG_OK;
+    std::vector<uint32_t> prow, pslots;
+    std::vector<uint32_t> col;
+    for (PairDesc &p : pairs) {
+        const LevelDesc &d2 = S.descs[p.l], &d1 = S.descs[p.l - 1];
+        p.row_first = (int64_t)(prow.size() / 2);
+        p.slot_first = (int64_t)(pslots.size() / 4);
+        size_t blk0 = pslots.size();
+        uint32_t used = 0, maxdv = 1;
+        auto close_block = [&]() {
+            if (used == 0) return;
+            uint32_t steps = 0;
+            while ((1u << steps) < maxdv) ++steps;
+            for (uint32_t q = used; q < 64; ++q) { pslots.push_back(0xFFFFFFFFu); pslots.push_back(0); pslots.push_back(0); pslots.push_back(0); }
+            for (uint32_t q = 0; q < 64; ++q) pslots[blk0 + 4 * q + 2] |= steps << 16;
+            blk0 = pslots.size(); used = 0; maxdv = 1;
+        };
+        for (int c2 = 0; c2 < d2.k2; ++c2) {
+            const int v = d2.b0 + c2;
+            const uint32_t n = (uint32_t)composed(v, d2.a0);
+            uint32_t t = 0;
+            col.clear();
+            for (uint32_t e2 = in_off[v]; e2 < in_off[v + 1]; ++e2) {
+                const uint32_t m = in_edge[e2] & 0x7FFFu, w2 = in_edge[e2] >> 31, r2 = e2 - in_off[v];
+                const int mv = d2.a0 + (int)m;
+                for (uint32_t e1 = in_off[mv]; e1 < in_off[mv + 1]; ++e1, ++t) {
+                    const uint32_t src = in_edge[e1] & 0x7FFFu, w1 = in_edge[e1] >> 31, r1 = e1 - in_off[mv];
+                    const uint32_t i2 = e2 - d2.in_base, i1 = e1 - d1.in_base;
+                    prow.push_back(src | (w1 << 15) | (m << 16) | (w2 << 24) | (n << 25));
+                    prow.push_back(i2 | (i1 << 11) | (r2 << 22) | (r1 << 25));
+                    col.push_back(src | (w1 << 15) | (m << 16) | (w2 << 24));
+                    col.push_back(i2 | (i1 << 16));
+                    col.push_back(r2 | (r1 << 8) | ((uint32_t)c2 << 20));
+                    col.push_back(0);
+                }
+            }
+            for (; t < (uint32_t)PAIR_MAX_INDEG; ++t) { prow.push_back(n << 25); prow.push_back(0); }
+            if (used + n > 64) close_block();
+            pslots.insert(pslots.end(), col.begin(), col.end());
+            used += n; maxdv = std::max(maxdv, n);
+        }
+        close_block();
+        p.nblocks = (int32_t)((int64_t)(pslots.size() / 4) - p.slot_first) / 64;
+    }
+    auto up = [&](DevBuf &b, const void *src, size_t bytes) -> int {
+        if (int rc = b.ensure(bytes + 16)) return rc;
+        DG_HIP(hipMemcpyAsync(b.p, src, bytes, hipMemcpyHostToDevice, c->stream));
+        return DG_OK;
+    };
+    if (int rc = up(S.d_pairs, pairs.data(), sizeof(PairDesc) * pairs.size())) return rc;
+    if (int rc = up(S.d_pair_at, at.data(), 4 * at.size())) return rc;
+    if (int rc = up(S.d_prow, prow.data(), 4 * prow.size())) return rc;
+    if (int rc = up(S.d_pslots, pslots.data(), 4 * pslots.size())) return rc;
+    DG_HIP(hipStreamSynchronize(c->stream));
+    if (getenv("DG_DEBUG"))
+        fprintf(stderr, "[dipgenie_hip] load: %zu level pairs (%.1f %% of the launches), composed tables %.1f MB, built in %.3f s\n", pairs.size(),
+                100.0 * (double)pairs.size() / std::max(1, L - 1), 4e-6 * (double)(prow.size() + pslots.size()), wall_s() - t0);
+    S.pairs.swap(pairs); S.pair_at.swap(at);
+    return DG_OK;
+}
+
+}
diff --git a/dipgenie_amd/csrc/dg_dp_run.hip b/dipgenie_amd/csrc/dg_dp_run.hip
--- a/dipgenie_amd/csrc/dg_dp_run.hip
+++ b/dipgenie_amd/csrc/dg_dp_run.hip
@@ -91,7 +91,7 @@
 
     Run(dg_ctx *c_, DpState &S_) : c(c_), S(S_), s(c_->stream) { sweep_prepare(S, X); }
     int n_win() const { return (int)S.dwin_t.size() - 1; }
-    int32_t *state_ptr(int level) const { return (int32_t *)(S.d_ring.as<char>() + (size_t)(level & 1) * S.state_alloc_bytes) + S.pad_front; }
+    int32_t *state_ptr(int level) const { return (int32_t *)(S.d_ring.as<char>() + (size_t)((level & 1) ^ X.flip) * S.state_alloc_bytes) + S.pad_front; }
     size_t level_cells(int level) const {
         const int64_t k = level == 0 ? 1 : S.descs[level].k2;
         return (size_t)(k * k * S.RP);
@@ -106,7 +106,10 @@
                 if (q1 > q0) sweep_warm_tables(S, X, q0, q1, s);
             }
             if (l >= next_warm) next_warm = l + (int)std::max<int64_t>(S.opt.warm_ahead, 1);
-            if (int rc = sweep_launch_level(S, X, l, s)) return rc;
+            if (X.pairs_ok && l + 1 < l1 && S.pair_at[l + 1] >= 0) {
+                if (S.level_win[l + 1] >= 0 && S.level_win[l + 1] != S.cur_win) load_window(S.level_win[l + 1]);
+                if (int rc = sweep_launch_pair(S, X, ++l, s)) return rc;
+            } else if (int rc = sweep_launch_level(S, X, l, s)) return rc;
             ++n_launch;
             if (S.opt.sync_every > 0 && n_launch % S.opt.sync_every == 0) DG_HIP(hipStreamSynchronize(s));
         }
@@ -118,8 +121,8 @@
         next_warm = lb;
         if (int rc = sweep_prefetch_begin(S, X, lb, le, n_win() == 1, s)) return rc;
         const int64_t gb = S.opt.graph_batch >= 0 ? S.opt.graph_batch : 1000;
-        const int pf_key = ((S.pf_active && S.opt.pf_far > 0) ? 1 : 0) | (X.rp_active << 1);
         for (int l0 = lb; l0 < le;) {
+            const int pf_key = ((S.pf_active && S.opt.pf_far > 0) ? 1 : 0) | (X.flip << 1) | (X.rp_active << 2);
             const bool use_graph = gb > 0 && n_win() == 1 && S.opt.sync_every == 0 && !S.graph_failed;
             const int l1 = use_graph ? (int)std::min<int64_t>((int64_t)l0 + gb, le) : le;
             while (S.delta_piece_next < (int)S.delta_piece_level.size() && S.delta_piece_level[S.delta_piece_next] < l1) {
@@ -133,8 +136,8 @@
                 slot = &S.graphs[key];
                 if (slot->exec) {
                     DG_HIP(hipGraphLaunch(slot->exec, s));
-                    X.hist.add(slot->hist);
-                    n_launch += l1 - l0; l0 = l1;
+                    X.hist.add(slot->hist); X.pair_hist.add(slot->pair_hist);
+                    n_launch += slot->n_launch; X.flip ^= slot->flips; l0 = l1;
                     continue;
                 }
                 if (hipStreamBeginCapture(s, hipStreamCaptureModeThreadLocal) == hipSuccess) capturing = true;
@@ -142,6 +145,8 @@
             }
             const int64_t n_launch_before = n_launch;
             const SweepHist hist_before = X.hist;
+            const PairHist pair_hist_before = X.pair_hist;
+            const int flip_before = X.flip;
             if (int rc = issue_levels(l0, l1, lb, le)) {
                 if (capturing) {
                     hipGraph_t cg = nullptr;
@@ -158,11 +163,14 @@
                 if (cg) (void)hipGraphDestroy(cg);
                 if (!ok) {
                     (void)hipGetLastError();
-                    slot->exec = nullptr; S.graph_failed = true; n_launch = n_launch_before; X.hist = hist_before;
+                    slot->exec = nullptr; S.graph_failed = true; n_launch = n_launch_before; X.hist = hist_before; X.pair_hist = pair_hist_before; X.flip = flip_before;
                     continue;
                 }
                 slot->hist = X.hist;
                 slot->hist.add(hist_before, -1);
+                slot->pair_hist = X.pair_hist;
+                slot->pair_hist.add(pair_hist_before, -1);
+                slot->n_launch = n_launch - n_launch_before; slot->flips = X.flip ^ flip_before;
                 DG_HIP(hipGraphLaunch(slot->exec, s));
             }
             l0 = l1;
@@ -226,6 +234,8 @@
         }
 #endif
         sweep_init_state(S, s);
+        X.pairs_ok = !S.pairs.empty() && S.opt.pair_levels && n_seg == 1 && n_win() == 1 && !X.digest && S.opt.use_fast && S.opt.adaptive_rc && S.opt.test_force_rc == 0 &&
+                     X.small_state && X.rp_active == S.RP;
         if (n_seg == 1) {
             if (int rc = sweep_and_walk(0, S.d_bp.p ? 1 : n_chunks_all, true, true)) return rc;
         } else {
@@ -308,6 +318,7 @@
     S.sink_host.clear();
     const int rc_run = run.forward_and_trace();
     S.launch_hist = run.X.hist;
+    S.pair_hist = run.X.pair_hist;
     if (rc_run) return rc_run;
     DG_HIP(hipMemcpyAsync(to.data(), S.d_ch_trace.p, sizeof(TraceOut) * to.size(), hipMemcpyDeviceToHost, s));
     DG_HIP(hipMemcpyAsync(edges.data(), S.d_ch_edges.p, 4 * edges.size(), hipMemcpyDeviceToHost, s));
@@ -435,6 +446,22 @@
     memcpy(buf, out.c_str(), out.size() + 1);
     return DG_OK;
 }
+extern "C" int dg_dp_get_pair_profile(dg_ctx *c, char *buf, int cap) {
+    if (!c || !c->dp || !buf || cap < 2) { dgi::set_error("dg_dp_get_pair_profile: no state"); return DG_ERR_STATE; }
+    std::string out;
+    for (int q = 0; q < dgi::N_PAIR_RCS; ++q)
+        if (const int64_t n = c->dp->pair_hist.n[q]) out += (out.empty() ? "" : " ") + dgi::pair_variant_name(q) + ':' + std::to_string(n);
+    if ((int)out.size() + 1 > cap) { dgi::set_error("dg_dp_get_pair_profile: buffer too small (%zu needed)", out.size() + 1); return DG_ERR_ARG; }
+    memcpy(buf, out.c_str(), out.size() + 1);
+    return DG_OK;
+}
+extern "C" int dg_dp_list_pair_variants(char *buf, int cap) {
+    std::string out;
+    for (int q = 0; q < dgi::N_PAIR_RCS; ++q) out += (out.empty() ? "" : " ") + dgi::pair_variant_name(q);
+    if (!buf || (int)out.size() + 1 > cap) { dgi::set_error("dg_dp_list_pair_variants: buffer too small (%zu needed)", out.size() + 1); return DG_ERR_ARG; }
+    memcpy(buf, out.c_str(), out.size() + 1);
+    return DG_OK;
+}
 extern "C" int dg_dp_list_sweep_variants(char *buf, int cap) {
     std::string out;
     for (int q = 0; q < dgi::SweepVariant::count(); ++q)
@@ -455,6 +482,7 @@
     {"objective_lds_bytes", &DpO::objective_lds_bytes, 0, true},
     {"rowx", &DpO::use_rowx, 0, false}, {"lean_chain", &DpO::use_lean_chain, 0, false}, {"segment_cells", &DpO::segment_cells, 0, false},
     {"host_threads", &DpO::host_threads, 1, false}, {"host_tables", &DpO::host_tables, 0, false}, {"delta_cap_entries", &DpO::delta_cap_entries, 0, true},
+    {"pair_levels", &DpO::pair_levels, 0, false}, {"pair_min", &DpO::pair_min, 1, false},
     {"lattice_chunk_cells", &DpO::chunk_units_cfg, 1, false},
 };
 static int dp_option(dg_ctx *c, const char *what, const char *key, const int64_t *set, int64_t *get) {
diff --git a/dipgenie_amd/csrc/dg_dp_sweep.hip b/dipgenie_amd/csrc/dg_dp_sweep.hip
--- a/dipgenie_amd/csrc/dg_dp_sweep.hip
+++ b/dipgenie_amd/csrc/dg_dp_sweep.hip
@@ -50,8 +50,8 @@
 __device__ __forceinline__ void sweep_level_pairs(const SweepArgs &A, int lvl, int wave_id, int n_waves) {
     const LevelDesc d = A.descs[lvl];
     const int RP = A.RP;
-    const int32_t *__restrict__ cur = (const int32_t *)(A.ring + (size_t)DG_SLOT(lvl - 1) * A.slot_bytes + A.pad_bytes);
-    int32_t *__restrict__ nxt = (int32_t *)(A.ring + (size_t)DG_SLOT(lvl) * A.slot_bytes + A.pad_bytes);
+    const int32_t *__restrict__ cur = (const int32_t *)(A.ring + (size_t)(DG_SLOT(lvl - 1) ^ A.flip) * A.slot_bytes + A.pad_bytes);
+    int32_t *__restrict__ nxt = (int32_t *)(A.ring + (size_t)(DG_SLOT(lvl) ^ A.flip) * A.slot_bytes + A.pad_bytes);
     const int lane = threadIdx.x & 63;
     const int nchunk = (RP + RC - 1) / RC;
     const int64_t ntask = (int64_t)d.k2 * d.ngroups * nchunk;
@@ -389,7 +389,7 @@
     const int g = (int)blockIdx.x * DG_PLAIN_GW + (wv % DG_PLAIN_GW);
     const int r0 = ((int)blockIdx.y * DG_PLAIN_CH + wv / DG_PLAIN_GW) * RC;
     if (g >= nblocks || r0 >= (rp_k & 0x1FFF)) return;
-    int32_t *nxt = (int32_t *)(A.ring + (size_t)DG_SLOT(lvl) * A.slot_bytes + A.pad_bytes);
+    int32_t *nxt = (int32_t *)(A.ring + (size_t)(DG_SLOT(lvl) ^ A.flip) * A.slot_bytes + A.pad_bytes);
     sweep_task<RC, DIGEST, GENERAL, 0>(H, A, d, state_rsrc(cur, buf_bytes), nxt, (int)blockIdx.z, g, r0, lvl);
 }
 
@@ -400,7 +400,7 @@
                                                             FastArgs A, LevelDesc d, int lvl, const uint16_t *dm, int dT, const int32_t *__restrict__ heavy_rows) {
     const LevelHead H{rowrec_l, slots_l, rowx_l, cur, dm, rowx_stride, rp_k & 0x1FFF, rp_k >> 13, A.pad_bytes, dT, A.buf_bytes};
     publish_level(A.progress, lvl);
-    int32_t *nxt = (int32_t *)(A.ring + (size_t)DG_SLOT(lvl) * A.slot_bytes + A.pad_bytes);
+    int32_t *nxt = (int32_t *)(A.ring + (size_t)(DG_SLOT(lvl) ^ A.flip) * A.slot_bytes + A.pad_bytes);
     const int r0 = (int)blockIdx.y * RC;
     const int zc = 4 * n_heavy;
     if ((int)blockIdx.z < zc) {
@@ -421,6 +421,114 @@
     sweep_task<RC, DIGEST, GENERAL, 1>(H, A, d, state_rsrc(cur, A.buf_bytes), nxt, (int)blockIdx.z - zc, g, r0, lvl);
 }
 
+template <int RC>
+__device__ __forceinline__ void relax_pair(const int (&vals)[RC], int dl, uint32_t ord, uint32_t mid, int r0, int w, int RP,
+                                           int (&bval)[RC], uint32_t (&bord)[RC], uint32_t (&bmid)[RC]) {
+#pragma unroll
+    for (int q = 0; q < RC; ++q) {
+        const int cand = vals[q] + dl;
+        const bool ok = (r0 + q < RP) & (r0 + q - w >= 0) & (vals[q] != NEG_INF);
+        const bool take = ok & ((cand > bval[q]) | ((cand == bval[q]) & (ord > bord[q])));
+        bval[q] = take ? cand : bval[q];
+        bord[q] = take ? ord : bord[q];
+        bmid[q] = take ? mid : bmid[q];
+    }
+}
+__device__ __forceinline__ void merge_best_pair(int ov, uint32_t oo, uint32_t om, bool same, int &bv, uint32_t &bo, uint32_t &bm) {
+    const bool take = same & ((ov > bv) | ((ov == bv) & (oo > bo)));
+    bv = take ? ov : bv;
+    bo = take ? oo : bo;
+    bm = take ? om : bm;
+}
+
+template <int RC>
+__global__ __launch_bounds__(256) void dp_sweep_pair_kernel(const uint2 *prow_l, const uint4 *pslots_l, const int32_t *cur, const uint16_t *dm1, const uint16_t *dm2,
+                                                            int nblocks, int rp_k, int pad_bytes, int dT1, int dT2, uint32_t buf_bytes,
+                                                            int32_t *__restrict__ nxt, uint16_t *__restrict__ bp1, uint16_t *__restrict__ bp2, int kk, int nt, int *progress, int lvl) {
+    publish_level(progress, lvl);
+    const int lane = threadIdx.x & 63;
+    const int g = (int)blockIdx.x * 4 + (int)(threadIdx.x >> 6), r0 = (int)blockIdx.y * RC, i2 = (int)blockIdx.z;
+    const int RP = rp_k & 0x1FFF, k0 = rp_k >> 13;
+    if (g >= nblocks) return;
+    const uint2 rec = prow_l[i2 * PAIR_MAX_INDEG + (lane & (PAIR_MAX_INDEG - 1))];
+    const uint4 sl = pslots_l[g * 64 + lane];
+    const __amdgpu_buffer_rsrc_t cur_rsrc = state_rsrc(cur, buf_bytes);
+    const int du = __builtin_amdgcn_readfirstlane((int)(rec.x >> 25)) & 0xF;
+    const int steps = __builtin_amdgcn_readfirstlane((int)(sl.z >> 16)) & 0xF;
+    const bool act = sl.x != 0xFFFFFFFFu;
+    const int j = (int)(sl.x & 0x7FFFu), wv = (int)((sl.x >> 15) & 1u) + (int)((sl.x >> 24) & 1u);
+    const uint32_t lanemid = (((sl.x >> 16) & 0xFFu) << 8) | ((sl.x >> 24) & 1u);
+    const int j2 = act ? (int)((sl.z >> 20) & 0xFFu) : -1 - lane;
+    const int c2 = dT2 ? (int)(sl.y & 0xFFFFu) : 0, c1 = dT1 ? (int)(sl.y >> 16) : 0;
+    const uint32_t ordc = ((uint32_t)(BP_MAX_RANK - (int)(sl.z & 0xFFu)) << 16) | (uint32_t)(BP_MAX_RANK - (int)((sl.z >> 8) & 0xFFu));
+    int bval[RC];
+    uint32_t bord[RC], bmid[RC];
+#pragma unroll
+    for (int q = 0; q < RC; ++q) { bval[q] = NEG_INF; bord[q] = 0; bmid[q] = 0; }
+    const int rowbytes = k0 * 4;
+    constexpr int U = RC >= 4 ? 4 : 8;
+    for (int t = 0; t < du; t += U) {
+        if (act) {
+            int vals[U][RC], dl[U];
+#pragma unroll
+            for (int u = 0; u < U; ++u) {
+                if (t + u < du) {
+                    const uint32_t px = (uint32_t)__builtin_amdgcn_readlane((int)rec.x, t + u), py = (uint32_t)__builtin_amdgcn_readlane((int)rec.y, t + u);
+                    const int iu = (int)(px & 0x7FFFu), w = (int)((px >> 15) & 1u) + (int)((px >> 24) & 1u) + wv;
+                    const int off = ((iu * RP + (r0 - w)) * k0 + j) * 4 + pad_bytes;
+                    dl[u] = (int)dm2[(int)(py & 0x7FFu) * dT2 + c2] + (int)dm1[(int)((py >> 11) & 0x7FFu) * dT1 + c1];
+#pragma unroll
+                    for (int q = 0; q < RC; ++q) vals[u][q] = __builtin_amdgcn_raw_buffer_load_b32(cur_rsrc, off + q * rowbytes, 0, 0);
+                }
+            }
+#pragma unroll
+            for (int u = 0; u < U; ++u) {
+                if (t + u < du) {
+                    const uint32_t px = (uint32_t)__builtin_amdgcn_readlane((int)rec.x, t + u), py = (uint32_t)__builtin_amdgcn_readlane((int)rec.y, t + u);
+                    const int w = (int)((px >> 15) & 1u) + (int)((px >> 24) & 1u) + wv;
+                    const uint32_t ord = ((uint32_t)(BP_MAX_RANK - (int)((py >> 22) & 7u)) << 24) | ((uint32_t)(BP_MAX_RANK - (int)((py >> 25) & 7u)) << 8) | ordc;
+                    const uint32_t mid = ((((px >> 16) & 0xFFu) << 16) | ((px >> 24) & 1u)) + lanemid;
+                    relax_pair<RC>(vals[u], dl[u], ord, mid, r0, w, RP, bval, bord, bmid);
+                }
+            }
+        }
+    }
+    if (steps > 0) {
+        const int oj2 = lane_down1(j2);
+        const bool same = (lane + 1 < 64) & (oj2 == j2);
+#pragma unroll
+        for (int q = 0; q < RC; ++q) merge_best_pair(lane_down1(bval[q]), (uint32_t)lane_down1((int)bord[q]), (uint32_t)lane_down1((int)bmid[q]), same, bval[q], bord[q], bmid[q]);
+    }
+    for (int st = 1, sh = 2; st < steps; ++st, sh <<= 1) {
+        const int oj2 = __shfl_down(j2, sh);
+        const bool same = (lane + sh < 64) & (oj2 == j2);
+#pragma unroll
+        for (int q = 0; q < RC; ++q)
+            merge_best_pair(__shfl_down(bval[q], sh), (uint32_t)__shfl_down((int)bord[q], sh), (uint32_t)__shfl_down((int)bmid[q], sh), same, bval[q], bord[q], bmid[q]);
+    }
+    const int pj2 = lane_up1(j2);
+    const bool head = act & ((lane == 0) | (pj2 != j2));
+    if (head) {
+        const int k1 = kk & 0xFF, k2 = kk >> 8;
+#pragma unroll
+        for (int q = 0; q < RC; ++q) {
+            const int r2 = r0 + q;
+            if (r2 < RP) {
+                const int idx = (i2 * RP + r2) * k2 + j2;
+                nxt[idx] = bval[q];
+                if (bp2) {
+                    const uint32_t b2 = ~(bord[q] >> 16);
+                    if (nt) store_bp_nt(&bp2[idx], b2); else bp2[idx] = (uint16_t)b2;
+                    if (bord[q]) {
+                        const uint32_t m = bmid[q];
+                        bp1[((int)(m >> 16) * RP + r2 - (int)(m & 0xFFu)) * k1 + (int)((m >> 8) & 0xFFu)] = (uint16_t)~bord[q];
+                    }
+                }
+            }
+        }
+    }
+}
+
 constexpr int WARM_RANGES = 5;
 struct WarmRanges { const char *p[WARM_RANGES]; long long n16[WARM_RANGES]; };
 __global__ __launch_bounds__(256) void dp_warm_tables_kernel(WarmRanges W) {
@@ -453,7 +561,8 @@
 }
 __global__ void dp_pf_probe_set_kernel(PfCtl *c, int token) { __hip_atomic_store(&c->probe, token, __ATOMIC_RELAXED, __HIP_MEMORY_SCOPE_AGENT); }
 
-__global__ __launch_bounds__(64) void dp_l2_prefetch_kernel(const LevelDesc *__restrict__ descs, FastArgs F, PfCtl *ctl, int seq, int lb, int le, int ahead_near, int delta_resident, int far) {
+__global__ __launch_bounds__(64) void dp_l2_prefetch_kernel(const LevelDesc *__restrict__ descs, FastArgs F, PfCtl *ctl, int seq, int lb, int le, int ahead_near, int delta_resident, int far,
+                                                            const int32_t *__restrict__ pair_at, const PairDesc *__restrict__ pairs, const uint2 *__restrict__ prow, const uint4 *__restrict__ pslots) {
     __shared__ int dump[64];
 #define DG_DROP_LOAD(PTR) __builtin_amdgcn_global_load_lds((const __attribute__((address_space(1))) void *)(PTR), (__attribute__((address_space(3))) void *)dump, 4, 0, 0)
     const bool far_role = (int)blockIdx.x >= PF_WORKGROUPS;
@@ -481,6 +590,20 @@
         if (lp - lv > ahead) { __builtin_amdgcn_s_sleep(48); continue; }
         const LevelDesc &d = descs[lp];
         const int k2 = __builtin_amdgcn_readfirstlane(d.k2), T = __builtin_amdgcn_readfirstlane(d.T);
+        const int pa = pair_at ? __builtin_amdgcn_readfirstlane(pair_at[lp]) : -1;
+        if (pa == -2) { ++lp; ++done; continue; }
+        if (pa >= 0) {
+            const PairDesc &p = pairs[pa];
+            lines((const char *)(prow + p.row_first), 8LL * PAIR_MAX_INDEG * k2);
+            lines((const char *)(pslots + p.slot_first), 1024LL * p.nblocks);
+            if (delta_resident) {
+                const LevelDesc &d1 = descs[lp - 1];
+                if (d.delta_off >= 0 && (long long)T * T <= (128 << 10)) lines((const char *)(F.delta + d.delta_off), 2LL * T * T);
+                if (d1.delta_off >= 0 && (long long)d1.T * d1.T <= (128 << 10)) lines((const char *)(F.delta + d1.delta_off), 2LL * d1.T * d1.T);
+            }
+            ++lp; ++done;
+            continue;
+        }
         lines((const char *)(F.rowrec + d.b0), 16LL * k2);
         lines((const char *)(F.slots + d.slot_first), 512LL * d.nblocks);
         lines((const char *)(F.in_edge + d.in_base), 4LL * T);
@@ -538,11 +661,11 @@
     A.grp_begin = S.d_grp.as<uint32_t>(); A.in_dst = S.d_in_dst.as<int32_t>(); A.dead_cols = S.d_dead.as<int32_t>();
     A.delta = A.delta_zero = S.d_delta.as<uint16_t>();
     A.ring = S.d_ring.as<char>(); A.slot_bytes = S.state_alloc_bytes; A.pad_bytes = 4 * (size_t)S.pad_front;
-    A.bp = nullptr; A.digest = S.d_digest.as<unsigned long long>(); A.RP = S.RP;
+    A.bp = nullptr; A.digest = S.d_digest.as<unsigned long long>(); A.RP = S.RP; A.flip = 0;
     FastArgs &F = X.F;
     F.rowrec = S.d_rowrec.as<uint4>(); F.slots = S.d_slots.as<uint2>(); F.in_edge = A.in_edge; F.rowx = S.d_rowx.as<uint32_t>(); F.dead_cols = A.dead_cols;
     F.delta = F.delta_zero = A.delta; F.bp = nullptr; F.digest = A.digest; F.RP = S.RP;
-    F.ring = S.d_ring.as<char>(); F.slot_bytes = (uint32_t)S.state_alloc_bytes;
+    F.ring = S.d_ring.as<char>(); F.slot_bytes = (uint32_t)S.state_alloc_bytes; F.flip = 0;
 #ifdef DG_SWEEP_PROBE
     F.probe = S.d_probe.as<unsigned long long>();
 #endif
@@ -588,11 +711,12 @@
         const dim3 grid((unsigned)((d.nblocks + 3) / 4), (unsigned)nch, (unsigned)(d.k2 + (v.coop ? 4 * d.n_heavy : 0)));
         const dim3 pgrid((unsigned)((d.nblocks + DG_PLAIN_GW - 1) / DG_PLAIN_GW), (unsigned)((nch + DG_PLAIN_CH - 1) / DG_PLAIN_CH), grid.z);
         const int32_t *hv = S.d_heavy.as<int32_t>();
-        const FastArgs &F = X.F;
+        FastArgs F = X.F;
+        F.flip = X.flip;
         const uint4 *rowrec_l = F.rowrec + d.b0;
         const uint2 *slots_l = F.slots + d.slot_first;
         const uint32_t *rowx_l = F.rowx + d.rowx_off;
-        const int32_t *cur = (const int32_t *)(F.ring + (size_t)DG_SLOT(l - 1) * F.slot_bytes);
+        const int32_t *cur = (const int32_t *)(F.ring + (size_t)(DG_SLOT(l - 1) ^ X.flip) * F.slot_bytes);
         const int dT = d.delta_off >= 0 ? d.T : 0;
         const uint16_t *dm = dT ? F.delta + d.delta_off - (int64_t)d.in_base * dT : F.delta_zero;
         const int rp_k = S.RP | (d.k << 13);
@@ -605,12 +729,54 @@
         const int nchunk = (S.RP + X.rc_sel - 1) / X.rc_sel;
         const int64_t ntask = (int64_t)d.k2 * d.ngroups * nchunk;
         const unsigned grid = (unsigned)std::min<int64_t>((ntask + 3) / 4, S.opt.max_blocks);
-        const SweepArgs &A = X.A;
+        SweepArgs A = X.A;
+        A.flip = X.flip;
         auto generic = [&](auto RC, auto DG, auto) { hipLaunchKernelGGL((dp_sweep_kernel<RC.value, DG.value>), dim3(grid), dim3(256), 0, s, A, l); };
         launched = launch_variant<RC_ALL>(X.rc_sel, X.digest, false, generic);
     }
     if (!launched) { set_error("sweep of level %d: no %s kernel is instantiated for chunks of %d recombination counts", l, v.coop ? "cooperative" : v.rc ? "fast" : "generic", v.rc ? v.rc : X.rc_sel); return DG_ERR_STATE; }
     X.hist.n[(size_t)v.index()]++;
+    return DG_OK;
+}
+
+static int choose_pair_rc(const DpState &S, const PairDesc &p) {
+    int best_q = 0;
+    double best = 1e300;
+    for (int q = 0; q < N_PAIR_RCS; ++q) {
+        const int rc = PAIR_RCS[q];
+        const double W = (double)p.k2 * p.nblocks * ((S.RP + rc - 1) / rc);
+        const double T = std::max(1.0, W / (double)S.opt.rc_cap) * ((double)S.opt.rc_t0_ns + (double)p.dmax * rc * (double)S.opt.rc_tg_ps * 1e-3) + W * (double)S.opt.rc_tw_ps * 1e-3;
+        if (T <= best) { best = T; best_q = q; }
+    }
+    return best_q;
+}
+std::string pair_variant_name(int q) { return "dp_sweep_pair_kernel<" + std::to_string(PAIR_RCS[q]) + ">"; }
+
+template <int Q = 0>
+static void launch_pair_rc(int q, dim3 grid, hipStream_t s, const uint2 *prow_l, const uint4 *pslots_l, const int32_t *cur, const uint16_t *dm1, const uint16_t *dm2, int nblocks, int rp_k,
+                           int pad_bytes, int dT1, int dT2, uint32_t buf_bytes, int32_t *nxt, uint16_t *bp1, uint16_t *bp2, int kk, int nt, int *progress, int lvl) {
+    if constexpr (Q < N_PAIR_RCS) {
+        if (q == Q) hipLaunchKernelGGL((dp_sweep_pair_kernel<PAIR_RCS[Q]>), grid, dim3(256), 0, s, prow_l, pslots_l, cur, dm1, dm2, nblocks, rp_k, pad_bytes, dT1, dT2, buf_bytes, nxt, bp1, bp2, kk, nt, progress, lvl);
+        else launch_pair_rc<Q + 1>(q, grid, s, prow_l, pslots_l, cur, dm1, dm2, nblocks, rp_k, pad_bytes, dT1, dT2, buf_bytes, nxt, bp1, bp2, kk, nt, progress, lvl);
+    }
+}
+
+int sweep_launch_pair(const DpState &S, SweepLaunch &X, int l, hipStream_t s) {
+    const PairDesc &p = S.pairs[(size_t)S.pair_at[l]];
+    const LevelDesc &d2 = S.descs[l], &d1 = S.descs[l - 1];
+    const FastArgs &F = X.F;
+    const int q = choose_pair_rc(S, p), rc = PAIR_RCS[q];
+    const int nch = (S.RP + rc - 1) / rc;
+    const dim3 grid((unsigned)((p.nblocks + 3) / 4), (unsigned)nch, (unsigned)p.k2);
+    const int32_t *cur = (const int32_t *)(F.ring + (size_t)(DG_SLOT(l - 2) ^ X.flip) * F.slot_bytes);
+    int32_t *nxt = (int32_t *)(F.ring + (size_t)(DG_SLOT(l - 1) ^ X.flip) * F.slot_bytes + F.pad_bytes);
+    const int dT1 = d1.delta_off >= 0 ? d1.T : 0, dT2 = d2.delta_off >= 0 ? d2.T : 0;
+    const uint16_t *dm1 = dT1 ? F.delta + d1.delta_off : F.delta_zero, *dm2 = dT2 ? F.delta + d2.delta_off : F.delta_zero;
+    const int nt = (int64_t)d2.k2 * d2.k2 * S.RP >= S.opt.bp_nt_min_cells ? 1 : 0;
+    launch_pair_rc(q, grid, s, S.d_prow.as<uint2>() + p.row_first, S.d_pslots.as<uint4>() + p.slot_first, cur, dm1, dm2, p.nblocks, S.RP | (p.k0 << 13), F.pad_bytes, dT1, dT2,
+                   F.buf_bytes, nxt, F.bp ? F.bp + d1.bp_off : nullptr, F.bp ? F.bp + d2.bp_off : nullptr, p.k1 | (p.k2 << 8), nt, F.progress, l);
+    X.flip ^= 1;
+    X.pair_hist.n[q]++;
     return DG_OK;
 }
 
@@ -672,7 +838,8 @@
     DG_HIP(hipStreamWaitEvent(S.pf_stream, S.pf_ev, 0));
     const int far = (int)S.opt.pf_far;
     hipLaunchKernelGGL(dp_l2_prefetch_kernel, dim3(PF_WORKGROUPS + (far > 0 ? PF_FAR_WORKGROUPS : 0)), dim3(64), 0, S.pf_stream, S.d_descs.as<LevelDesc>(), X.F,
-                       S.d_pfctl.as<PfCtl>(), seq, lb, le, (int)S.opt.l2_prefetch, delta_resident ? 1 : 0, far);
+                       S.d_pfctl.as<PfCtl>(), seq, lb, le, (int)S.opt.l2_prefetch, delta_resident ? 1 : 0, far,
+                       X.pairs_ok ? S.d_pair_at.as<int32_t>() : (const int32_t *)nullptr, S.d_pairs.as<PairDesc>(), S.d_prow.as<uint2>(), S.d_pslots.as<uint4>());
     S.pf_active = true;
     return DG_OK;
 }
diff --git a/dipgenie_amd/csrc/dg_dp_tables.hip b/dipgenie_amd/csrc/dg_dp_tables.hip
--- a/dipgenie_amd/csrc/dg_dp_tables.hip
+++ b/dipgenie_amd/csrc/dg_dp_tables.hip
@@ -530,6 +530,8 @@
     S.n_dtrans = (int64_t)dtrans.size();
     S.n_edges = g->out_off[nV];
     plan_delta_windows(S, dtrans, dblk_first);
+    if (int rc = dp_build_pairs(c, g, S)) return rc;
+    lap("level pairs");
     const size_t n_edges = (size_t)g->out_off[nV];
     const size_t st_bytes = (size_t)S.max_level_cells * 4 * 2, dl_bytes = (size_t)S.delta_buf_entries * 2;
     size_t bp_bytes = 0, ck_bytes = 0;
@@ -543,7 +545,7 @@
     if (int rc = S.d_ckpt.ensure(ck_bytes)) return rc;
     if (int rc = S.d_pfctl.ensure(256)) return rc;
     DG_HIP(hipMemsetAsync(S.d_pfctl.p, 0, 256, s));
-    S.pad_front = 2 * (int64_t)max_k;
+    S.pad_front = (S.pairs.empty() ? 2 : 4) * (int64_t)max_k;
     const size_t pad_bytes = 4 * (size_t)(S.pad_front + 33 * (int64_t)max_k);
     S.state_alloc_bytes = (((size_t)S.max_level_cells * 4 + pad_bytes) + 255) & ~(size_t)255;
     if (int rc = S.d_ring.ensure(S.state_alloc_bytes * 2)) return rc;
diff --git a/include/dipgenie_hip.h b/include/dipgenie_hip.h
--- a/include/dipgenie_hip.h
+++ b/include/dipgenie_hip.h
@@ -96,6 +96,8 @@
 int dg_dp_get_table_digest(dg_ctx *, uint64_t *out, int n);
 int dg_dp_get_launch_profile(dg_ctx *, char *buf, int cap);
 int dg_dp_list_sweep_variants(char *buf, int cap);
+int dg_dp_get_pair_profile(dg_ctx *, char *buf, int cap);
+int dg_dp_list_pair_variants(char *buf, int cap);
 
 typedef struct dg_hap_graph {
     int32_t n_vertices, R;
```

After: 65.63 billion, median of 6. 10.0% higher.
